# IntelLabs/bayesian-torch

Hardware: AMD Instinct MI355X
Metric: MC-samples/sec (Bayesian-ResNet18, 224^2, bs=64) (higher is better)
Workload: dtype bf16

## Files before the change

### bayesian_torch_amd/_lib.py

```python
import ctypes
import os

_HERE = os.path.dirname(os.path.abspath(__file__))
_LIB = None

KIND_REPARAM, KIND_FLIPOUT = 0, 1
ACT_F32, ACT_BF16 = 0, 1
PREC_F32, PREC_BF16, PREC_BF16X3 = 0, 1, 2
PREC_CODE = {"f32": 0, "bf16": 1, "bf16x3": 2}
FLAG_TRANSPOSED, FLAG_KL_ACCUM, FLAG_ROWFUSE, FLAG_OUT_F32, FLAG_OUT_BF16, FLAG_GATHER, FLAG_SWAP_SIGNS, FLAG_CONCURRENT = 1, 2, 4, 8, 16, 32, 64, 128
FLAG_REVERSE = 256
E_UNSUPPORTED = -3
STREAM_EPS_W, STREAM_EPS_B, STREAM_SIGN_IN, STREAM_SIGN_OUT = 0, 1, 2, 3
ABI_VERSION = 9
FLAG_LANES_SHIFT = 16
FLAG_LANES_MASK = 0xff << FLAG_LANES_SHIFT
SAMPLE_SKIP_MU = 1


class BtxError(RuntimeError):
    pass


class Geom(ctypes.Structure):
    _fields_ = [(n, ctypes.c_int32) for n in (
        "NB", "D", "H", "W", "C", "N", "KD", "KH", "KW", "sd", "sh", "sw", "pd", "ph", "pw",
        "dd", "dh", "dw", "od", "oh", "ow", "groups")]


class Rng(ctypes.Structure):
    _fields_ = [("seed", ctypes.c_uint64), ("sample_idx", ctypes.c_uint32), ("layer_id", ctypes.c_uint32),
                ("sample_idx_dev", ctypes.c_void_p)]


class BnFuse(ctypes.Structure):
    _fields_ = [("residual", ctypes.c_void_p), ("relu", ctypes.c_int32), ("mask", ctypes.c_void_p), ("dres", ctypes.c_void_p)]


class Epilogue(ctypes.Structure):
    _fields_ = [("scale", ctypes.c_void_p), ("shift", ctypes.c_void_p), ("residual", ctypes.c_void_p),
                ("relu", ctypes.c_int32), ("pool", ctypes.c_int32)]


class Lanes(ctypes.Structure):
    _fields_ = [("n", ctypes.c_int32), ("x_stride", ctypes.c_int64), ("out_stride", ctypes.c_int64),
                ("res_stride", ctypes.c_int64)]


class PlanInfo(ctypes.Structure):
    _fields_ = [(n, ctypes.c_int32) for n in ("family", "ksplits", "kper", "kgroups", "wide", "tall", "par_major", "pool_band",
                                              "nwg", "lanes")] + [("ws_bytes", ctypes.c_uint64)]


FAMILIES = ("gather", "regstage", "dma", "gemm8", "patch", "taps", "taps2", "stem", "stem_pool")


class Noise(ctypes.Structure):
    _fields_ = [("eps_w", ctypes.c_void_p), ("eps_b", ctypes.c_void_p),
                ("sign_in", ctypes.c_void_p), ("sign_out", ctypes.c_void_p), ("sampled_w", ctypes.c_void_p)]


class SampleItem(ctypes.Structure):
    _fields_ = [("geom", ctypes.POINTER(Geom)), ("mu_w", ctypes.c_void_p), ("rho_w", ctypes.c_void_p),
                ("out", ctypes.c_void_p), ("kind", ctypes.c_int32), ("layer_id", ctypes.c_uint32),
                ("src_KW", ctypes.c_int32), ("src_C", ctypes.c_int32)]


class LstmLayer(ctypes.Structure):
    _fields_ = [("mu_w", ctypes.c_void_p), ("rho_w", ctypes.c_void_p), ("mu_b", ctypes.c_void_p), ("rho_b", ctypes.c_void_p),
                ("layer_id", ctypes.c_uint32), ("sample_idx", ctypes.c_uint32), ("sample_idx_dev", ctypes.c_void_p)]


class LstmGrads(ctypes.Structure):
    _fields_ = [("dmu_w", ctypes.c_void_p), ("drho_w", ctypes.c_void_p), ("dmu_b", ctypes.c_void_p), ("drho_b", ctypes.c_void_p)]


class KlItem(ctypes.Structure):
    _fields_ = [("mu", ctypes.c_void_p), ("rho", ctypes.c_void_p), ("prior_mu_t", ctypes.c_void_p),
                ("prior_sigma_t", ctypes.c_void_p), ("dmu", ctypes.c_void_p), ("drho", ctypes.c_void_p),
                ("prior_mu", ctypes.c_float), ("prior_sigma", ctypes.c_float), ("n", ctypes.c_size_t)]


class Q8Chain(ctypes.Structure):
    _fields_ = [(n, ctypes.c_float) for n in ("s_sigma", "s_mu", "s_eps", "inv_s_eps", "s_d", "inv_s_d", "inv_s_w")] + \
               [("bias_div", ctypes.c_double)]


class Q8Add(ctypes.Structure):
    _fields_ = [(n, ctypes.c_float) for n in ("s_a", "pre_a", "s_b", "pre_b", "inv_s")] + \
               [("zero_point", ctypes.c_int32), ("relu", ctypes.c_int32)]


class Q8Delta(ctypes.Structure):
    _fields_ = [("inv_s_eps", ctypes.c_float), ("mult", ctypes.c_float), ("mean_bias", ctypes.c_int32), ("pert_bias", ctypes.c_int32),
                ("div_mean", ctypes.c_double), ("div_pert", ctypes.c_double)]


class Q8Flipout(ctypes.Structure):
    _fields_ = [(n, ctypes.c_int32) for n in ("z_x", "z_xp", "z_mean", "z_pert", "z_p2", "sin_pos", "sin_neg", "sout_pos", "sout_neg")] + \
               [(n, ctypes.c_float) for n in ("mult_xp", "mult_mean", "mult_pert", "mult_p2", "out_scale")]


class OptimItem(ctypes.Structure):
    _fields_ = [("p", ctypes.c_void_p), ("g", ctypes.c_void_p), ("state0", ctypes.c_void_p), ("state1", ctypes.c_void_p),
                ("n", ctypes.c_int64)]


class OptimHyper(ctypes.Structure):
    _fields_ = [(n, ctypes.c_float) for n in ("neg_lr", "wd", "decay_mul", "one_m_b1", "b2", "one_m_b2", "eps", "neg_step_size",
                                              "bc2s", "momentum", "one_m_damp")] + \
               [("flags", ctypes.c_uint32), ("reserved", ctypes.c_uint32 * 4)]


OPT_MAXIMIZE, OPT_NESTEROV, OPT_DECOUPLED, OPT_FIRST_STEP, OPT_COUPLED_WD = 1, 2, 4, 8, 16
OPTIM_CHUNK, OPTIM_MAX_ITEMS = 4096, 65536
Q8_BIAS_NONE, Q8_BIAS_MU, Q8_BIAS_SIGMA_EPS = 0, 1, 2

EXPORTS = ("btx_abi_version", "btx_strerror", "btx_kl_workspace_bytes", "btx_kl_gauss", "btx_kl_model_workspace_bytes",
           "btx_kl_gauss_model", "btx_kl_gauss_model_bwd", "btx_contract_wgrad",
           "btx_contract_workspace_bytes", "btx_contract_fwd", "btx_contract_fwd_ex", "btx_contract_fwd_lanes", "btx_contract_pool_shape", "btx_contract_plan_info", "btx_out_shape", "btx_fill_eps", "btx_fill_sign", "btx_rho_grad",
           "btx_mc_packed_floats", "btx_mc_accumulate", "btx_mc_accumulate_lanes", "btx_sampled_w_bytes", "btx_sample_weights", "btx_sampled_w_bytes_lanes", "btx_sample_weights_lanes", "btx_rowfuse_pack", "btx_maxpool2d_cl", "btx_avgpool_global_cl",
           "btx_bn_workspace_bytes", "btx_bn_train_fwd", "btx_bn_train_bwd", "btx_dgrad_weights",
           "btx_wgrad_workspace_bytes", "btx_contract_wgrad_ws", "btx_maxpool2d_cl_train", "btx_maxpool2d_cl_bwd",
           "btx_lstm_workspace_bytes", "btx_lstm_fwd", "btx_lstm_train_saved_bytes", "btx_lstm_train_workspace_bytes",
           "btx_lstm_fwd_train", "btx_lstm_bwd",
           "btx_calib_workspace_bytes", "btx_avu_fwd", "btx_avu_bwd", "btx_eau_fwd", "btx_eau_bwd",
           "btx_q8_weight_row_bytes", "btx_q8_quantize_act", "btx_q8_sample_weights", "btx_q8_contract",
           "btx_q8_add", "btx_q8_contract_res", "btx_q8_maxpool2d_cl", "btx_q8_avgpool2d_cl",
           "btx_q8_sample_delta", "btx_q8_contract_flipout",
           "btx_optim_sgd", "btx_optim_adam", "btx_optim_grad_norm_workspace_bytes", "btx_optim_grad_norm",
           "btx_mcloss_workspace_bytes", "btx_mc_ce_fwd", "btx_mc_ce_bwd", "btx_avu_mc_fwd", "btx_avu_mc_bwd",
           "btx_bias_grad_workspace_bytes", "btx_bias_grad")


# ... 172 lines not shown
```

### bayesian_torch_amd/csrc/btx_api.hip

```cpp
#include <hip/hip_runtime.h>
#include <math.h>
#include <string.h>
#include "../../include/btx.h"
#include <stdlib.h>
#include "btx_contract.h"
#include "btx_rng.h"
#include "btx_presample.h"

using namespace btx;

static int contract_fwd_impl(int kind, const BtxGeom* g, const void* x, const float* mu_w, const float* rho_w,
                             const float* mu_b, const float* rho_b, void* out, const BtxRng* rng, const BtxNoise* noise,
                             int act_dtype, int prec, uint32_t flags, void* ws, size_t ws_bytes, void* stream,
                             const BtxEpilogue* ep, const BtxLanes* ln) {
  if (!g || !x || !mu_w || !rho_w || !out || !rng) return BTX_E_NULL;
  const int lanes = ln ? ln->n : 1;
  if ((mu_b == nullptr) != (rho_b == nullptr)) return BTX_E_NULL;
  const uintptr_t al = (uintptr_t)x | (uintptr_t)mu_w | (uintptr_t)rho_w | (uintptr_t)out |
                       (uintptr_t)(noise && noise->eps_w ? noise->eps_w : nullptr) |
                       (uintptr_t)(ep && ep->residual ? ep->residual : nullptr);
  FwdSel sel;
  int rc = select_fwd(kind, g, act_dtype, prec, flags, (al & 15) != 0, noise, ep, &sel);
  if (rc) return rc;
  const Plan& pl = sel.pl;
  const void* sampled_w = (noise && noise->sampled_w) ? noise->sampled_w : nullptr;
  if (sel.need && (!ws || ws_bytes < sel.need)) return BTX_E_WORKSPACE;
  if (sel.need && (((uintptr_t)ws) & 15)) return BTX_E_ALIGN;

  ContractParams p;
  memset(&p, 0, sizeof(p));
  p.x = x; p.mu = mu_w; p.rho = rho_w; p.mu_b = mu_b; p.rho_b = rho_b; p.out = out;
  p.partial = pl.ksplits > 1 ? (float*)ws : nullptr;
  p.lanes = lanes; p.lane_nwg = pl.nwg; p.fd_lane_nwg = make_fastdiv((uint32_t)(pl.nwg > 0 ? pl.nwg : 1));
  if (lanes > 1) {
    p.lane_x = ln->x_stride; p.lane_out = ln->out_stride; p.lane_res = ln->res_stride;
    p.lane_partial = (long long)(plan_ws(pl, g, 1));
  }
  if (noise) {
    p.eps_w = noise->eps_w; p.eps_b = noise->eps_b;
    p.sign_in = noise->sign_in; p.sign_out = noise->sign_out;
  }
  p.NB = g->NB; p.D = g->D; p.H = g->H; p.W = g->W; p.C = g->C; p.Cg = pl.Cg;
  p.Do = pl.Do; p.Ho = pl.Ho; p.Wo = pl.Wo; p.N = g->N; p.Ng = pl.Ng;
  p.KD = g->KD; p.KH = g->KH; p.KW = g->KW;
  p.sd = g->sd; p.sh = g->sh; p.sw = g->sw; p.pd = g->pd; p.ph = g->ph; p.pw = g->pw;
  p.dd = g->dd; p.dh = g->dh; p.dw = g->dw;
  p.M = pl.M; p.K = pl.K;
  p.mtiles = pl.mtiles; p.ntiles = pl.ntiles; p.groups = g->groups; p.ksplits = pl.ksplits; p.kper = pl.kper;
  p.transposed = (flags & BTX_FLAG_TRANSPOSED) ? 1 : 0;
  p.pointwise = (!p.transposed && g->KD == 1 && g->KH == 1 && g->KW == 1 && g->sd == 1 && g->sh == 1 && g->sw == 1 &&
                 g->pd == 0 && g->ph == 0 && g->pw == 0) ? 1 : 0;
  p.out_bf16 = sel.out_bf16;
  if (ep) { p.ep_scale = ep->scale; p.ep_shift = ep->shift; p.ep_res = ep->residual; p.ep_relu = ep->relu; }
  if (flags & BTX_FLAG_ROWFUSE) {
    p.Cg = g->KW * g->C;
    p.KW = 1;
    p.sign_unaligned = 1;
  }
  p.fd_Cg = make_fastdiv((uint32_t)p.Cg); p.fd_KW = make_fastdiv((uint32_t)p.KW); p.fd_KH = make_fastdiv((uint32_t)p.KH);
  p.seed_lo = (uint32_t)rng->seed; p.seed_hi = (uint32_t)(rng->seed >> 32);
  p.sample = rng->sample_idx; p.layer = rng->layer_id;
  p.sample_ptr = rng->sample_idx_dev;
  p.fd_sd = make_fastdiv((uint32_t)g->sd); p.fd_sh = make_fastdiv((uint32_t)g->sh); p.fd_sw = make_fastdiv((uint32_t)g->sw);
  if (sel.par_major) {
    p.par_major = 1; p.par_Hh = pl.Ho / 2; p.par_Wh = pl.Wo / 2; p.par_Mq = g->NB * p.par_Hh * p.par_Wh; p.par_Mqp = sel.par_mqp;
    p.fd_par_Mqp = make_fastdiv((uint32_t)p.par_Mqp); p.fd_par_Hh = make_fastdiv((uint32_t)p.par_Hh);
    p.fd_par_Wh = make_fastdiv((uint32_t)p.par_Wh);
  }
  p.swap_signs = (flags & BTX_FLAG_SWAP_SIGNS) ? 1 : 0;
  p.reverse = (flags & BTX_FLAG_REVERSE) ? 1 : 0;
  sign_keys(rng, p.swap_signs ? BTX_STREAM_SIGN_OUT : BTX_STREAM_SIGN_IN, &p.kin_a, &p.kin_b);
  sign_keys(rng, p.swap_signs ? BTX_STREAM_SIGN_IN : BTX_STREAM_SIGN_OUT, &p.kout_a, &p.kout_b);
  {
    const long long in_elems = (long long)g->NB * g->D * g->H * g->W * g->C;
    const long long xb = in_elems * (act_dtype == BTX_ACT_BF16 ? 2 : 4), wb = (long long)g->N * pl.K * 4;
    p.x_bytes = xb < 0xffffffffLL ? (uint32_t)xb : 0xffffffffu;
    p.w_bytes = wb < 0xffffffffLL ? (uint32_t)wb : 0xffffffffu;
  }

  p.fd_inner = make_fastdiv((uint32_t)(pl.ntiles * g->groups * pl.ksplits)); p.fd_ksplits = make_fastdiv((uint32_t)pl.ksplits);
  p.fd_ntiles = make_fastdiv((uint32_t)pl.ntiles); p.fd_rtiles = make_fastdiv(1u);
  p.fd_mtiles = make_fastdiv((uint32_t)(pl.mtiles > 0 ? pl.mtiles : 1));
  {
    const double w_b = (prec == BTX_PREC_BF16 ? 2.0 : 4.0) * (double)g->N * pl.K * (kind == BTX_KIND_FLIPOUT ? 2 : 1);
    p.wg_order = (uses_tiles(sel.family) && pl.mtiles > 1 && w_b >= WG_MAJOR_MIB * 1048576.0) ? 1 : 0;
  }
  p.fd_Wo = make_fastdiv((uint32_t)pl.Wo); p.fd_Ho = make_fastdiv((uint32_t)pl.Ho); p.fd_Do = make_fastdiv((uint32_t)pl.Do);
  if (uses_tiles(sel.family)) {
    p.wt = sampled_w ? (void*)sampled_w : (void*)((unsigned char*)ws + sel.wt_off);
    p.wt_ready = sampled_w ? 1 : 0;
    p.wt_bytes = (uint32_t)sel.wt_all;
    p.wt_delta_off = (uint32_t)sel.wt_one;
    p.lane_wt = (long long)sel.wt_one;
    p.lane_wt_delta = (kind == BTX_KIND_FLIPOUT) ? 1 : 0;
  }
  hipStream_t st = (hipStream_t)stream;
  typedef int (*LaunchFn)(int, const ContractParams&, int, hipStream_t);
  auto launch = [&](LaunchFn f32, LaunchFn bf16, LaunchFn x3) {
    return (prec == BTX_PREC_BF16 ? bf16 : prec == BTX_PREC_BF16X3 ? x3 : f32)(kind, p, pl.nwg * lanes, st);
  };
  switch (sel.family) {
    case BTX_FAMILY_STEM_POOL: {
      const StemPoolPlan& spp = sel.spp;
      p.pt_R = spp.PB; p.pt_rtiles = spp.bands; p.pt_Rp = spp.Rp; p.pt_astage = spp.astage; p.st_sbytes = spp.sbytes;
      p.pt_lds = spp.lds; p.pt_PP = spp.patch_bytes; p.sp_Hq = spp.Hq; p.sp_Wq = spp.Wq;
      p.fd_rtiles = make_fastdiv((uint32_t)spp.bands);
      rc = launch_stem_pool_bf16(kind, p, pl.nwg * lanes, st);
      break;
    }
    case BTX_FAMILY_STEM: {
      const StemPlan& stp = sel.stp;
      p.pt_R = stp.R; p.pt_Rp = stp.Rp; p.pt_rtiles = stp.rtiles; p.pt_nw = stp.nw; p.pt_astage = stp.astage;
      p.st_sbytes = stp.sbytes; p.pt_lds = stp.lds; p.pt_PP = stp.patch_bytes;
      p.fd_rtiles = make_fastdiv((uint32_t)stp.rtiles);
      rc = launch(launch_contract_stem_f32, launch_contract_stem_bf16, launch_contract_stem_x3);
      break;
    }
    case BTX_FAMILY_PATCH:
    case BTX_FAMILY_TAPS:
    case BTX_FAMILY_TAPS2: {
      const PatchPlan& pt = sel.pt;
      p.pt_G = pt.G; p.pt_R = pt.R; p.pt_Rp = pt.Rp; p.pt_Wp = pt.Wp; p.pt_PP = pt.PP; p.pt_NI = pt.NI;
      p.fd_ptWp = make_fastdiv((uint32_t)pt.Wp); p.fd_ptRp = make_fastdiv((uint32_t)pt.Rp); p.fd_ptR = make_fastdiv((uint32_t)pt.R);
      p.fd_rtiles = make_fastdiv((uint32_t)pt.rtiles);
      p.pt_rtiles = pt.rtiles; p.pt_nw = pt.nw; p.pt_astage = pt.astage; p.pt_lds = pt.lds;
      p.pt_taps = pt.taps; p.pt_kg = pt.kg; p.pt_lds_g = pt.lds_g;
      p.pt_wide = (pt.taps == 33 || pt.taps == 332) ? pt.wide : 0;
      if (p.pt_wide) {
        p.fd_ntiles = make_fastdiv((uint32_t)(pl.ntiles / 2));
        p.fd_inner = make_fastdiv((uint32_t)((pl.ntiles / 2) * g->groups * pl.ksplits));
      }
      p.pt_tall = pt.tall; p.pt_P = pt.P; p.pt_Wt = pt.Wt; p.pt_ncs = pt.ncs;
      p.fd_P = make_fastdiv((uint32_t)pt.P); p.fd_Wt = make_fastdiv((uint32_t)pt.Wt); p.fd_ncs = make_fastdiv((uint32_t)pt.ncs);
      rc = launch(launch_contract_patch_f32, launch_contract_patch_bf16, launch_contract_patch_x3);
      break;
    }
    case BTX_FAMILY_GEMM8:
      p.pt_rtiles = sel.g8_pairs;
      p.fd_rtiles = make_fastdiv((uint32_t)sel.g8_pairs); p.fd_inner = make_fastdiv((uint32_t)(sel.g8_pairs * g->groups));
      rc = launch(launch_contract_gemm8_f32, launch_contract_gemm8_bf16, launch_contract_gemm8_x3);
      break;
    case BTX_FAMILY_DMA:
      rc = launch(launch_contract_dma_f32, launch_contract_dma_bf16, launch_contract_dma_x3);
      break;
    default: {
      const bool gen2 = sel.family == BTX_FAMILY_GATHER || (noise && (noise->eps_w || noise->sign_in));
      rc = (prec == BTX_PREC_BF16) ? launch_contract_bf16(kind, act_dtype == BTX_ACT_BF16, gen2, p, pl.nwg * lanes, st)
                                   : launch_contract_f32(kind, act_dtype == BTX_ACT_BF16, gen2, p, pl.nwg * lanes, st);
    }
  }
  if (rc) return rc;
  if (pl.ksplits > 1) {
    const long long total = (long long)pl.M * g->N;
// ... 124 lines not shown
```

### bayesian_torch_amd/csrc/btx_contract.h

```cpp
#pragma once
#include <hip/hip_runtime.h>
#include <stdint.h>
#include "btx_rng.h"
#include "btx_plan.h"

typedef __attribute__((ext_vector_type(8))) __bf16 bf16x8;
typedef __attribute__((ext_vector_type(4))) __bf16 bf16x4;
typedef __attribute__((ext_vector_type(4))) float f32x4;
typedef __attribute__((ext_vector_type(8))) float f32x8;
typedef __attribute__((ext_vector_type(16))) float f32x16;
typedef __attribute__((ext_vector_type(4))) uint32_t u32x4;
typedef __attribute__((ext_vector_type(2))) uint32_t u32x2;

namespace btx {

constexpr int NTHREADS = 512;
constexpr int ACTS_OFF = 0;
constexpr int SIGN_OFF = NG * BM * 16;
constexpr int WMU_OFF = SIGN_OFF + NG * BM * 4;
constexpr int WDL_OFF = WMU_OFF + NG * BN * 16;
constexpr int STAGE_BYTES = WDL_OFF + NG * BN * 16;
constexpr int LDS_BYTES = 2 * STAGE_BYTES;

struct FastDiv {
  uint32_t m, sh;
};
static inline FastDiv make_fastdiv(uint32_t d) {
  FastDiv f;
  uint32_t l = 0;
  while ((1ull << l) < d) ++l;
  f.m = (uint32_t)((((1ull << l) - d) << 32) / d + 1);
  f.sh = (l < 1 ? l : 1) | ((l > 0 ? l - 1 : 0) << 8);
  return f;
}
__device__ __forceinline__ uint32_t fdiv(uint32_t x, const FastDiv& f) {
  const uint32_t t = __umulhi(x, f.m);
  return (t + ((x - t) >> (f.sh & 31u))) >> (f.sh >> 8);
}
static inline void sign_keys(const BtxRng* rng, uint32_t stream, uint32_t* ka, uint32_t* kb) {
  const BtxPhilox4 k = btx_philox4x32_10(0u, rng->sample_idx, rng->layer_id, stream, (uint32_t)rng->seed,
                                         (uint32_t)(rng->seed >> 32));
  *ka = k.x[0];
  *kb = k.x[1];
}
__device__ __forceinline__ void fdivmod(uint32_t x, const FastDiv& f, uint32_t d, uint32_t& q, uint32_t& r) {
  q = fdiv(x, f);
  r = x - q * d;
}

struct ContractParams {
  const void* x;
  const float* mu;
  const float* rho;
  const float* mu_b;
  const float* rho_b;
  void* out;
  float* partial;
  const float* eps_w;
  const float* eps_b;
  const int8_t* sign_in;
  const int8_t* sign_out;
  int NB, D, H, W, C, Cg;
  int Do, Ho, Wo, N, Ng;
  int KD, KH, KW;
  int sd, sh, sw, pd, ph, pw, dd, dh, dw;
  int M, K;
  int mtiles, ntiles, groups, ksplits, kper;
  int transposed;
  int pointwise;
  uint32_t seed_lo, seed_hi, sample, layer;
  const uint32_t* sample_ptr;
  uint32_t kin_a, kin_b, kout_a, kout_b;
  const float* ep_scale;
  const float* ep_shift;
  const void* ep_res;
  int ep_relu;
  int out_bf16;
  int sign_unaligned;
  uint32_t x_bytes, w_bytes;
  int pt_G, pt_R, pt_Rp, pt_Wp, pt_PP, pt_NI, pt_rtiles;
  FastDiv fd_Wo, fd_Ho, fd_Do, fd_ptWp, fd_ptRp, fd_ptR;
  FastDiv fd_inner, fd_ksplits, fd_ntiles, fd_Cg, fd_KW, fd_KH, fd_rtiles;
  FastDiv fd_mtiles;
  int swap_signs;
  int par_major, par_Mq, par_Mqp, par_Hh, par_Wh;
  FastDiv fd_par_Mqp, fd_par_Hh, fd_par_Wh;
  FastDiv fd_sd, fd_sh, fd_sw;
  int wg_order;
  int pt_nw, pt_astage, pt_lds;
  int pt_kg;
  int pt_lds_g;
  int pt_taps;
  int pt_wide;
  int sp_Hq, sp_Wq;
  int st_sbytes;
  void* wt;
  uint32_t wt_bytes, wt_delta_off;
  int wt_ready;
  int pt_tall, pt_P, pt_Wt, pt_ncs;
  FastDiv fd_P, fd_Wt, fd_ncs;
  int lanes, lane_nwg;
  FastDiv fd_lane_nwg;
  long long lane_x, lane_out, lane_res, lane_wt, lane_partial;
  int lane_wt_delta;
  int reverse;
};

__device__ __forceinline__ uint32_t sample_word_scalar(const uint32_t* ptr) {
  return *(const __attribute__((address_space(4))) uint32_t*)(uintptr_t)ptr;
}

__device__ __forceinline__ int xcd_logical() {
  const int nwg = gridDim.x, L = blockIdx.x;
  const int q = nwg >> 3, r = nwg & 7, xcd = L & 7, slot = L >> 3;
  return (xcd < r ? xcd * (q + 1) : r * (q + 1) + (xcd - r) * q) + slot;
}

__device__ __forceinline__ ContractParams lane_view(const ContractParams& q, int& logical) {
  ContractParams p = q;
  if (q.reverse) logical = (int)gridDim.x - 1 - logical;
  if (q.lanes > 1) {
    uint32_t lane, loc;
    fdivmod((uint32_t)logical, q.fd_lane_nwg, (uint32_t)q.lane_nwg, lane, loc);
    logical = (int)loc;
    const long long l = (long long)lane;
    p.x = (const unsigned char*)q.x + l * q.lane_x;
    p.out = (unsigned char*)q.out + l * q.lane_out;
    if (q.ep_res) p.ep_res = (const unsigned char*)q.ep_res + l * q.lane_res;
    if (q.wt) {
      if (q.lane_wt_delta) p.wt_delta_off = q.wt_delta_off + (uint32_t)(l * q.lane_wt);
      else p.wt = (unsigned char*)q.wt + l * q.lane_wt;
    }
    if (q.partial) p.partial = (float*)((unsigned char*)q.partial + l * q.lane_partial);
    if (q.sample_ptr) p.sample_ptr = q.sample_ptr + lane;
    p.sample = q.sample + lane;
  }
  return p;
}

#define BTX_SECTION_PARAMS(name, logical_var)                                                                         \
  const __attribute__((address_space(4))) ContractParams* name##_karg =                                               \
      (const __attribute__((address_space(4))) ContractParams*)__builtin_amdgcn_kernarg_segment_ptr();                \
  asm volatile("" : "+s"(name##_karg));                                                                               \
  int logical_var = xcd_logical();                                                                                    \
  const ContractParams name = lane_view(*(const ContractParams*)name##_karg, logical_var)

__device__ __forceinline__ ContractParams lane_view_flat(const ContractParams& q, int& logical) {
  ContractParams p = q;
  const int q_rev = q.reverse, q_lnwg = q.lane_nwg, q_lwd = q.lane_wt_delta;
  const FastDiv q_fd = {q.fd_lane_nwg.m, q.fd_lane_nwg.sh};
  const long long q_lx = q.lane_x, q_lo = q.lane_out, q_lr = q.lane_res, q_lw = q.lane_wt, q_lp = q.lane_partial;
  const unsigned char* q_x = (const unsigned char*)q.x;
  unsigned char* q_out = (unsigned char*)q.out;
  const unsigned char* q_res = (const unsigned char*)q.ep_res;
  unsigned char* q_wt = (unsigned char*)q.wt;
  unsigned char* q_part = (unsigned char*)q.partial;
  const uint32_t* q_sp = q.sample_ptr;
  const uint32_t q_smp = q.sample, q_wdo = q.wt_delta_off;
  asm volatile("" ::"s"(q_rev), "s"(q_lnwg), "s"(q_lwd), "s"(q_fd.m), "s"(q_fd.sh), "s"(q_lx), "s"(q_lo), "s"(q_lr), "s"(q_lw), "s"(q_lp), "s"(q_x),
               "s"(q_out), "s"(q_res), "s"(q_wt), "s"(q_part), "s"(q_sp), "s"(q_smp), "s"(q_wdo));
  logical = q_rev ? (int)gridDim.x - 1 - logical : logical;
  uint32_t lane, loc;
  fdivmod((uint32_t)logical, q_fd, (uint32_t)q_lnwg, lane, loc);
  logical = (int)loc;
  const long long l = (long long)lane;
  const long long wo = l * q_lw;
  p.x = q_x + l * q_lx;
  p.out = q_out + l * q_lo;
  p.ep_res = q_res ? (const void*)(q_res + l * q_lr) : nullptr;
  p.wt_delta_off = q_wdo + (q_lwd ? (uint32_t)wo : 0u);
  p.wt = q_wt ? (void*)(q_wt + (q_lwd ? 0ll : wo)) : nullptr;
  p.partial = q_part ? (float*)(q_part + l * q_lp) : nullptr;
  p.sample_ptr = q_sp ? q_sp + lane : nullptr;
  p.sample = q_smp + lane;
  return p;
}
#define BTX_SECTION_PARAMS_FLAT(name, logical_var)                                                                    \
  const __attribute__((address_space(4))) ContractParams* name##_karg =                                               \
      (const __attribute__((address_space(4))) ContractParams*)__builtin_amdgcn_kernarg_segment_ptr();                \
  asm volatile("" : "+s"(name##_karg));                                                                               \
  int logical_var = xcd_logical();                                                                                    \
  const ContractParams name = lane_view_flat(*(const ContractParams*)name##_karg, logical_var)


struct RngLive {
  uint32_t sample, kin_a, kin_b, kout_a, kout_b;
};
template <int KIND>
// ... 621 lines not shown
```

### bayesian_torch_amd/csrc/btx_contract_patch.h

```cpp
#pragma once
#include <type_traits>
#include "btx_contract.h"
#include "btx_contract_dma.h"
#include "btx_epilogue.h"
#include "btx_presample.h"
#include "btx_mma.h"
#include "btx_contract_taps.h"
#include "btx_contract_taps2.h"

namespace btx {



template <int PREC, int KIND, int NW, int MI>
__global__ __launch_bounds__(64 * NW, (MI == 4) ? 1 : 2) void contract_patch_kernel(const ContractParams) {
  BTX_SECTION_PARAMS(p, logical);
  const RngLive rl = rng_live<KIND>(p);
  constexpr int NT = 64 * NW;
  constexpr int WPX = 32 * MI;
  constexpr int MAXNI = (MI == 4) ? 16 : PT_MAXNI;
  constexpr int SJ = (MI == 4) ? 4 : 2;
  using ACT = typename std::conditional<PREC == 1, __bf16, float>::type;
  constexpr int G = (PREC == 1) ? 8 : 4;
  constexpr int BK = NG * G;
// ... 180 lines not shown
      int allowed = nissued - m1;
      if (next_cb && t == (T >= 2 ? T - 2 : 0)) allowed = min(allowed, nissued - mpiece);
      wait_vmcnt(allowed);
      asm volatile("s_waitcnt lgkmcnt(0)\n\ts_barrier" ::: "memory");
      m1 = m2;
      if (++t == T) { t = 0; ++cbi; }
    };
    int s = 0;
    for (; s + 1 < nstages; s += 2) {
      iter(s, fa, fb);
      iter(s + 1, fb, fa);
    }
    if (s < nstages) iter(s, fa, fb);
  }

  {
    BTX_SECTION_PARAMS(pe, logical2);
    const int nimg = min(pe.pt_G, pe.NB - img0), nrow = min(pe.pt_R, pe.Ho - row0);
    const int nvalid = nimg * nrow * pe.Wo;
    const uint32_t m0 = (uint32_t)(img0 * pe.Ho + row0) * (uint32_t)pe.Wo;
    if constexpr (MI == 2) {
      staged_epilogue<KIND, NW>(pe, rl, accm, accd, smem, tid, wave, lane, ntile, group, split, m0, nvalid);
    } else {
#pragma unroll
      for (int hf = 0; hf < MI / 2; ++hf) {
        __builtin_amdgcn_sched_barrier(0);
        staged_epilogue<KIND, NW>(pe, rl, reinterpret_cast<const f32x16(&)[2][2]>(accm[2 * hf]),
                                  reinterpret_cast<const f32x16(&)[2][2]>(accd[2 * hf]), smem, tid, wave, lane, ntile,
                                  group, split, m0, nvalid, wave * (MI / 2) + hf, hf == 0);
      }
    }
  }
}

template <int PREC>
static int launch_contract_patch_impl(int kind, const ContractParams& p, int nwg, hipStream_t st) {
#define BTX_LAUNCH_PT(KIND, NW, MI)                                                                                 \
  do {                                                                                                            \
    auto kfn = contract_patch_kernel<PREC, KIND, NW, MI>;                                                           \
    static bool attr_done = false;                                                                                \
    if (!attr_done) {                                                                                             \
      hipError_t e = hipFuncSetAttribute((const void*)kfn, hipFuncAttributeMaxDynamicSharedMemorySize, 163840);   \
      if (e != hipSuccess) return (int)e;                                                                         \
      attr_done = true;                                                                                           \
    }                                                                                                             \
    hipLaunchKernelGGL(kfn, dim3(nwg), dim3(64 * NW), p.pt_lds, st, p);                                           \
  } while (0)
  int rc = launch_presample_impl<PREC>(kind, p, st);
  if (rc) return rc;
  if (p.pt_taps == 332) {
#define BTX_LAUNCH_T2(KIND, ...)                                                                                  \
  do {                                                                                                            \
    auto kfn = contract_taps2_kernel<PREC, KIND, ##__VA_ARGS__>;                                                  \
    static bool attr_done = false;                                                                                \
    if (!attr_done) {                                                                                             \
      hipError_t e = hipFuncSetAttribute((const void*)kfn, hipFuncAttributeMaxDynamicSharedMemorySize, 163840);   \
      if (e != hipSuccess) return (int)e;                                                                         \
      attr_done = true;                                                                                           \
    }                                                                                                             \
    hipLaunchKernelGGL(kfn, dim3(nwg), dim3(256), p.pt_lds, st, p);                                               \
  } while (0)
    if constexpr (PREC == 1) {
      if (p.pt_wide && kind == 0) {
        BTX_LAUNCH_T2(0, true);
        return (int)hipGetLastError();
      }
    }
    if (kind == 0) BTX_LAUNCH_T2(0); else BTX_LAUNCH_T2(1);
#undef BTX_LAUNCH_T2
    return (int)hipGetLastError();
  }
  if (p.pt_taps == 33) {
#define BTX_LAUNCH_TP(KIND, KG, ...)                                                                               \
  do {                                                                                                            \
    auto kfn = contract_taps_kernel<PREC, KIND, 3, 3, KG, ##__VA_ARGS__>;                                           \
    static bool attr_done = false;                                                                                \
    if (!attr_done) {                                                                                             \
      hipError_t e = hipFuncSetAttribute((const void*)kfn, hipFuncAttributeMaxDynamicSharedMemorySize, 163840);   \
      if (e != hipSuccess) return (int)e;                                                                         \
      attr_done = true;                                                                                           \
    }                                                                                                             \
    hipLaunchKernelGGL(kfn, dim3(nwg), dim3(256 * KG), p.pt_lds, st, p);                                          \
  } while (0)
    if (p.pt_kg == 2) { if (kind == 0) BTX_LAUNCH_TP(0, 2); else BTX_LAUNCH_TP(1, 2); }
    else {
      if constexpr (PREC == 1) {
        if (p.pt_wide && kind == 0) {
          BTX_LAUNCH_TP(0, 1, true);
          return (int)hipGetLastError();
        }
      }
      if (kind == 0) BTX_LAUNCH_TP(0, 1); else BTX_LAUNCH_TP(1, 1);
    }
#undef BTX_LAUNCH_TP
    return (int)hipGetLastError();
  }
  if (p.pt_nw == 4) { if (kind == 0) BTX_LAUNCH_PT(0, 4, 2); else BTX_LAUNCH_PT(1, 4, 2); }
  else { if (kind == 0) BTX_LAUNCH_PT(0, 8, 2); else BTX_LAUNCH_PT(1, 8, 2); }
#undef BTX_LAUNCH_PT
  return (int)hipGetLastError();
}

}
```

### bayesian_torch_amd/csrc/btx_contract_taps.h

```cpp
#pragma once
#include <type_traits>
#include "btx_contract.h"
#include "btx_contract_dma.h"
#include "btx_epilogue.h"
#include "btx_mma.h"

namespace btx {

__device__ __forceinline__ void dma16s(__amdgpu_buffer_rsrc_t rsrc, uint32_t voff, uint32_t soff,
                                       unsigned char* lds_wave_base) {
  __builtin_amdgcn_raw_ptr_buffer_load_lds(rsrc, (__attribute__((address_space(3))) void*)lds_wave_base, 16, voff, soff,
                                           0, 0);
}

template <int N>
__device__ __forceinline__ void end_stage() {
  asm volatile("s_waitcnt vmcnt(%0)\n\ts_waitcnt lgkmcnt(0)\n\ts_barrier" ::"n"(N) : "memory");
}

template <int I, int N, class F>
__device__ __forceinline__ void static_for(F&& f) {
  if constexpr (I < N) {
    f(std::integral_constant<int, I>{});
    static_for<I + 1, N>(f);
  }
}

constexpr int TP_MAXNI = 6;

template <int T>
constexpr int tp_pieces(int t) {
  constexpr int PST = T - 3;
  constexpr int PPS = (TP_MAXNI + PST - 1) / PST;
  if (t < 0) t += T;
  if (t >= PST) return 0;
  int n = 0;
  for (int i = 0; i < PPS; ++i)
    if (t + PST * i < TP_MAXNI) ++n;
  return n;
}

template <int PREC, int KIND, int KH, int KW, int KG, bool WIDE = false>
__global__ __launch_bounds__(256 * KG, 2) void contract_taps_kernel(const ContractParams) {
  static_assert(!WIDE || (PREC == 1 && KG == 1 && KIND == 0), "wide tile: bf16 Reparameterization, one K-group");
  constexpr int K2 = (KIND == 1 || WIDE) ? 1 : 0;
  BTX_SECTION_PARAMS(p, logical);
  constexpr int NW = 4, NT = 256, MI = 2, T = KH * KW;
  static_assert(T >= 5 && T <= 32, "tap-unrolled kernel: 5..32 taps");
  constexpr int MAXNI = TP_MAXNI;
  constexpr int PST = T - 3;
  constexpr int WOPS = K2 ? 2 : 1;
  using ACT = typename std::conditional<PREC == 1, __bf16, float>::type;
  constexpr int G = (PREC == 1) ? 8 : 4;
  constexpr int BK = NG * G;
  constexpr int ESZ = (int)sizeof(ACT);
  extern __shared__ __attribute__((aligned(16))) unsigned char smem_all[];

  uint32_t smp = p.sample;
  if (p.sample_ptr) smp = sample_word_scalar(p.sample_ptr);

  const int tid = threadIdx.x & 255;
  const int lane = tid & 63;
  const int l31 = lane & 31;
  const int h = lane >> 5;
  const int wave_all = __builtin_amdgcn_readfirstlane((int)(threadIdx.x >> 6));
  const int wave = wave_all & 3;
  const int kg = (KG == 1) ? 0 : (wave_all >> 2);
  unsigned char* const smem = smem_all + kg * p.pt_lds_g;

  uint32_t u_mtile, u_rem, u_split, u_ntile, u_group, u_t;
  const uint32_t ntg = (uint32_t)(WIDE ? p.ntiles >> 1 : p.ntiles);
  if (p.wg_order) fdivmod((uint32_t)logical, p.fd_mtiles, (uint32_t)p.mtiles, u_rem, u_mtile);
  else fdivmod((uint32_t)logical, p.fd_inner, ntg * (uint32_t)(p.groups * p.ksplits), u_mtile, u_rem);
  fdivmod(u_rem, p.fd_ksplits, (uint32_t)p.ksplits, u_t, u_split);
  fdivmod(u_t, p.fd_ntiles, ntg, u_group, u_ntile);
  const int mtile = (int)u_mtile, split = (int)u_split, ntile = (int)u_ntile, group = (int)u_group;

  const bool tall = p.pt_tall != 0;
  uint32_t u_ig, u_rt;
  if (tall) fdivmod((uint32_t)mtile, p.fd_ncs, (uint32_t)p.pt_ncs, u_rt, u_ig);
  else fdivmod((uint32_t)mtile, p.fd_rtiles, (uint32_t)p.pt_rtiles, u_ig, u_rt);
  const int img0 = tall ? 0 : (int)u_ig * p.pt_G, row0 = (int)u_rt * p.pt_R, col0 = tall ? (int)u_ig * p.pt_Wt : 0;
  auto patch_src = [&](int q, bool& ok) __attribute__((always_inline)) -> uint32_t {
    uint32_t ut, upc, ugi, upr;
    fdivmod((uint32_t)q, p.fd_ptWp, (uint32_t)p.pt_Wp, ut, upc);
    int img, ih, iw;
    if (tall) {
      fdivmod((uint32_t)row0 + ut, p.fd_P, (uint32_t)p.pt_P, ugi, upr);
      img = (int)ugi; ih = (int)upr - p.ph; iw = col0 + (int)upc - p.pw;
      ok = (int)ut < p.pt_Rp;
    } else {
      fdivmod(ut, p.fd_ptRp, (uint32_t)p.pt_Rp, ugi, upr);
      img = img0 + (int)ugi; ih = row0 + (int)upr - p.ph; iw = (int)upc - p.pw;
      ok = true;
    }
    ok = ok && img < p.NB && (unsigned)ih < (unsigned)p.H && (unsigned)iw < (unsigned)p.W;
    return (uint32_t)((img * p.H + ih) * p.W + iw);
  };
  const int ncb_total = p.Cg / BK;
  const int cb_per = p.kper / BK;
  const int cb0 = split * cb_per + kg * (cb_per / KG);
  const int ncb = (KG == 1) ? min(ncb_total, cb0 + cb_per) - cb0 : cb_per / KG;
  const int a_stage = p.pt_astage, s_stage = p.pt_astage >> 4;
  const int PT_A_OFF = 0, PT_S_OFF = 2 * a_stage, PT_W_OFF = 2 * a_stage + 2 * s_stage;
  const int PT_X_OFF = PT_W_OFF + PT_WD * DW_STAGE;

  const __amdgpu_buffer_rsrc_t x_rsrc = __builtin_amdgcn_make_buffer_rsrc((void*)p.x, 0, p.x_bytes, 0x00020000);
  const __amdgpu_buffer_rsrc_t wt_rsrc = __builtin_amdgcn_make_buffer_rsrc((void*)p.wt, 0, p.wt_bytes, 0x00020000);

  const uint32_t w_voff = (uint32_t)lane * 16u + (uint32_t)wave * 1024u;
  const uint32_t w_sbase = (uint32_t)(group * p.ntiles + (WIDE ? 2 * ntile : ntile)) * (uint32_t)(p.K / G) * 1024u;
  const uint32_t w_second = WIDE ? (uint32_t)(p.K / G) * 1024u : p.wt_delta_off;
  const uint32_t CgG = (uint32_t)(p.Cg / G);
  const int w_lds = PT_W_OFF + wave * 1024;
  int wslot = 0;
  auto issue_w = [&](uint32_t tap, uint32_t cb, int slot) __attribute__((always_inline)) {
    const uint32_t soff = w_sbase + (tap * CgG + cb * (uint32_t)NG) * 1024u;
    unsigned char* ld = smem + w_lds + slot * DW_STAGE;
    dma16s(wt_rsrc, w_voff, soff, ld);
    if constexpr (K2) dma16s(wt_rsrc, w_voff, soff + w_second, ld + 4096);
  };
  if (ncb > 0) issue_w(0u, (uint32_t)cb0, 0);

  uint32_t sg_off[2];
  bool sg_ok[2];
  uint32_t* const pix_tab = (uint32_t*)(smem + PT_S_OFF + s_stage);
#pragma unroll
  for (int j = 0; j < 2; ++j) {
    const int q = tid + NT * j;
    sg_ok[j] = q < p.pt_PP;
    bool inside;
    const uint32_t ipix = patch_src(sg_ok[j] ? q : 0, inside);
    sg_off[j] = ipix * (uint32_t)p.C + (uint32_t)(group * p.Cg);
    if (q * 4 < s_stage) pix_tab[q] = (sg_ok[j] && inside) ? sg_off[j] : 0xffffffffu;
    if (p.sign_in)
      sg_ok[j] = sg_ok[j] && inside;
  }
  asm volatile("s_waitcnt lgkmcnt(0)\n\ts_barrier" ::: "memory");

  const int g_lane = (lane & 3) ^ ((lane >> 4) & 3);
  uint32_t pp_boff[MAXNI];
  uint32_t pmask = 0;
  uint32_t pp_e[MAXNI];
#pragma unroll
  for (int j = 0; j < MAXNI; ++j) {
    const int q = 16 * (wave + NW * j) + (lane >> 2);
    pp_e[j] = pix_tab[q < p.pt_PP ? q : 0];
  }
#pragma unroll
  for (int j = 0; j < MAXNI; ++j) {
    const int q = 16 * (wave + NW * j) + (lane >> 2);
    uint32_t bo = DMA_OOB;
    if (j < p.pt_NI && q < p.pt_PP) {
      const uint32_t e = pp_e[j];
      if (e != 0xffffffffu) bo = (e + (uint32_t)(G * g_lane)) * (uint32_t)ESZ;
    }
    pp_boff[j] = bo;
    if (j < p.pt_NI && 16 * (wave + NW * j) < p.pt_PP) {
      pmask |= 1u << j;
      if (ncb > 0)
        dma16(x_rsrc, bo == DMA_OOB ? DMA_OOB : bo + (uint32_t)(cb0 * BK * ESZ), smem + PT_A_OFF + (wave + NW * j) * 1024);
    }
  }
  pmask = __builtin_amdgcn_readfirstlane(pmask);
  if (ncb > 0) {
    issue_w(1u, (uint32_t)cb0, 1);
    issue_w(2u, (uint32_t)cb0, 2);
  }

  RngLive rl = {smp, p.kin_a, p.kin_b, p.kout_a, p.kout_b};
  if (p.sample_ptr || p.lanes > 1) {
    rl.sample = __builtin_amdgcn_readfirstlane(smp);
    if constexpr (KIND == 1) {
      const uint32_t si = p.swap_signs ? 3u : 2u, so = p.swap_signs ? 2u : 3u;
      const BtxPhilox4 ki = btx_philox4x32_10(0u, rl.sample, p.layer, si, p.seed_lo, p.seed_hi);
      const BtxPhilox4 ko = btx_philox4x32_10(0u, rl.sample, p.layer, so, p.seed_lo, p.seed_hi);
      rl.kin_a = __builtin_amdgcn_readfirstlane(ki.x[0]); rl.kin_b = __builtin_amdgcn_readfirstlane(ki.x[1]);
      rl.kout_a = __builtin_amdgcn_readfirstlane(ko.x[0]); rl.kout_b = __builtin_amdgcn_readfirstlane(ko.x[1]);
    }
  }

  auto write_signs = [&](int slot, int cb) __attribute__((always_inline)) {
    if constexpr (KIND == 1) {
      unsigned char* ss = smem + PT_S_OFF + slot * s_stage;
#pragma unroll
      for (int j = 0; j < 2; ++j) {
        if (sg_ok[j]) {
          const uint32_t off = sg_off[j] + (uint32_t)(cb * BK);
          uint32_t w;
          if (p.sign_in) w = sign_word_explicit(p.sign_in, off, p.x_bytes / (uint32_t)ESZ);
          else w = btx_sign_word(off >> 5, rl.kin_a, rl.kin_b);
          if constexpr (G == 4) w <<= 8 * ((off >> 4) & 1);
          *(uint32_t*)(ss + (tid + NT * j) * 4) = w;
        }
      }
    }
  };

  int q0[MI];
#pragma unroll
  for (int mi = 0; mi < MI; ++mi) {
    const int pl = wave * 64 + mi * 32 + l31;
    uint32_t ut, uc, ugi, ur;
    if (tall) {
      fdivmod((uint32_t)pl, p.fd_Wt, (uint32_t)p.pt_Wt, ur, uc);
      q0[mi] = ((int)ur < p.pt_R) ? (int)ur * p.pt_Wp + (int)uc : 0;
    } else {
      fdivmod((uint32_t)pl, p.fd_Wo, (uint32_t)p.Wo, ut, uc);
      fdivmod(ut, p.fd_ptR, (uint32_t)p.pt_R, ugi, ur);
      const int c = (int)uc, r = (int)ur, gi = (int)ugi;
      const bool ok = (gi < p.pt_G) && (img0 + gi < p.NB) && (row0 + r < p.Ho);
      q0[mi] = ok ? (gi * p.pt_Rp + r) * p.pt_Wp + c : 0;
    }
  }
  const int row_step = p.dh * p.pt_Wp;

  constexpr bool ZI = (PREC == 1 && KG == 1);
  f32x16 accm[MI][2], accd[MI][2];
  auto clear_acc = [&](int a0) __attribute__((always_inline)) {
#pragma unroll
    for (int a = 0; a < MI; ++a)
#pragma unroll
      for (int b = 0; b < 2; ++b)
#pragma unroll
        for (int r = 0; r < 16; ++r)
          if (a >= a0) { accm[a][b][r] = 0.f; accd[a][b][r] = 0.f; }
  };
  if (!ZI || ncb <= 0) clear_acc(0);

  using Frag = StageFragT<MI>;
  auto load_frag = [&](Frag& f, int aslot, int toffv, int wsl, auto mia_tag) __attribute__((always_inline)) {
    constexpr int MIA = decltype(mia_tag)::value;
    const unsigned char* as = smem + PT_A_OFF + aslot * a_stage;
    const unsigned char* ss = smem + PT_S_OFF + aslot * s_stage;
    const unsigned char* ws = smem + PT_W_OFF + wsl * DW_STAGE;
    int q[MI];
#pragma unroll
    for (int mi = 0; mi < MI; ++mi) q[mi] = q0[mi] + toffv;
#pragma unroll
    for (int kk = 0; kk < NG / 2; ++kk) {
      const int row = 2 * kk + h;
#pragma unroll
      for (int mi = 0; mi < MIA; ++mi) f.a[kk][mi] = *(const u32x4*)(as + q[mi] * 64 + ((row ^ ((q[mi] >> 2) & 3)) * 16));
#pragma unroll
      for (int ni = 0; ni < 2; ++ni) f.wm[kk][ni] = *(const u32x4*)(ws + (row * BN + ni * 32 + l31) * 16);
    }
    if constexpr (KIND == 1) {
#pragma unroll
      for (int mi = 0; mi < MIA; ++mi) f.sw[mi] = *(const uint32_t*)(ss + q[mi] * 4);
    }
  };

  if (ncb > 0) {
    write_signs(0, cb0);
    asm volatile("s_waitcnt vmcnt(%0)\n\ts_waitcnt lgkmcnt(0)\n\ts_barrier" ::"n"(KG == 1 ? WOPS : 2 * WOPS) : "memory");
    Frag fa, fb;
    const int nvalid_px = tall ? p.pt_R * p.pt_Wt : min(p.pt_G, p.NB - img0) * min(p.pt_R, p.Ho - row0) * p.Wo;
    const bool mi1_dead = wave * 64 + 32 >= nvalid_px;
    auto kloop = [&](auto mia_tag) __attribute__((always_inline)) {
    constexpr int MIA = decltype(mia_tag)::value;
    if constexpr (KG == 1) load_frag(fa, 0, 0, 0, mia_tag);
    auto block = [&](auto par_tag, auto first_tag, int cbi, bool last) __attribute__((always_inline)) {
      constexpr int PAR = decltype(par_tag)::value;
      constexpr bool FIRST = decltype(first_tag)::value;
      static_for<0, T>([&](auto t_tag) __attribute__((always_inline)) {
        constexpr int t = decltype(t_tag)::value;
        constexpr int sp = (PAR * T + t) & 1;
        Frag& cur = (KG == 1 && sp) ? fb : fa;
        Frag& nxt = (KG == 1 && sp) ? fa : fb;
        asm volatile("" : "+v"(q0[0]), "+v"(q0[1]));
        constexpr int t3 = (t + 3) % T, c3 = (t + 3) / T;
        if constexpr (c3 == 0) {
          issue_w((uint32_t)t3, (uint32_t)(cb0 + cbi), (wslot + 3) & 3);
        } else {
          if (!last) issue_w((uint32_t)t3, (uint32_t)(cb0 + cbi + 1), (wslot + 3) & 3);
        }
        constexpr int KP = tp_pieces<T>(t);
        if constexpr (t < PST) {
          if (!last) {
            const uint32_t cboff = (uint32_t)((cb0 + cbi + 1) * BK * ESZ);
#pragma unroll
            for (int i = 0; i < KP; ++i) {
              const int j = t + PST * i;
              const uint32_t bo = pp_boff[j];
              unsigned char* dst = ((pmask >> j) & 1u) ? smem + PT_A_OFF + (PAR ^ 1) * a_stage + (wave + NW * j) * 1024
                                                        : smem + PT_X_OFF;
              dma16(x_rsrc, bo == DMA_OOB ? DMA_OOB : bo + cboff, dst);
            }
            if constexpr (t == 0) write_signs(PAR ^ 1, cb0 + cbi + 1);
          }
        }
        DeltaFrag df;
        if constexpr (KG == 1) {
          load_delta<K2>(df, smem + PT_W_OFF + wslot * DW_STAGE, l31, h);
          constexpr int t1 = (t + 1) % T, c1 = (t + 1) / T;
          load_frag(nxt, PAR ^ c1, (t1 / KW) * row_step + (t1 % KW) * p.dw, (wslot + 1) & 3, mia_tag);
          if constexpr (FIRST && t == 0) stage_mma<PREC, K2, MI, MIA, true, KIND == 1>(cur, df, accm, accd, l31, h);
          else stage_mma<PREC, K2, MI, MIA, false, KIND == 1>(cur, df, accm, accd, l31, h);
          if (!last) end_stage<WOPS + KP>();
          else end_stage<(c3 == 0) ? WOPS : 0>();
        } else {
          load_delta<KIND>(df, smem + PT_W_OFF + wslot * DW_STAGE, l31, h);
          load_frag(cur, PAR, (t / KW) * row_step + (t % KW) * p.dw, wslot, mia_tag);
          __builtin_amdgcn_sched_barrier(0);
          asm volatile("s_barrier" ::: "memory");
          __builtin_amdgcn_sched_barrier(0);
          stage_mma<PREC, KIND, MI, MIA>(cur, df, accm, accd, l31, h);
          __builtin_amdgcn_sched_barrier(0);
          if (!last) {
            end_stage<2 * WOPS + KP + tp_pieces<T>(t - 1) + tp_pieces<T>(t - 2)>();
          } else {
            constexpr int a_ = (t + 3 < T) ? 1 : 0, b_ = (t == 0) ? 1 : ((t + 2 < T) ? 1 : 0);
            end_stage<WOPS * (a_ + b_)>();
          }
        }
        wslot = (wslot + 1) & 3;
      });
    };
    if (KG == 2 && kg == 1) asm volatile("s_barrier" ::: "memory");
    using P0 = std::integral_constant<int, 0>;
    using P1 = std::integral_constant<int, 1>;
    if constexpr (ZI) {
      if constexpr (MIA < MI) clear_acc(MIA);
      block(P0{}, std::true_type{}, 0, ncb == 1);
      int cbi = 1;
      for (; cbi + 2 <= ncb; cbi += 2) {
        block(P1{}, std::false_type{}, cbi, false);
        block(P0{}, std::false_type{}, cbi + 1, cbi + 2 == ncb);
      }
      if (cbi < ncb) block(P1{}, std::false_type{}, cbi, true);
    } else {
      int cbi = 0;
      for (; cbi + 2 <= ncb; cbi += 2) {
        block(P0{}, std::false_type{}, cbi, false);
        block(P1{}, std::false_type{}, cbi + 1, cbi + 2 == ncb);
      }
      if (cbi < ncb) block(P0{}, std::false_type{}, cbi, true);
    }
    if (KG == 2 && kg == 0) asm volatile("s_barrier" ::: "memory");
    };
    if (mi1_dead) kloop(std::integral_constant<int, 1>{});
    else kloop(std::integral_constant<int, 2>{});
  }

  {
    BTX_SECTION_PARAMS(pe, logical2);
    const int nimg = min(pe.pt_G, pe.NB - img0), nrow = min(pe.pt_R, pe.Ho - row0);
    const int nvalid = nimg * nrow * pe.Wo;
    const uint32_t m0 = (uint32_t)(img0 * pe.Ho + row0) * (uint32_t)pe.Wo;
    const PixTall pmt = {pe, row0, col0};
    if constexpr (KG == 1) {
      if constexpr (WIDE) {
        float* const ba0 = (float*)(smem + NW * PT_EP_WAVE);
        float* const ba1 = ba0 + 4 * BN;
        {
          const bool has_bias = (split == 0) && (pe.mu_b != nullptr);
          const bool has_aff = (pe.ksplits == 1) && ((pe.ep_scale != nullptr) || (pe.ep_shift != nullptr));
          if (has_bias || has_aff) {
            if (tid < 64) ep_fill_constants<0>(pe, rl, ba0, tid, 2 * ntile, group, has_bias, has_aff);
            else if (tid < 128) ep_fill_constants<0>(pe, rl, ba1, tid - 64, 2 * ntile + 1, group, has_bias, has_aff);
          }
          __syncthreads();
        }
        if (tall) {
          staged_epilogue_pm<0, NW, PixTall>(pe, rl, accm, accm, smem, tid, wave, lane, 2 * ntile, group, split, pmt, -1, true, ba0);
          staged_epilogue_pm<0, NW, PixTall>(pe, rl, accd, accd, smem, tid, wave, lane, 2 * ntile + 1, group, split, pmt, -1, true, ba1);
        } else {
          staged_epilogue<0, NW>(pe, rl, accm, accm, smem, tid, wave, lane, 2 * ntile, group, split, m0, nvalid, -1, true, ba0);
          staged_epilogue<0, NW>(pe, rl, accd, accd, smem, tid, wave, lane, 2 * ntile + 1, group, split, m0, nvalid, -1, true, ba1);
        }
      } else
      if (tall) staged_epilogue_pm<KIND, NW, PixTall>(pe, rl, accm, accd, smem, tid, wave, lane, ntile, group, split, pmt);
      else staged_epilogue<KIND, NW>(pe, rl, accm, accd, smem, tid, wave, lane, ntile, group, split, m0, nvalid);
    } else {
      float* ba_lds = (float*)(smem_all + 131072);
      const bool to_partial = pe.ksplits > 1;
      const bool has_bias = (split == 0) && (pe.mu_b != nullptr);
      const bool has_aff = !to_partial && ((pe.ep_scale != nullptr) || (pe.ep_shift != nullptr));
      if (kg == 1) {
#pragma unroll
        for (int mi = 0; mi < MI; ++mi)
#pragma unroll
          for (int ni = 0; ni < 2; ++ni)
#pragma unroll
            for (int c = 0; c < 4; ++c) {
              const int i = (mi * 2 + ni) * 4 + c;
              *(f32x4*)(smem_all + (i * 256 + tid) * 16) =
                  (f32x4){accm[mi][ni][4 * c], accm[mi][ni][4 * c + 1], accm[mi][ni][4 * c + 2], accm[mi][ni][4 * c + 3]};
              if constexpr (KIND == 1)
                *(f32x4*)(smem_all + ((16 + i) * 256 + tid) * 16) =
                    (f32x4){accd[mi][ni][4 * c], accd[mi][ni][4 * c + 1], accd[mi][ni][4 * c + 2], accd[mi][ni][4 * c + 3]};
            }
      } else if (has_bias || has_aff) {
        ep_fill_constants<KIND>(pe, rl, ba_lds, tid, ntile, group, has_bias, has_aff);
      }
      __syncthreads();
      if (kg == 0) {
#pragma unroll
        for (int mi = 0; mi < MI; ++mi)
#pragma unroll
          for (int ni = 0; ni < 2; ++ni)
#pragma unroll
            for (int c = 0; c < 4; ++c) {
              const int i = (mi * 2 + ni) * 4 + c;
              const f32x4 v = *(const f32x4*)(smem_all + (i * 256 + tid) * 16);
#pragma unroll
              for (int r = 0; r < 4; ++r) accm[mi][ni][4 * c + r] += v[r];
              if constexpr (KIND == 1) {
                const f32x4 w = *(const f32x4*)(smem_all + ((16 + i) * 256 + tid) * 16);
#pragma unroll
                for (int r = 0; r < 4; ++r) accd[mi][ni][4 * c + r] += w[r];
              }
            }
      }
      __syncthreads();
      if (kg == 0) {
        if (tall) staged_epilogue_pm<KIND, NW, PixTall>(pe, rl, accm, accd, smem_all, tid, wave, lane, ntile, group, split, pmt, -1,
                                                        true, ba_lds);
        else staged_epilogue<KIND, NW>(pe, rl, accm, accd, smem_all, tid, wave, lane, ntile, group, split, m0, nvalid, -1, true,
                                       ba_lds);
      }
    }
  }
}

}
```

### bayesian_torch_amd/csrc/btx_contract_taps2.h

```cpp
#pragma once
#include <type_traits>
#include "btx_contract.h"
#include "btx_contract_dma.h"
#include "btx_contract_taps.h"
#include "btx_epilogue.h"
#include "btx_mma.h"

namespace btx {

constexpr int T2_MAXNI = 5;
constexpr int T2_WD = 3;
constexpr int T2_T = 9;

constexpr int t2_seq(int s) { return s < 4 ? 0 : (s == 4 ? 1 : (s < 7 ? 2 : 3)); }
constexpr int t2_tap(int s) {
  return s == 0 ? 0 : s == 1 ? 2 : s == 2 ? 6 : s == 3 ? 8 : s == 4 ? 4 : s == 5 ? 1 : s == 6 ? 7 : s == 7 ? 3 : 5;
}
constexpr int t2_a(int k) { return (k == 0 || k == 2) ? 1 : 0; }
constexpr int t2_b(int k) { return (k == 0 || k == 3) ? 1 : 0; }
constexpr int t2_np(int s) { return (s == 0 || s == 5 || s == 7) ? 3 : ((s == 1 || s == 6 || s == 8) ? 2 : (s == 4 ? 5 : 0)); }
constexpr int t2_p0(int s) { return (s == 1 || s == 6 || s == 8) ? 3 : 0; }
constexpr int t2_fseq(int s) { return s < 2 ? 2 : (s == 4 ? 3 : (s < 7 ? 4 : 5)); }

template <int PREC, int KIND, bool WIDE = false>
// ... 174 lines not shown
    for (int kk = 0; kk < NG / 2; ++kk) {
      const int row = 2 * kk + h;
#pragma unroll
      for (int mi = 0; mi < MIA; ++mi) f.a[kk][mi] = *(const u32x4*)(as + q[mi] * 64 + ((row ^ ((q[mi] >> 2) & 3)) * 16));
#pragma unroll
      for (int ni = 0; ni < 2; ++ni) f.wm[kk][ni] = *(const u32x4*)(ws + (row * BN + ni * 32 + l31) * 16);
    }
    if constexpr (KIND == 1) {
#pragma unroll
      for (int mi = 0; mi < MIA; ++mi) f.sw[mi] = *(const uint32_t*)(ss + q[mi] * 4);
    }
  };

  if (ncb > 0) {
    int sl0 = 0, sl1 = 1, sl2 = 2;
    issue_plane(0, MAXNI, 1, 1, cb0, sl0 * a_stage);
    issue_w((uint32_t)t2_tap(1), (uint32_t)cb0, 1);
    issue_plane(0, MAXNI, 0, 0, cb0, sl1 * a_stage);
    write_signs(1, 1, cb0, sl0 * s_stage);
    write_signs(0, 0, cb0, sl1 * s_stage);
    asm volatile("s_waitcnt vmcnt(%0)\n\ts_waitcnt lgkmcnt(0)\n\ts_barrier" ::"n"(MAXNI + WOPS) : "memory");
    Frag fa;
    const int nvalid_px = min(p.pt_G, p.NB - img0) * min(p.pt_R, p.Ho - row0) * p.Wo;
    const bool mi1_dead = wave * 64 + 32 >= nvalid_px;
    auto kloop = [&](auto mia_tag) __attribute__((always_inline)) {
      constexpr int MIA = decltype(mia_tag)::value;
      auto block = [&](int cbi, bool last) __attribute__((always_inline)) {
        static_for<0, T>([&](auto t_tag) __attribute__((always_inline)) {
          constexpr int s = decltype(t_tag)::value;
          asm volatile("" : "+v"(q0[0]), "+v"(q0[1]), "+v"(pvalid), "+v"(sg_v), "+v"(sg_base[0]), "+v"(sg_base[1]));
          asm volatile("" : "+v"(pp_base[0]), "+v"(pp_base[1]), "+v"(pp_base[2]), "+v"(pp_base[3]), "+v"(pp_base[4]));
          auto slot_of = [&](int k) __attribute__((always_inline)) { return (k % 3) == 0 ? sl0 : ((k % 3) == 1 ? sl1 : sl2); };
          constexpr int s2 = (s + 2) % T, c2 = (s + 2) / T;
          if constexpr (c2 == 0) issue_w((uint32_t)t2_tap(s2), (uint32_t)(cb0 + cbi), (wslot + 2) % WD);
          else { if (!last) issue_w((uint32_t)t2_tap(s2), (uint32_t)(cb0 + cbi + 1), (wslot + 2) % WD); }
          constexpr int NP = t2_np(s);
          if constexpr (NP > 0) {
            constexpr int FS = t2_fseq(s), FK = FS % 4, FC = FS / 4;
            if (FC == 0 || !last) {
              const int so = slot_of(FS);
              issue_plane(t2_p0(s), NP, t2_a(FK), t2_b(FK), cb0 + cbi + FC, so * a_stage);
              if constexpr (t2_p0(s) == 0) write_signs(t2_a(FK), t2_b(FK), cb0 + cbi + FC, so * s_stage);
            }
          }
          DeltaFrag df;
          load_delta<K2>(df, smem + PT_W_OFF + wslot * DW_STAGE, l31, h);
          {
            constexpr int TP = t2_tap(s);
            const int so = slot_of(t2_seq(s));
            load_frag(fa, so * a_stage, so * s_stage, ((TP / 3) == 2 ? Wp : 0) + ((TP % 3) == 2 ? 1 : 0), wslot, mia_tag);
          }
          stage_mma<PREC, K2, MI, MIA, false, KIND == 1>(fa, df, accm, accd, l31, h);
          if (!last) end_stage<WOPS + NP>();
          else end_stage<((s + 2 < T) ? WOPS : 0) + ((t2_fseq(s) < 4) ? NP : 0)>();
          wslot = (wslot + 1) % WD;
        });
        const int t0 = sl0; sl0 = sl1; sl1 = sl2; sl2 = t0;
      };
      for (int cbi = 0; cbi + 1 < ncb; ++cbi) block(cbi, false);
      block(ncb - 1, true);
    };
    if (mi1_dead) kloop(std::integral_constant<int, 1>{});
    else kloop(std::integral_constant<int, 2>{});
  }

  {
    BTX_SECTION_PARAMS(pe, logical2);
    const int nimg = min(pe.pt_G, pe.NB - img0), nrow = min(pe.pt_R, pe.Ho - row0);
    const int nvalid = nimg * nrow * pe.Wo;
    const uint32_t m0 = (uint32_t)(img0 * pe.Ho + row0) * (uint32_t)pe.Wo;
    if constexpr (WIDE) {
      float* const ba0 = (float*)(smem + NW * PT_EP_WAVE);
      float* const ba1 = ba0 + 4 * BN;
      const bool has_bias = (split == 0) && (pe.mu_b != nullptr);
      const bool has_aff = (pe.ksplits == 1) && ((pe.ep_scale != nullptr) || (pe.ep_shift != nullptr));
      if (has_bias || has_aff) {
        if (tid < 64) ep_fill_constants<0>(pe, rl, ba0, tid, 2 * ntile, group, has_bias, has_aff);
        else if (tid < 128) ep_fill_constants<0>(pe, rl, ba1, tid - 64, 2 * ntile + 1, group, has_bias, has_aff);
      }
      __syncthreads();
      staged_epilogue<0, NW>(pe, rl, accm, accm, smem, tid, wave, lane, 2 * ntile, group, split, m0, nvalid, -1, true, ba0);
      staged_epilogue<0, NW>(pe, rl, accd, accd, smem, tid, wave, lane, 2 * ntile + 1, group, split, m0, nvalid, -1, true, ba1);
    } else
    staged_epilogue<KIND, NW>(pe, rl, accm, accd, smem, tid, wave, lane, ntile, group, split, m0, nvalid);
  }
}

}
```

### bayesian_torch_amd/csrc/btx_epilogue.h

```cpp
#pragma once
#include <type_traits>
#include "btx_contract.h"

namespace btx {

template <int I, int N, class F>
__device__ __forceinline__ void static_for_ep(F&& f) {
  if constexpr (I < N) {
    f(std::integral_constant<int, I>{});
    static_for_ep<I + 1, N>(f);
  }
}

struct EpRaw {
  float mu, rho, eps, sc, sh;
};
__device__ __forceinline__ EpRaw ep_load_constants(const ContractParams& p, int t, int ntile, int group, bool has_bias,
                                                   bool has_aff) {
  EpRaw r = {0.f, 0.f, 0.f, 1.f, 0.f};
  if (t < BN) {
    const int col = ntile * BN + t;
    const int gcol = group * p.Ng + (col < p.Ng ? col : 0);
    if (has_bias && col < p.Ng) {
      r.mu = p.mu_b[gcol];
// ... 25 lines not shown
  }
}
template <int KIND>
__device__ __forceinline__ void ep_fill_constants(const ContractParams& p, const RngLive& rl, float* ba_lds, int t,
                                                  int ntile, int group, bool has_bias, bool has_aff) {
  const EpRaw r = ep_load_constants(p, t, ntile, group, has_bias, has_aff);
  ep_store_constants<KIND>(p, rl, r, ba_lds, t, ntile, group, has_bias);
}

struct PixContig {
  uint32_t m0;
  int nvalid;
  __device__ __forceinline__ uint32_t operator()(int pl, bool& ok) const { ok = pl < nvalid; return m0 + (uint32_t)pl; }
  __device__ __forceinline__ uint32_t first() const { return m0; }
  struct Walk {
    uint32_t g; int pl, nvalid;
    __device__ __forceinline__ uint32_t get(bool& ok) const { ok = pl < nvalid; return g; }
    __device__ __forceinline__ void step8() { g += 8u; pl += 8; }
  };
  __device__ __forceinline__ Walk walk(int pl) const { return Walk{m0 + (uint32_t)pl, pl, nvalid}; }
};
__device__ __forceinline__ uint32_t par_major_pixel(const ContractParams& p, uint32_t L) {
  uint32_t cls, q, t, b, nb, a;
  fdivmod(L, p.fd_par_Mqp, (uint32_t)p.par_Mqp, cls, q);
  fdivmod(q, p.fd_par_Wh, (uint32_t)p.par_Wh, t, b);
  fdivmod(t, p.fd_par_Hh, (uint32_t)p.par_Hh, nb, a);
  return (nb * (uint32_t)p.Ho + 2u * a + (cls >> 1)) * (uint32_t)p.Wo + 2u * b + (cls & 1u);
}
struct PixParity {
  const ContractParams& p;
  uint32_t m0;
  int nvalid;
  __device__ __forceinline__ uint32_t operator()(int pl, bool& ok) const {
    ok = pl < nvalid;
    return ok ? par_major_pixel(p, m0 + (uint32_t)pl) : 0u;
  }
  __device__ __forceinline__ uint32_t first() const { return 0u; }
  struct Walk {
    const ContractParams& p;
    uint32_t L; int pl, nvalid;
    __device__ __forceinline__ uint32_t get(bool& ok) const { ok = pl < nvalid; return ok ? par_major_pixel(p, L) : 0u; }
    __device__ __forceinline__ void step8() { L += 8u; pl += 8; }
  };
  __device__ __forceinline__ Walk walk(int pl) const { return Walk{p, m0 + (uint32_t)pl, pl, nvalid}; }
};
struct PixTall {
  const ContractParams& p;
  int row0, col0;
  __device__ __forceinline__ uint32_t operator()(int pl, bool& ok) const {
    uint32_t r, c, img, oh;
    fdivmod((uint32_t)pl, p.fd_Wt, (uint32_t)p.pt_Wt, r, c);
    fdivmod((uint32_t)row0 + r, p.fd_P, (uint32_t)p.pt_P, img, oh);
    const int ow = col0 + (int)c;
    ok = (int)r < p.pt_R && (int)oh < p.Ho && (int)img < p.NB && ow < p.Wo;
    return ok ? ((img * (uint32_t)p.Ho + oh) * (uint32_t)p.Wo + (uint32_t)ow) : 0u;
  }
  __device__ __forceinline__ uint32_t first() const { return 0u; }
  struct Walk {
    const ContractParams& p;
    int r, c, oh, img, col0;
    __device__ __forceinline__ uint32_t get(bool& ok) const {
      const int ow = col0 + c;
      ok = r < p.pt_R && oh < p.Ho && img < p.NB && ow < p.Wo;
      return ok ? (uint32_t)((img * p.Ho + oh) * p.Wo + ow) : 0u;
    }
    __device__ __forceinline__ void step8() {
      c += 8;
#pragma unroll
      for (int i = 0; i < 2; ++i)
        if (c >= p.pt_Wt) { c -= p.pt_Wt; ++r; if (++oh >= p.pt_P) { oh -= p.pt_P; ++img; } }
    }
  };
  __device__ __forceinline__ Walk walk(int pl) const {
    uint32_t r, c, img, oh;
    fdivmod((uint32_t)pl, p.fd_Wt, (uint32_t)p.pt_Wt, r, c);
    fdivmod((uint32_t)row0 + r, p.fd_P, (uint32_t)p.pt_P, img, oh);
    return Walk{p, (int)r, (int)c, (int)oh, (int)img, col0};
  }
};

struct EpNoHook {
  __device__ __forceinline__ void operator()() const {}
};
template <int KIND, int NW, class PM = PixContig, bool RES_PRE = false, class HOOK = EpNoHook>
__device__ __forceinline__ void staged_epilogue_pm(const ContractParams& p, const RngLive& rl, const f32x16 (&accm)[2][2],
                                                   const f32x16 (&accd)[2][2], unsigned char* smem, int tid, int wave,
                                                   int lane, int ntile, int group, int split, const PM& pm,
                                                   int pwave = -1, bool first = true,
                                                   float* ba_ext = nullptr, const HOOK& hook = HOOK{},
                                                   const uint32_t* wsh_ext = nullptr) {
  if (pwave < 0) pwave = wave;
  constexpr int EP_ROW = PT_EP_ROW;
  constexpr int EP_WAVE = PT_EP_WAVE;
  const int l31 = lane & 31, h = lane >> 5;
  const bool to_partial = p.ksplits > 1;
  const bool has_bias = (split == 0) && (p.mu_b != nullptr);
  const bool has_aff = !to_partial && ((p.ep_scale != nullptr) || (p.ep_shift != nullptr));
  const bool has_ba = has_bias || has_aff;
  float* ba_lds = ba_ext ? ba_ext : (float*)(smem + NW * EP_WAVE);
  if (has_ba && first && !ba_ext) {
    ep_fill_constants<KIND>(p, rl, ba_lds, tid, ntile, group, has_bias, has_aff);
    __syncthreads();
  }
  unsigned char* ep = smem + wave * EP_WAVE;

  constexpr bool BUFIO = RES_PRE && std::is_same<PM, PixContig>::value;
  u32x4 rpre[8];
  auto io_off = [&](int lane_) __attribute__((always_inline)) -> uint32_t {
    return ((pm.first() + (uint32_t)(pwave * 64 + (lane_ >> 3))) * (uint32_t)p.N + (uint32_t)(group * p.Ng + ntile * BN + (lane_ & 7) * 8)) * 2u;
  };
  const uint32_t io_step = 8u * (uint32_t)p.N * 2u, io_bytes = (uint32_t)p.M * (uint32_t)p.N * 2u;
  if constexpr (RES_PRE) {
    const bool all_vec = ((p.N & 7) == 0) && (((group * p.Ng) & 7) == 0) && (ntile * BN + BN <= p.Ng);
    if (all_vec && !to_partial && p.ep_res != nullptr && p.out_bf16 && p.ep_relu != 2) {
      if constexpr (BUFIO) {
        const __amdgpu_buffer_rsrc_t res_rsrc = __builtin_amdgcn_make_buffer_rsrc((void*)p.ep_res, 0, io_bytes, 0x00020000);
        const uint32_t io_voff = io_off(lane);
#pragma unroll
        for (int i = 0; i < 8; ++i) rpre[i] = __builtin_amdgcn_raw_buffer_load_b128(res_rsrc, io_voff, io_step * (uint32_t)i, 0);
      } else {
        const uint32_t cbase = (uint32_t)(group * p.Ng + ntile * BN + (lane & 7) * 8);
        auto wk = pm.walk(pwave * 64 + (lane >> 3));
#pragma unroll
        for (int i = 0; i < 8; ++i) {
          bool ok;
          const uint32_t gp = wk.get(ok);
          wk.step8();
          rpre[i] = *(const u32x4*)((const __bf16*)p.ep_res + (ok ? gp * (uint32_t)p.N + cbase : cbase + pm.first() * (uint32_t)p.N));
        }
      }
    }
  }

  hook();

  const bool fast = (ntile * BN + BN <= p.Ng) &&
                    (KIND == 0 || (!p.sign_out && (p.N & 31) == 0 && ((group * p.Ng) & 31) == 0));
  if (fast) {
    uint32_t wsh[2][2];
    uint32_t SB = 0x80000000u;
    asm volatile("" : "+s"(SB));
    if constexpr (KIND == 1) {
      if (wsh_ext) {
#pragma unroll
        for (int i = 0; i < 4; ++i) wsh[i >> 1][i & 1] = wsh_ext[i];
      } else {
#pragma unroll
        for (int mi = 0; mi < 2; ++mi) {
          bool pok;
          const uint32_t orow = pm(pwave * 64 + mi * 32 + l31, pok) * (uint32_t)p.N + (uint32_t)(group * p.Ng + ntile * BN);
#pragma unroll
          for (int ni = 0; ni < 2; ++ni)
            wsh[mi][ni] = btx_sign_word((orow + 32u * ni) >> 5, rl.kout_a, rl.kout_b) << (2 * h);
        }
      }
    }
    auto body = [&](auto bias_tag, auto aff_tag) __attribute__((always_inline)) {
      constexpr bool BIAS = decltype(bias_tag)::value, BA = decltype(aff_tag)::value;
      struct Cst { f32x4 bm, bd, sc, sh; };
      auto ldc = [&](int g, Cst& c) __attribute__((always_inline)) {
        const int cl = (g >> 2) * 32 + 8 * (g & 3) + 4 * h;
        if constexpr (BIAS) {
          c.bm = *(const f32x4*)(ba_lds + cl);
          c.bd = *(const f32x4*)(ba_lds + BN + cl);
        }
        if constexpr (BA) {
          c.sc = *(const f32x4*)(ba_lds + 2 * BN + cl);
          c.sh = *(const f32x4*)(ba_lds + 3 * BN + cl);
        }
      };
      Cst c0, c1;
      ldc(0, c0);
      static_for_ep<0, 8>([&](auto g_tag) __attribute__((always_inline)) {
        constexpr int g = decltype(g_tag)::value, ni = g >> 2, q = g & 3;
        Cst& cur = (g & 1) ? c1 : c0;
        Cst& nxt = (g & 1) ? c0 : c1;
        if constexpr (g < 7) ldc(g + 1, nxt);
        const int cl = ni * 32 + 8 * q + 4 * h;
#pragma unroll
        for (int mi = 0; mi < 2; ++mi) {
          f32x4 v;
#pragma unroll
          for (int rr = 0; rr < 4; ++rr) {
            float val = accm[mi][ni][4 * q + rr];
            if constexpr (BIAS) val += cur.bm[rr];
            if constexpr (KIND == 1) {
              float dl = accd[mi][ni][4 * q + rr];
              if constexpr (BIAS) dl += cur.bd[rr];
              const int sft = 31 - (((rr & 1) ? 31 : 15) - 4 * q - (rr >> 1));
              val += u2f(__builtin_amdgcn_bitop3_b32(f2u(dl), wsh[mi][ni] << sft, SB, 0x78));
            }
            if constexpr (BA) val = __builtin_fmaf(val, cur.sc[rr], cur.sh[rr]);
            v[rr] = val;
          }
          *(f32x4*)(ep + (mi * 32 + l31) * EP_ROW + cl * 4) = v;
        }
      });
    };
    if (has_bias) body(std::true_type{}, std::true_type{});
    else if (has_ba) body(std::false_type{}, std::true_type{});
    else body(std::false_type{}, std::false_type{});
  } else {
#pragma unroll 1
    for (int mi = 0; mi < 2; ++mi) {
      bool pix_ok;
      const uint32_t gp_ = pm(pwave * 64 + mi * 32 + l31, pix_ok);
      const uint32_t orow = (pix_ok ? gp_ : pm.first()) * (uint32_t)p.N + (uint32_t)(group * p.Ng);
#pragma unroll
      for (int ni = 0; ni < 2; ++ni) {
#pragma unroll
        for (int q = 0; q < 4; ++q) {
          const int cl = ni * 32 + 8 * q + 4 * h;
          const int c0 = ntile * BN + cl;
          float v[4];
#pragma unroll
          for (int rr = 0; rr < 4; ++rr) {
            const int col = c0 + rr;
            float val = (mi == 0 ? accm[0][ni][4 * q + rr] : accm[1][ni][4 * q + rr]);
            if (has_ba) val += ba_lds[cl + rr];
            if constexpr (KIND == 1) {
              float dl = (mi == 0 ? accd[0][ni][4 * q + rr] : accd[1][ni][4 * q + rr]);
              if (has_ba) dl += ba_lds[BN + cl + rr];
              uint32_t flip = 0;
              if (col < p.Ng && pix_ok) {
                if (p.sign_out) {
                  flip = (p.sign_out[orow + col] < 0) ? 0x80000000u : 0u;
                } else {
                  const uint32_t io = orow + col;
                  const uint32_t w1 = btx_sign_word(io >> 5, rl.kout_a, rl.kout_b);
                  flip = (w1 << (31 - btx_sign_bitpos(io & 31u))) & 0x80000000u;
                }
              }
              val += u2f(f2u(dl) ^ flip);
            }
            if (has_ba) val = __builtin_fmaf(val, ba_lds[2 * BN + cl + rr], ba_lds[3 * BN + cl + rr]);
            v[rr] = val;
          }
          *(f32x4*)(ep + (mi * 32 + l31) * EP_ROW + cl * 4) = (f32x4){v[0], v[1], v[2], v[3]};
        }
      }
    }
  }
  asm volatile("s_waitcnt lgkmcnt(0)" ::: "memory");
  __builtin_amdgcn_sched_barrier(0);

  {
    const int cg = lane & 7;
    const int col0 = ntile * BN + cg * 8;
    const int nv = min(8, p.Ng - col0);
    const uint32_t cbase = (uint32_t)(group * p.Ng + col0);
    const bool all_vec = ((p.N & 7) == 0) && (((group * p.Ng) & 7) == 0) && (ntile * BN + BN <= p.Ng) && p.ep_relu != 2;
    const bool res = !to_partial && p.ep_res != nullptr, relu = !to_partial && p.ep_relu;
    const bool relu6 = relu && p.ep_relu == 2;
    auto fast = [&](auto outk_tag, auto res_tag, auto relu_tag) __attribute__((always_inline)) {
      constexpr int OUTK = decltype(outk_tag)::value;
      constexpr bool RES = decltype(res_tag)::value, RELU = decltype(relu_tag)::value;
      auto wk = pm.walk(pwave * 64 + (lane >> 3));
      int lane_s2 = lane;
      asm volatile("" : "+v"(lane_s2));
      const uint32_t io_voff = BUFIO ? io_off(lane_s2) : 0u;
      constexpr int NP = RES_PRE ? 8 : 4;
#pragma unroll
      for (int hf = 0; hf < 8 / NP; ++hf) {
        uint32_t idx[NP];
        bool pk[NP];
        u32x4 r0[NP], r1[NP];
#pragma unroll
        for (int i = 0; i < NP; ++i) {
          if constexpr (BUFIO && OUTK == 1) {
            pk[i] = true; idx[i] = 0;
            if constexpr (RES) r0[i] = rpre[hf * NP + i];
            continue;
          }
          const uint32_t gp = wk.get(pk[i]);
          wk.step8();
          idx[i] = gp * (uint32_t)p.N + cbase;
          if constexpr (RES) {
            const uint32_t li = pk[i] ? idx[i] : cbase + pm.first() * (uint32_t)p.N;
            if constexpr (OUTK == 1 && RES_PRE) r0[i] = rpre[hf * NP + i];
            else if constexpr (OUTK == 1) r0[i] = *(const u32x4*)((const __bf16*)p.ep_res + li);
            else { r0[i] = *(const u32x4*)((const float*)p.ep_res + li); r1[i] = *(const u32x4*)((const float*)p.ep_res + li + 4); }
          }
        }
        f32x4 lo[NP], hi[NP];
#pragma unroll
        for (int i = 0; i < NP; ++i) {
          const int pix = (hf * NP + i) * 8 + (lane >> 3);
          lo[i] = *(const f32x4*)(ep + pix * EP_ROW + cg * 32);
          hi[i] = *(const f32x4*)(ep + pix * EP_ROW + cg * 32 + 16);
        }
#pragma unroll
        for (int i = 0; i < NP; ++i) {
          float v[8] = {lo[i][0], lo[i][1], lo[i][2], lo[i][3], hi[i][0], hi[i][1], hi[i][2], hi[i][3]};
          if constexpr (RES) {
            if constexpr (OUTK == 1) {
#pragma unroll
              for (int j = 0; j < 4; ++j) { v[2 * j] += u2f(r0[i][j] << 16); v[2 * j + 1] += u2f(r0[i][j] & 0xffff0000u); }
            } else {
#pragma unroll
              for (int j = 0; j < 4; ++j) { v[j] += u2f(r0[i][j]); v[4 + j] += u2f(r1[i][j]); }
            }
          }
          if constexpr (RELU) {
#pragma unroll
            for (int j = 0; j < 8; ++j) v[j] = fmaxf(v[j], 0.f);
          }
          if constexpr (OUTK == 1 && !BUFIO) {
            const f32x4 x0 = {v[0], v[1], v[2], v[3]}, x1 = {v[4], v[5], v[6], v[7]};
            const u32x2 p0 = __builtin_bit_cast(u32x2, __builtin_convertvector(x0, bf16x4));
            const u32x2 p1 = __builtin_bit_cast(u32x2, __builtin_convertvector(x1, bf16x4));
            const __amdgpu_buffer_rsrc_t out_rsrc = __builtin_amdgcn_make_buffer_rsrc((void*)p.out, 0, io_bytes, 0x00020000);
            __builtin_amdgcn_raw_buffer_store_b128((u32x4){p0[0], p0[1], p1[0], p1[1]}, out_rsrc, pk[i] ? idx[i] * 2u : 0xfffffff0u, 0, 0);
          } else
          if (pk[i]) {
            if constexpr (OUTK == 0) {
              float* dst = p.partial + (size_t)split * p.M * p.N + idx[i];
              *(f32x4*)dst = (f32x4){v[0], v[1], v[2], v[3]};
              *(f32x4*)(dst + 4) = (f32x4){v[4], v[5], v[6], v[7]};
            } else if constexpr (OUTK == 1) {
              const f32x4 x0 = {v[0], v[1], v[2], v[3]}, x1 = {v[4], v[5], v[6], v[7]};
              const u32x2 p0 = __builtin_bit_cast(u32x2, __builtin_convertvector(x0, bf16x4));
              const u32x2 p1 = __builtin_bit_cast(u32x2, __builtin_convertvector(x1, bf16x4));
              if constexpr (BUFIO) {
                const __amdgpu_buffer_rsrc_t out_rsrc = __builtin_amdgcn_make_buffer_rsrc((void*)p.out, 0, io_bytes, 0x00020000);
                __builtin_amdgcn_raw_buffer_store_b128((u32x4){p0[0], p0[1], p1[0], p1[1]}, out_rsrc, io_voff,
                                                       io_step * (uint32_t)(hf * NP + i), 0);
              } else {
                *(u32x4*)((__bf16*)p.out + idx[i]) = (u32x4){p0[0], p0[1], p1[0], p1[1]};
              }
            } else {
              float* dst = (float*)p.out + idx[i];
              *(f32x4*)dst = (f32x4){v[0], v[1], v[2], v[3]};
              *(f32x4*)(dst + 4) = (f32x4){v[4], v[5], v[6], v[7]};
            }
          }
        }
      }
    };
    using T = std::true_type;
    using F = std::false_type;
    if (all_vec) {
      if (to_partial) fast(std::integral_constant<int, 0>{}, F{}, F{});
      else if (p.out_bf16) {
        if (res) { if (relu) fast(std::integral_constant<int, 1>{}, T{}, T{}); else fast(std::integral_constant<int, 1>{}, T{}, F{}); }
        else { if (relu) fast(std::integral_constant<int, 1>{}, F{}, T{}); else fast(std::integral_constant<int, 1>{}, F{}, F{}); }
      } else {
        if (res) { if (relu) fast(std::integral_constant<int, 2>{}, T{}, T{}); else fast(std::integral_constant<int, 2>{}, T{}, F{}); }
        else { if (relu) fast(std::integral_constant<int, 2>{}, F{}, T{}); else fast(std::integral_constant<int, 2>{}, F{}, F{}); }
      }
    } else {
      auto wk = pm.walk(pwave * 64 + (lane >> 3));
#pragma unroll 1
      for (int r8 = 0; r8 < 8; ++r8) {
        const int pix = r8 * 8 + (lane >> 3);
        bool pok;
        const uint32_t gp = wk.get(pok);
        wk.step8();
        if (pok && nv > 0) {
          const uint32_t idx = gp * (uint32_t)p.N + cbase;
          const float* row = (const float*)(ep + pix * EP_ROW + cg * 32);
#pragma unroll 1
          for (int j = 0; j < nv; ++j) {
            float y = row[j];
            if (to_partial) { p.partial[(size_t)split * p.M * p.N + idx + j] = y; continue; }
            if (res) y += p.out_bf16 ? (float)((const __bf16*)p.ep_res)[idx + j] : ((const float*)p.ep_res)[idx + j];
            if (relu) y = fmaxf(y, 0.f);
            if (relu6) y = fminf(y, 6.f);
            if (p.out_bf16) ((__bf16*)p.out)[idx + j] = (__bf16)y;
            else ((float*)p.out)[idx + j] = y;
          }
        }
      }
    }
  }
}

template <int KIND, int NW, bool RES_PRE = false>
__device__ __forceinline__ void staged_epilogue(const ContractParams& p, const RngLive& rl, const f32x16 (&accm)[2][2],
                                                const f32x16 (&accd)[2][2], unsigned char* smem, int tid, int wave,
                                                int lane, int ntile, int group, int split, uint32_t m0, int nvalid,
                                                int pwave = -1, bool first = true, float* ba_ext = nullptr) {
  const PixContig pm = {m0, nvalid};
  staged_epilogue_pm<KIND, NW, PixContig, RES_PRE>(p, rl, accm, accd, smem, tid, wave, lane, ntile, group, split, pm, pwave, first,
                                                   ba_ext);
}

}
```

### bayesian_torch_amd/csrc/btx_mma.h

```cpp
#pragma once
#include "btx_contract.h"

namespace btx {

typedef __attribute__((ext_vector_type(2))) float f32x2;
typedef __attribute__((ext_vector_type(2))) __bf16 bf16x2;

__device__ __forceinline__ void split_bf16_pair(uint32_t x0, uint32_t x1, uint32_t& hi, uint32_t& lo) {
#pragma clang fp contract(off)
  const f32x2 v = {u2f(x0), u2f(x1)};
  hi = __builtin_bit_cast(uint32_t, __builtin_convertvector(v, bf16x2));
  const f32x2 r = {v[0] - u2f(hi << 16), v[1] - u2f(hi & 0xffff0000u)};
  lo = __builtin_bit_cast(uint32_t, __builtin_convertvector(r, bf16x2));
}
__device__ __forceinline__ void split_bf16_granules(const u32x4& g0, const u32x4& g1, u32x4& hi, u32x4& lo) {
  uint32_t h_, l_;
  split_bf16_pair(g0[0], g0[1], h_, l_); hi[0] = h_; lo[0] = l_;
  split_bf16_pair(g0[2], g0[3], h_, l_); hi[1] = h_; lo[1] = l_;
  split_bf16_pair(g1[0], g1[1], h_, l_); hi[2] = h_; lo[2] = l_;
  split_bf16_pair(g1[2], g1[3], h_, l_); hi[3] = h_; lo[3] = l_;
}
__device__ __forceinline__ f32x16 mfma3(const u32x4& wh, const u32x4& wl, const u32x4& ah, const u32x4& al, f32x16 c) {
  c = __builtin_amdgcn_mfma_f32_32x32x16_bf16(__builtin_bit_cast(bf16x8, wl), __builtin_bit_cast(bf16x8, ah), c, 0, 0, 0);
  c = __builtin_amdgcn_mfma_f32_32x32x16_bf16(__builtin_bit_cast(bf16x8, wh), __builtin_bit_cast(bf16x8, al), c, 0, 0, 0);
  return __builtin_amdgcn_mfma_f32_32x32x16_bf16(__builtin_bit_cast(bf16x8, wh), __builtin_bit_cast(bf16x8, ah), c, 0, 0, 0);
}

template <int MI>
struct StageFragT {
  u32x4 a[NG / 2][MI], wm[NG / 2][2];
  uint32_t sw[MI];
};
using StageFrag = StageFragT<2>;

struct DeltaFrag {
  u32x4 w[NG / 2][2];
};
template <int KIND>
__device__ __forceinline__ void load_delta(DeltaFrag& d, const unsigned char* ws, int l31, int h) {
  if constexpr (KIND == 1) {
#pragma unroll
    for (int kk = 0; kk < NG / 2; ++kk)
#pragma unroll
      for (int ni = 0; ni < 2; ++ni)
        d.w[kk][ni] = *(const u32x4*)(ws + NG * BN * 16 + ((2 * kk + h) * BN + ni * 32 + l31) * 16);
  }
}

template <int PREC, int KIND, int MI = 2, int MIA = MI, bool ZERO = false, bool MASK = true>
__device__ __forceinline__ void stage_mma(StageFragT<MI>& f, const DeltaFrag& dfrag, f32x16 (&accm)[MI][2],
                                          f32x16 (&accd)[MI][2], int l31, int h) {
    const u32x4 (&wd)[NG / 2][2] = dfrag.w;
    if constexpr (PREC == 2) {
      static_assert(NG == 4, "split-bf16: one 32x32x16 K-step per 16-k stage");
      u32x4 ah[MI], al[MI];
#pragma unroll
      for (int mi = 0; mi < MIA; ++mi) split_bf16_granules(f.a[0][mi], f.a[1][mi], ah[mi], al[mi]);
#pragma unroll
      for (int ni = 0; ni < 2; ++ni) {
        const u32x4 wh = {f.wm[0][ni][0], f.wm[0][ni][1], f.wm[1][ni][0], f.wm[1][ni][1]};
        const u32x4 wl = {f.wm[0][ni][2], f.wm[0][ni][3], f.wm[1][ni][2], f.wm[1][ni][3]};
#pragma unroll
        for (int mi = 0; mi < MIA; ++mi) accm[mi][ni] = mfma3(wh, wl, ah[mi], al[mi], accm[mi][ni]);
      }
      if constexpr (KIND == 1) {
#pragma unroll
        for (int mi = 0; mi < MIA; ++mi) {
#pragma unroll
          for (int r = 0; r < 4; ++r) {
            const uint32_t m = (f.sw[mi] << (2 * ((r >> 1) * 2 + h) + (r & 1))) & 0x80008000u;
            ah[mi][r] ^= m;
            al[mi][r] ^= m;
          }
        }
#pragma unroll
        for (int ni = 0; ni < 2; ++ni) {
          const u32x4 dh = {wd[0][ni][0], wd[0][ni][1], wd[1][ni][0], wd[1][ni][1]};
          const u32x4 dl = {wd[0][ni][2], wd[0][ni][3], wd[1][ni][2], wd[1][ni][3]};
#pragma unroll
          for (int mi = 0; mi < MIA; ++mi) accd[mi][ni] = mfma3(dh, dl, ah[mi], al[mi], accd[mi][ni]);
        }
      }
      return;
    }
#pragma unroll
    for (int kk = 0; kk < NG / 2; ++kk) {
      if constexpr (PREC == 1) {
#pragma unroll
        for (int mi = 0; mi < MIA; ++mi)
#pragma unroll
          for (int ni = 0; ni < 2; ++ni) {
            if constexpr (ZERO) {
              const f32x16 zc = {0.f, 0.f, 0.f, 0.f, 0.f, 0.f, 0.f, 0.f, 0.f, 0.f, 0.f, 0.f, 0.f, 0.f, 0.f, 0.f};
              accm[mi][ni] = __builtin_amdgcn_mfma_f32_32x32x16_bf16(
                  __builtin_bit_cast(bf16x8, f.wm[kk][ni]), __builtin_bit_cast(bf16x8, f.a[kk][mi]), kk == 0 ? zc : accm[mi][ni], 0, 0, 0);
            } else accm[mi][ni] = __builtin_amdgcn_mfma_f32_32x32x16_bf16(
                __builtin_bit_cast(bf16x8, f.wm[kk][ni]), __builtin_bit_cast(bf16x8, f.a[kk][mi]), accm[mi][ni], 0, 0, 0);
          }
      } else {
#pragma unroll
        for (int e = 0; e < 4; ++e)
#pragma unroll
          for (int mi = 0; mi < MIA; ++mi)
#pragma unroll
            for (int ni = 0; ni < 2; ++ni)
              accm[mi][ni] = __builtin_amdgcn_mfma_f32_32x32x2f32(u2f(f.wm[kk][ni][e]), u2f(f.a[kk][mi][e]), accm[mi][ni], 0, 0, 0);
      }
    }
    if constexpr (KIND == 1) {
#pragma unroll
      for (int kk = 0; kk < NG / 2; ++kk) {
        const int row = 2 * kk + h;
        if constexpr (PREC == 1) {
          if constexpr (MASK) {
#pragma unroll
            for (int mi = 0; mi < MIA; ++mi) {
              const uint32_t swr = f.sw[mi] << (4 * row);
#pragma unroll
              for (int d = 0; d < 4; ++d) f.a[kk][mi][d] ^= ((swr << d) & 0x80008000u);
            }
          }
#pragma unroll
          for (int mi = 0; mi < MIA; ++mi)
#pragma unroll
            for (int ni = 0; ni < 2; ++ni) {
              if constexpr (ZERO) {
                const f32x16 zc = {0.f, 0.f, 0.f, 0.f, 0.f, 0.f, 0.f, 0.f, 0.f, 0.f, 0.f, 0.f, 0.f, 0.f, 0.f, 0.f};
                accd[mi][ni] = __builtin_amdgcn_mfma_f32_32x32x16_bf16(
                    __builtin_bit_cast(bf16x8, wd[kk][ni]), __builtin_bit_cast(bf16x8, f.a[kk][mi]), kk == 0 ? zc : accd[mi][ni], 0, 0, 0);
              } else accd[mi][ni] = __builtin_amdgcn_mfma_f32_32x32x16_bf16(
                  __builtin_bit_cast(bf16x8, wd[kk][ni]), __builtin_bit_cast(bf16x8, f.a[kk][mi]), accd[mi][ni], 0, 0, 0);
            }
        } else {
#pragma unroll
          for (int mi = 0; mi < MIA; ++mi) {
            const uint32_t swr = f.sw[mi] << (2 * row);
#pragma unroll
            for (int e = 0; e < 4; ++e) f.a[kk][mi][e] ^= ((swr << ((e >> 1) + ((e & 1) ? 0 : 16))) & 0x80000000u);
          }
#pragma unroll
          for (int e = 0; e < 4; ++e)
#pragma unroll
            for (int mi = 0; mi < MIA; ++mi)
#pragma unroll
              for (int ni = 0; ni < 2; ++ni)
                accd[mi][ni] = __builtin_amdgcn_mfma_f32_32x32x2f32(u2f(wd[kk][ni][e]), u2f(f.a[kk][mi][e]), accd[mi][ni], 0, 0, 0);
        }
      }
    }
}

}
```

### bayesian_torch_amd/csrc/btx_plan.cpp

```cpp
#include <string.h>
#include "btx_plan.h"

namespace btx {

static inline long long plan_lanes(uint32_t flags) {
  const long long n = (flags >> BTX_FLAG_LANES_SHIFT) & 0xffu;
  return n > 1 ? n : 1;
}

static inline bool throughput_plan(uint32_t flags) { return (flags & BTX_FLAG_CONCURRENT) || plan_lanes(flags) > 1; }

static int split_k(long long base1, int units, int unit_cost, int max_split, bool full_splits, bool throughput, bool short_exit) {
  int ks = 1;
  long long best = -1;
  for (int c = 1; c <= max_split; ++c) {
    if (full_splits && units % c) continue;
    const int per = (units + c - 1) / c;
    const long long rounds = (base1 * c + SLOTS - 1) / SLOTS;
    const long long cost = rounds * (per * unit_cost + 4) + (c > 1 ? 1 : 0);
    if (best < 0 || cost < best) { best = cost; ks = c; }
    if (throughput && (base1 * c >= 64 || (short_exit && base1 * c >= 16 && per <= 16))) { ks = c; break; }
  }
  return ks;
}
// ... 312 lines not shown
      pl.mtiles = (int)(4 * tiles_per_class);
      pl.ksplits = 1; pl.kper = pl.K;
      pl.nwg = pl.mtiles * pl.ntiles * g->groups;
    }
  }
  StemPlan stp = {};
  bool stem = false;
  if (dma && rowfuse) {
    Plan sp;
    if (!make_plan(g, prec, flags, DBM, &sp) && make_stem_plan(g, act_dtype, prec, sp, &stp)) {
      sp.ksplits = 1; sp.kper = sp.K; sp.nwg = stp.nwg;
      pl = sp;
      stem = true;
    }
  }
  StemPoolPlan spp = {};
  const bool want_pool = ep && ep->pool;
  if (want_pool) {
    Plan sp;
    if (ep->pool != 1 || !stem || ep->residual || ep->relu == 2 || (noise && (noise->sign_in || noise->sign_out)) ||
        (flags & (BTX_FLAG_OUT_F32 | BTX_FLAG_SWAP_SIGNS)) || make_plan(g, prec, flags, DBM, &sp) ||
        !make_stem_pool_plan(g, act_dtype, prec, sp, &spp, lanes))
      return BTX_E_UNSUPPORTED;
    pl.nwg = spp.nwg;
  }
  PatchPlan pt = {};
  bool patch = false;
  if (dma && !rowfuse) {
    Plan pp;
    if (make_patch_plan(g, act_dtype, prec, flags, &pp, &pt, kind)) { pl = pp; patch = true; }
    else if (make_patch2_plan(g, act_dtype, prec, flags, &pp, &pt, kind)) { pl = pp; patch = true; }
  }
  int out_bf16 = (act_dtype == BTX_ACT_BF16) ? 1 : 0;
  if (flags & (BTX_FLAG_OUT_F32 | BTX_FLAG_OUT_BF16)) {
    if (!dma) return BTX_E_UNSUPPORTED;
    out_bf16 = (flags & BTX_FLAG_OUT_BF16) ? 1 : 0;
  }
  bool gemm8 = false;
  int g8_pairs = 1;
  {
    const int bk8 = NG * (prec == BTX_PREC_BF16 ? 8 : 4);
    if (dma && !rowfuse && !patch && kind == BTX_KIND_FLIPOUT &&
        !(flags & BTX_FLAG_TRANSPOSED) && g->KD == 1 && g->KH == 1 && g->KW == 1 &&
        g->pd == 0 && g->ph == 0 && g->pw == 0 && (pl.K % bk8) == 0 && pl.K >= 4 * bk8 && pl.K >= GEMM8_MIN_K && (pl.Ng % 128) == 0) {
      const long long mt = (pl.M + 255) / 256;
      g8_pairs = pl.Ng / 128;
      const long long nwg = mt * g->groups * g8_pairs;
      if (nwg * lanes <= 0x7fffffffLL) {
        gemm8 = true;
        pl.mtiles = (int)mt; pl.ksplits = 1; pl.kper = pl.K; pl.nwg = (int)nwg;
      }
    }
  }
  size_t need = plan_ws(pl, g, lanes);
  size_t wt_off = 0, wt_one = 0, wt_all = 0;
  const void* sampled_w = (noise && noise->sampled_w) ? noise->sampled_w : nullptr;
  if (sampled_w && (((uintptr_t)sampled_w) & 15)) return BTX_E_ALIGN;
  if (dma) {
    wt_off = pad256(need);
    wt_all = patch_wt_bytes(pl, g, kind, prec, &wt_one, lanes);
    if (sampled_w && wt_all < 0xfff00000ULL) wt_off = need;
    if (wt_off + wt_all >= 0xfff00000ULL) {
      if (rowfuse || (flags & (BTX_FLAG_OUT_F32 | BTX_FLAG_OUT_BF16)) || lanes > 1) return BTX_E_UNSUPPORTED;
      dma = false;
      rc = make_plan(g, prec, flags, BM, &pl);
      if (rc) return rc;
      need = plan_ws(pl, g, lanes);
    } else if (!sampled_w) {
      need = wt_off + wt_all;
    }
  }
  if ((long long)pl.nwg * lanes > 0x7fffffffLL) return BTX_E_UNSUPPORTED;
  if (!dma) s->family = gen ? BTX_FAMILY_GATHER : BTX_FAMILY_REGSTAGE;
  else if (want_pool) s->family = BTX_FAMILY_STEM_POOL;
  else if (stem) s->family = BTX_FAMILY_STEM;
  else if (patch) s->family = pt.taps == 33 ? BTX_FAMILY_TAPS : pt.taps == 332 ? BTX_FAMILY_TAPS2 : BTX_FAMILY_PATCH;
  else s->family = gemm8 ? BTX_FAMILY_GEMM8 : BTX_FAMILY_DMA;
  s->par_major = (par_major && s->family == BTX_FAMILY_DMA) ? 1 : 0;
  s->par_mqp = par_mqp; s->g8_pairs = g8_pairs; s->out_bf16 = out_bf16;
  s->stp = stp; s->spp = spp;
  if (dma && patch) s->pt = pt;
  else s->pt.kg = 1;
  s->need = need; s->wt_off = wt_off; s->wt_one = wt_one; s->wt_all = wt_all;
  return 0;
}

}

using namespace btx;

extern "C" {

int btx_out_shape(const BtxGeom* g, uint32_t flags, int32_t* Do, int32_t* Ho, int32_t* Wo) {
  if (!g || !Do || !Ho || !Wo) return BTX_E_NULL;
  if (g->NB <= 0 || g->D <= 0 || g->H <= 0 || g->W <= 0 || g->C <= 0 || g->N <= 0 || g->KD <= 0 || g->KH <= 0 ||
      g->KW <= 0 || g->sd <= 0 || g->sh <= 0 || g->sw <= 0 || g->dd <= 0 || g->dh <= 0 || g->dw <= 0 ||
      g->pd < 0 || g->ph < 0 || g->pw < 0 || g->groups <= 0)
    return BTX_E_SHAPE;
  if (g->C % g->groups || g->N % g->groups) return BTX_E_SHAPE;
  if (flags & BTX_FLAG_TRANSPOSED) {
    *Do = (g->D - 1) * g->sd - 2 * g->pd + g->dd * (g->KD - 1) + g->od + 1;
    *Ho = (g->H - 1) * g->sh - 2 * g->ph + g->dh * (g->KH - 1) + g->oh + 1;
    *Wo = (g->W - 1) * g->sw - 2 * g->pw + g->dw * (g->KW - 1) + g->ow + 1;
  } else {
    *Do = (g->D + 2 * g->pd - g->dd * (g->KD - 1) - 1) / g->sd + 1;
    *Ho = (g->H + 2 * g->ph - g->dh * (g->KH - 1) - 1) / g->sh + 1;
    *Wo = (g->W + 2 * g->pw - g->dw * (g->KW - 1) - 1) / g->sw + 1;
  }
  if (*Do <= 0 || *Ho <= 0 || *Wo <= 0) return BTX_E_SHAPE;
  return 0;
}

int btx_contract_pool_shape(const BtxGeom* g, int act_dtype, int prec, uint32_t flags, int32_t* Hq, int32_t* Wq) {
  if (!g || !(flags & BTX_FLAG_ROWFUSE) || (flags & (BTX_FLAG_TRANSPOSED | BTX_FLAG_OUT_F32 | BTX_FLAG_SWAP_SIGNS | BTX_FLAG_GATHER)))
    return 0;
  Plan sp;
  StemPlan stp;
  StemPoolPlan spp;
  if (make_plan(g, prec, flags, DBM, &sp) || !make_stem_plan(g, act_dtype, prec, sp, &stp) ||
      !make_stem_pool_plan(g, act_dtype, prec, sp, &spp))
    return 0;
  if (Hq) *Hq = spp.Hq;
  if (Wq) *Wq = spp.Wq;
  return 1;
}

size_t btx_contract_workspace_bytes(const BtxGeom* g, int kind, int act_dtype, int prec, uint32_t flags) {
  Plan a, b;
  if (!g || make_plan(g, prec, flags, BM, &a) || make_plan(g, prec, flags, DBM, &b)) return 0;
  (void)kind;
  const int lanes = (int)plan_lanes(flags);
  auto with_tiles = [&](const Plan& pl) {
    return pad256(plan_ws(pl, g, lanes)) + patch_wt_bytes(pl, g, BTX_KIND_FLIPOUT, prec, nullptr, lanes);
  };
  auto raise = [](size_t& w, size_t v) { if (v > w) w = v; };
  size_t wa = plan_ws(a, g, lanes);
  raise(wa, with_tiles(b));
  Plan b4;
  if (!make_plan(g, prec, flags, 256, &b4)) raise(wa, with_tiles(b4));
  Plan c;
  PatchPlan pt;
  if (make_patch_plan(g, act_dtype, prec, flags, &c, &pt) || make_patch2_plan(g, act_dtype, prec, flags, &c, &pt)) {
    raise(wa, with_tiles(c));
    if ((make_patch_plan(g, act_dtype, prec, flags, &c, &pt, BTX_KIND_REPARAM) ||
         make_patch2_plan(g, act_dtype, prec, flags, &c, &pt, BTX_KIND_REPARAM)) && pt.wide)
      raise(wa, with_tiles(c));
  }
  return wa;
}

int btx_contract_plan_info(int kind, const BtxGeom* g, int act_dtype, int prec, uint32_t flags, const BtxEpilogue* ep,
                           BtxPlanInfo* out) {
  if (!g || !out) return BTX_E_NULL;
  memset(out, 0, sizeof(*out));
  FwdSel s;
  const int rc = select_fwd(kind, g, act_dtype, prec, flags, false, nullptr, ep, &s);
  if (rc) return rc;
  out->family = s.family;
  out->ksplits = s.pl.ksplits;
  out->kper = s.pl.kper;
  out->kgroups = s.pt.kg;
  out->wide = s.pt.wide;
  out->tall = s.pt.tall;
  out->par_major = s.par_major;
  out->pool_band = s.spp.PB;
  out->nwg = s.pl.nwg;
  out->lanes = (int32_t)plan_lanes(flags);
  out->ws_bytes = (uint64_t)s.need;
  return 0;
}

size_t btx_sampled_w_bytes(const BtxGeom* g, int kind, int prec) { return btx_sampled_w_bytes_lanes(g, kind, prec, 1); }

size_t btx_sampled_w_bytes_lanes(const BtxGeom* g, int kind, int prec, int lanes) {
  Plan pl;
  if (!g || lanes < 1 || lanes > 255 || make_plan(g, prec, 0, DBM, &pl)) return 0;
  size_t one = 0;
  const size_t tiles = patch_wt_bytes(pl, g, kind, prec, &one, lanes);
  return tiles + (kind == BTX_KIND_FLIPOUT ? one * (prec == BTX_PREC_BF16 ? 2 : 1) : 0);
}

}
```

### bayesian_torch_amd/csrc/btx_plan.h

```cpp
#pragma once
#include <stddef.h>
#include <stdint.h>
#include "../../include/btx.h"

namespace btx {

constexpr int BM = 256;
constexpr int BN = 64;
constexpr int NG = 4;
constexpr int DBM = 512;

constexpr int PT_WD = 4;
constexpr int PT_EP_ROW = 272;
constexpr int PT_EP_WAVE = 64 * PT_EP_ROW;
constexpr int PT_MAXNI = 8;

constexpr long long SLOTS = 256;
constexpr double TALL_MIN_GAIN = 1.15;
constexpr int GEMM8_MIN_K = 128;
constexpr double WG_MAJOR_MIB = 3.0;

struct Plan {
  int Do, Ho, Wo, Cg, Ng, M, K, mtiles, ntiles, ksplits, kper, nwg;
};

struct PatchPlan {
  int G, R, Rp, Wp, PP, NI, rtiles, nw, astage, lds;
  int taps, kg, lds_g;
  int wide;
  int tall, P, Wt, ncs;
};

struct StemPlan {
  int R, Rp, rtiles, nw, astage, sbytes, lds, patch_bytes, nwg;
};

struct StemPoolPlan {
  int PB, bands, Rp, astage, sbytes, lds, patch_bytes, nwg, Hq, Wq;
};

struct FwdSel {
  int family;
  Plan pl;
  int par_major;
  int par_mqp, g8_pairs, out_bf16;
  StemPlan stp;
  StemPoolPlan spp;
  PatchPlan pt;
  size_t need, wt_off, wt_one, wt_all;
};
static inline bool uses_tiles(int family) { return family >= BTX_FAMILY_DMA; }

int select_fwd(int kind, const BtxGeom* g, int act_dtype, int prec, uint32_t flags, bool unaligned, const BtxNoise* noise,
               const BtxEpilogue* ep, FwdSel* s);

int make_plan(const BtxGeom* g, int prec, uint32_t flags, int bm, Plan* pl);
size_t plan_ws(const Plan& pl, const BtxGeom* g, int lanes = 1);
size_t patch_wt_bytes(const Plan& pl, const BtxGeom* g, int kind, int prec, size_t* one, int lanes = 1);

}
```

### bayesian_torch_amd/functional.py

```python
import ctypes
import os

import torch
import torch.nn.functional as F

from . import _lib
from . import rng as _rng

_PRECISION = os.environ.get("BTX_PRECISION", "f32")
PRECISIONS = ("f32", "bf16", "bf16x3")


def set_precision(prec):
    global _PRECISION
    if prec not in PRECISIONS:
        raise ValueError("precision must be one of %s" % (PRECISIONS,))
    _PRECISION = prec


def get_precision():
    return _PRECISION


_ALT_ORDER = True
# ... 157 lines not shown
def _alloc_out(op, nb, out_sp, dtype, device):
    if op.nd == 0:
        return torch.empty((nb, op.out_channels), dtype=dtype, device=device)
    if op.nd == 3:
        return torch.empty((nb, op.out_channels) + tuple(out_sp), dtype=dtype, device=device,
                           memory_format=torch.channels_last_3d)
    return torch.empty((nb, op.out_channels, out_sp[1], out_sp[2]), dtype=dtype, device=device,
                       memory_format=torch.channels_last)


def _sign_to_int8_cl(s, op):
    phys, _, _, _ = _to_channels_last(s.to(torch.int8), op)
    return phys


def _weight_geom(op):
    g = _lib.Geom()
    g.NB, g.D, g.H, g.W = 1, max(op.kernel[0], 1), max(op.kernel[1], 1), max(op.kernel[2], 1)
    g.C, g.N = op.in_channels, op.out_channels
    g.KD, g.KH, g.KW = op.kernel
    g.sd = g.sh = g.sw = 1
    g.dd = g.dh = g.dw = 1
    g.groups = op.groups
    return g


def sample_weights(items, seed, sample_idx, prec, device, sample_dev=None, lanes=1, bufs=None, skip_mu=False):
    L = _lib.lib()
    if not items:
        return []
    prec_c = _lib.PREC_CODE[prec]
    arr = (_lib.SampleItem * len(items))()
    geoms, outs = [], []
    for i, (kind, op, mu_p, rho_p, layer_id, *src) in enumerate(items):
        g = _weight_geom(op)
        geoms.append(g)
        nbytes = L.btx_sampled_w_bytes_lanes(ctypes.byref(g), kind, prec_c, int(lanes))
        if nbytes == 0:
            raise _lib.BtxError("btx_sampled_w_bytes: unsupported geometry")
        buf = bufs[i] if bufs is not None else torch.empty(nbytes, dtype=torch.uint8, device=device)
        if buf.numel() != nbytes:
            raise _lib.BtxError("sample_weights: buffer %d does not match the item (bytes %d != %d)" % (i, buf.numel(), nbytes))
        outs.append(buf)
        arr[i].geom = ctypes.pointer(g)
        arr[i].mu_w, arr[i].rho_w, arr[i].out = mu_p.data_ptr(), rho_p.data_ptr(), buf.data_ptr()
        arr[i].kind, arr[i].layer_id = kind, int(layer_id) & 0xFFFFFFFF
        if src:
            arr[i].src_KW, arr[i].src_C = int(src[0]), int(src[1])
    stream = torch.cuda.current_stream(device).cuda_stream
    r = _lib.Rng(int(seed), int(sample_idx) & 0xFFFFFFFF, 0, sample_dev.data_ptr() if sample_dev is not None else None)
    _lib.check(L.btx_sample_weights_lanes(arr, len(items), ctypes.byref(r), prec_c, stream, int(lanes),
                                          _lib.SAMPLE_SKIP_MU if skip_mu else 0))
    return outs


_REFUSED_CACHE = {}


def _lanes_refused(kind, op, nb, spatial, dtype, out_dtype, prec_c, extra_flags, lanes):
    flags = (_lib.FLAG_TRANSPOSED if op.transposed else 0) | extra_flags | (lanes << _lib.FLAG_LANES_SHIFT)
    if out_dtype is not None and out_dtype != dtype:
        flags |= _lib.FLAG_OUT_BF16 if out_dtype == torch.bfloat16 else _lib.FLAG_OUT_F32
    act = _lib.ACT_BF16 if dtype == torch.bfloat16 else _lib.ACT_F32
    key = (id(op), nb, spatial, kind, act, prec_c, flags)
    hit = _REFUSED_CACHE.get(key)
    if hit is None or hit[1] is not op:
        L = _lib.lib()
        g = _lib.Geom()
        g.NB, (g.D, g.H, g.W), g.C, g.N = nb, spatial, op.in_channels, op.out_channels
        g.KD, g.KH, g.KW = op.kernel
        g.sd, g.sh, g.sw = op.stride
        g.pd, g.ph, g.pw = op.padding
        g.dd, g.dh, g.dw = op.dilation
        g.od, g.oh, g.ow = op.output_padding
        g.groups = op.groups
        info = _lib.PlanInfo()
        rc = L.btx_contract_plan_info(kind, ctypes.byref(g), act, prec_c, flags, None, ctypes.byref(info))
        if len(_REFUSED_CACHE) > 4096:
            _REFUSED_CACHE.clear()
        hit = _REFUSED_CACHE[key] = (rc == _lib.E_UNSUPPORTED and
                                     L.btx_contract_plan_info(kind, ctypes.byref(g), act, prec_c, flags & ~_lib.FLAG_LANES_MASK,
                                                              None, ctypes.byref(info)) == 0, op)
    return hit[0]


def act_code(act):
    if isinstance(act, str):
        codes = {"none": 0, "relu": 1, "relu6": 2}
        if act not in codes:
            raise ValueError("epilogue activation must be one of %s, got %r" % (sorted(codes), act))
        return codes[act]
    if act is None or isinstance(act, bool):
        return int(bool(act))
    if act in (0, 1, 2):
        return int(act)
    raise ValueError("epilogue activation code must be 0, 1 or 2, got %r" % (act,))


def apply_act_aten(out, act):
    code = act_code(act)
    if code == 1:
        return torch.relu(out)
    if code == 2:
        return torch.clamp(out, 0.0, 6.0)
    return out


def contract_hip(kind, x, mu_p, rho_p, mu_b, rho_b, op, seed, sample_idx, layer_id, prec=None, noise=None,
                 extra_flags=0, out_dtype=None, epilogue=None, sampled_w=None, sample_dev=None, lanes=1, lane_batch=None,
                 self_sampling_weights=None):
    L = _lib.lib()
    if not x.is_cuda:
        raise _lib.BtxError("contract_hip needs a CUDA (ROCm) tensor")
    if x.dtype == torch.float32:
        act = _lib.ACT_F32
    elif x.dtype == torch.bfloat16:
        act = _lib.ACT_BF16
    else:
        raise _lib.BtxError("activations must be float32 or bfloat16, got %s" % x.dtype)
    prec = prec or _PRECISION
    prec_c = _lib.PREC_CODE[prec]
    xp, nb, spatial, restore = _to_channels_last(x, op)
    out_sp = op.out_spatial(spatial)
    if min(out_sp) <= 0:
        raise ValueError("output size is too small")
    lanes = int(lanes)
    nb_out, x_shared = nb, False
    if lanes > 1:
        if noise:
            raise _lib.BtxError("explicit noise tensors are single-sample (lanes == 1)")
        if lane_batch is None:
            raise _lib.BtxError("lanes > 1 needs lane_batch")
        rows = int(lane_batch) * (nb // x.shape[0] if (op.nd == 0 and x.dim() > 1 and x.shape[0] > 0) else 1)
        if nb == rows:
            x_shared, nb_out = True, rows * lanes
        elif nb != rows * lanes:
            raise _lib.BtxError("lanes=%d x lane_batch=%d does not match the input batch %d" % (lanes, lane_batch, x.shape[0]))
        nb = rows
        esz_o = (out_dtype or x.dtype).itemsize
        out_lane = nb * out_sp[0] * out_sp[1] * out_sp[2] * op.out_channels * esz_o
        x_lane = 0 if x_shared else (xp.numel() // lanes) * xp.element_size()
        pooled = epilogue is not None and epilogue.get("pool")
        if not pooled and (((x_lane | out_lane) & 15) or _lanes_refused(kind, op, nb, spatial, x.dtype, out_dtype, prec_c,
                                                                         extra_flags, lanes)):
            outs = []
            if sampled_w is not None and self_sampling_weights is not None:
                mu_p, rho_p = self_sampling_weights()
            elif sampled_w is not None and (extra_flags & _lib.FLAG_ROWFUSE):
                raise _lib.BtxError("row-fused launch with pre-sampled tiles and unaligned lane strides: the per-lane fallback "
                                    "needs the padded parameters (self_sampling_weights)")
            xl = x.reshape((lanes, -1) + tuple(x.shape[1:])) if not x_shared else None
            res = epilogue.get("residual") if epilogue is not None else None
            for l in range(lanes):
                ep_l = epilogue
                if res is not None:
                    ep_l = dict(epilogue, residual=res.reshape((lanes, -1) + tuple(res.shape[1:]))[l])
                with concurrent_plan():
                    outs.append(contract_hip(kind, x if x_shared else xl[l], mu_p, rho_p, mu_b, rho_b, op, seed,
                                             int(sample_idx) + l, layer_id, prec=prec, extra_flags=extra_flags,
                                             out_dtype=out_dtype, epilogue=ep_l,
                                             sample_dev=sample_dev[l:l + 1] if sample_dev is not None else None))
            return torch.cat(outs, 0)
    flags = (_lib.FLAG_TRANSPOSED if op.transposed else 0) | extra_flags | (_lib.FLAG_CONCURRENT if _CONCURRENT else 0)
    if lanes > 1:
        flags |= lanes << _lib.FLAG_LANES_SHIFT
    rev = 0
    if _ALT_ORDER:
        _ORDER_TOGGLE[0] ^= 1
        rev = _lib.FLAG_REVERSE if _ORDER_TOGGLE[0] else 0
    if out_dtype is not None and out_dtype != x.dtype:
        flags |= _lib.FLAG_OUT_BF16 if out_dtype == torch.bfloat16 else _lib.FLAG_OUT_F32
    gkey = (id(op), nb, spatial, kind, act, prec_c, flags)
    cached = _GEOM_CACHE.get(gkey)
    if cached is None or cached[2] is not op:
        g = _lib.Geom()
        g.NB, (g.D, g.H, g.W), g.C, g.N = nb, spatial, op.in_channels, op.out_channels
        g.KD, g.KH, g.KW = op.kernel
        g.sd, g.sh, g.sw = op.stride
        g.pd, g.ph, g.pw = op.padding
        g.dd, g.dh, g.dw = op.dilation
        g.od, g.oh, g.ow = op.output_padding
        g.groups = op.groups
        if len(_GEOM_CACHE) > 4096:
            _GEOM_CACHE.clear()
        cached = _GEOM_CACHE[gkey] = (g, L.btx_contract_workspace_bytes(ctypes.byref(g), kind, act, prec_c, flags), op)
    g, need = cached[0], cached[1]
    if epilogue is not None and epilogue.get("pool"):
        hq, wq = ctypes.c_int32(0), ctypes.c_int32(0)
        if not L.btx_contract_pool_shape(ctypes.byref(g), act, prec_c, flags, ctypes.byref(hq), ctypes.byref(wq)):
            raise _lib.BtxError("the fused stem max-pool is not available for this geometry (contract_pool_ok)")
        out_sp = (1, hq.value, wq.value)
    out = _alloc_out(op, nb_out, out_sp, out_dtype or x.dtype, x.device)
    stream = torch.cuda.current_stream(x.device).cuda_stream
    ws = _workspace(x.device, need, stream) if need else None
    r = _lib.Rng(int(seed), int(sample_idx) & 0xFFFFFFFF, int(layer_id) & 0xFFFFFFFF,
                 sample_dev.data_ptr() if sample_dev is not None else None)
    keep = []
    nz = None
    if sampled_w is not None:
        nz = _lib.Noise()
        nz.sampled_w = sampled_w.data_ptr()
        keep.append(sampled_w)
    if noise:
        nz = nz or _lib.Noise()
        if noise.get("eps_w_packed") is not None:
            t = noise["eps_w_packed"]
            keep.append(t); nz.eps_w = t.data_ptr()
        elif noise.get("eps_w") is not None:
            t = pack_gemm_major(noise["eps_w"].to(device=x.device, dtype=torch.float32), op)
            keep.append(t); nz.eps_w = t.data_ptr()
        if noise.get("eps_b") is not None:
            t = noise["eps_b"].to(device=x.device, dtype=torch.float32).contiguous()
            keep.append(t); nz.eps_b = t.data_ptr()
        if noise.get("sign_in") is not None:
            t = _sign_to_int8_cl(noise["sign_in"].to(x.device), op)
            keep.append(t); nz.sign_in = t.data_ptr()
        if noise.get("sign_out") is not None:
            so = noise["sign_out"].to(x.device)
            if op.nd == 0:
                so = so.reshape(-1, op.out_channels)
            t = _sign_to_int8_cl(so, op)
            keep.append(t); nz.sign_out = t.data_ptr()
    ev0 = None
    if _LAUNCH_LOG is not None:
        ev0 = torch.cuda.Event(enable_timing=True)
        ev0.record(torch.cuda.current_stream(x.device))
    ep = None
    if epilogue is not None:
        ep = _lib.Epilogue()
        for name in ("scale", "shift"):
            t = epilogue.get(name)
            if t is not None:
                if t.dtype != torch.float32 or t.numel() != op.out_channels or not t.is_contiguous():
                    raise ValueError("epilogue %s must be a contiguous float32 [out_channels] tensor" % name)
                keep.append(t)
                setattr(ep, name, t.data_ptr())
        res = epilogue.get("residual")
        if res is not None:
            if op.nd == 0:
                res = res.reshape(-1, op.out_channels)
            rp, _, _, _ = _to_channels_last(res, OpDesc(op.nd, op.out_channels, op.out_channels))
            rp = on_grid(rp)
            if rp.dtype != out.dtype or rp.numel() != out.numel():
                raise ValueError("epilogue residual must match the output shape and dtype")
            keep.append(rp)
            ep.residual = rp.data_ptr()
        ep.relu = act_code(epilogue.get("relu"))
        ep.pool = 1 if epilogue.get("pool") else 0
    args = (kind, ctypes.byref(g), xp.data_ptr(), mu_p.data_ptr(), rho_p.data_ptr(),
            mu_b.data_ptr() if mu_b is not None else None, rho_b.data_ptr() if rho_b is not None else None,
            out.data_ptr(), ctypes.byref(r), ctypes.byref(nz) if nz is not None else None,
            act, prec_c, flags | rev, ws.data_ptr() if ws is not None else None,
            ws.numel() if ws is not None else 0, stream, ctypes.byref(ep) if ep is not None else None)
    if lanes > 1:
        ln = _lib.Lanes()
        ln.n = lanes
        ln.x_stride = 0 if x_shared else (xp.numel() // lanes) * xp.element_size()
        ln.out_stride = (out.numel() // lanes) * out.element_size()
        ln.res_stride = ln.out_stride
        rc = L.btx_contract_fwd_lanes(*args, ctypes.byref(ln))
    else:
        rc = L.btx_contract_fwd_ex(*args)
    if rc == _lib.E_UNSUPPORTED and ep is not None and ep.relu == 2:
        ep.relu = 1
        rc = L.btx_contract_fwd_lanes(*args, ctypes.byref(ln)) if lanes > 1 else L.btx_contract_fwd_ex(*args)
        _lib.check(rc)
        out.clamp_(max=6.0)
    _lib.check(rc)
    if ev0 is not None:
        ev1 = torch.cuda.Event(enable_timing=True)
        ev1.record(torch.cuda.current_stream(x.device))
        m_rows = nb_out * out_sp[0] * out_sp[1] * out_sp[2]
        k_red = op.kernel[0] * op.kernel[1] * op.kernel[2] * (op.in_channels // op.groups)
        flops = 2.0 * m_rows * op.out_channels * k_red * (2 if kind == _lib.KIND_FLIPOUT else 1)
        tag = "%s/%s/%s k%dx%dx%d cin%d cout%d M%d" % ("flipout" if kind else "reparam", prec,
                                                     "bf16" if act == _lib.ACT_BF16 else "f32", op.kernel[0],
                                                     op.kernel[1], op.kernel[2], op.in_channels, op.out_channels, m_rows)
        _LAUNCH_LOG.append((tag, flops, ev0, ev1))
    if op.nd == 0 and x_shared:
        res = out.reshape((lanes * x.shape[0],) + tuple(x.shape[1:-1]) + (op.out_channels,))
    else:
        res = restore(out, out_sp)
    return res.contiguous() if (_OUT_LAYOUT == "contiguous" and op.nd > 0) else res


WGRAD_ATOMICS = False
BIAS_ATOMICS = False


def wgrad_hip(kind, x, dy, op, seed, sample_idx, layer_id, w_shape, signs=None, swap=False, bias=False, rowfuse=None,
              _flags=0, raw=False, sample_dev=None, rho_flat=None):
    L = _lib.lib()
    if op.transposed:
        raise _lib.BtxError("wgrad_hip wants the plain-convolution geometry (exchange x and dy for transposed layers)")
    if rowfuse is not None:
        plan, fop = rowfuse, rowfuse["op"]
        xin = rowfuse_input(x, plan, dy.dtype)
        fo = fop.out_spatial((1, plan["Hp"], plan["Wp"]))
        if (fo[1], fo[2]) != tuple(dy.shape[2:]):
            dy = F.pad(dy, (0, fo[2] - dy.shape[3], 0, fo[1] - dy.shape[2]))
        kh, kwp, cp, kw, cin = fop.kernel[1], plan["kwp"], plan["cp"], plan["kw"], plan["cin"]
        dwm, dwd, dbm, dbd = wgrad_hip(kind, xin, dy, fop, seed, sample_idx, layer_id, (fop.out_channels, cp, kh, kwp),
                                       bias=bias, _flags=_lib.FLAG_ROWFUSE, sample_dev=sample_dev)
        un = lambda t: t[:, :cin, :, :kw].contiguous() if t is not None else None
        return un(dwm), un(dwd), dbm, dbd
    xp, nb, spatial, _ = _to_channels_last(x, op)
    yop = OpDesc(op.nd, op.out_channels, op.out_channels)
    dy2 = dy.reshape(-1, op.out_channels) if op.nd == 0 else dy
    dyp, _, _, _ = _to_channels_last(dy2, yop)
    if xp.dtype != dyp.dtype:
        dyp = dyp.to(xp.dtype)
    act = _lib.ACT_BF16 if xp.dtype == torch.bfloat16 else _lib.ACT_F32
    if xp.dtype not in (torch.float32, torch.bfloat16):
        raise _lib.BtxError("activations must be float32 or bfloat16, got %s" % xp.dtype)
    g = _lib.Geom()
    g.NB, (g.D, g.H, g.W), g.C, g.N = nb, spatial, op.in_channels, op.out_channels
    g.KD, g.KH, g.KW = op.kernel
    g.sd, g.sh, g.sw = op.stride
    g.pd, g.ph, g.pw = op.padding
    g.dd, g.dh, g.dw = op.dilation
    g.groups = op.groups
    n, kred = op.out_channels, op.kernel[0] * op.kernel[1] * op.kernel[2] * (op.in_channels // op.groups)
    dev = x.device
    dwm = torch.empty(n * kred, dtype=torch.float32, device=dev)
    flip = kind == _lib.KIND_FLIPOUT
    dwd = torch.empty(n * kred, dtype=torch.float32, device=dev) if flip else None
    dbm = torch.empty(n, dtype=torch.float32, device=dev) if bias else None
    dbd = torch.empty(n, dtype=torch.float32, device=dev) if (bias and flip) else None
    nz, keep = None, []
    if signs is not None and flip:
        nz = _lib.Noise()
# ... 458 lines not shown
```

### bayesian_torch_amd/layers/base_variational_layer.py

```python
import collections
import warnings
from itertools import repeat

import torch
import torch.nn as nn
from torch.nn import Parameter

from .. import _lib
from .. import functional as BF
from .. import rng as _rng

_BACKEND = "auto"


def set_backend(name):
    global _BACKEND
    if name not in ("auto", "hip", "torch"):
        raise ValueError("backend must be auto|hip|torch")
    _BACKEND = name


def get_kernel_size(x, n):
    if isinstance(x, collections.abc.Iterable):
        return tuple(x)
# ... 214 lines not shown
            if return_kl:
                kl = kl + self.kl_div(self.mu_bias, sigma_b, self.prior_bias_mu, self.prior_bias_sigma)
        x_tmp = x * sign_in
        pert_tmp = BF.contract_aten(x_tmp, delta, b, op)
        pert = pert_tmp * sign_out
        out = outputs + pert
        for stub, t in zip(self.quint_quant, (x, outputs, sign_in, sign_out, x_tmp, pert_tmp, pert, out)):
            stub(t)
        for stub, t in zip(self.qint_quant, (sigma_w, mu, eps_w, delta)):
            stub(t)
        if return_kl:
            return out, kl
        return out

    def forward(self, input, return_kl=True):
        if self.dnn_to_bnn_flag:
            return_kl = False
        if self.quant_prepare:
            return self._forward_calibrate(input, return_kl)
        if self._use_hip(input):
            if self._needs_grad(input):
                if self.__dict__.get("_btx_lanes", 1) > 1:
                    raise _lib.BtxError("MC sample lanes are an inference feature: clear them before a training step")
                from .. import autograd as _ag
                s_idx = self._btx_sample
                self.__dict__["_btx_sample"] = s_idx + 1
                mu, rho = self._w()
                out = _ag.ContractFn.apply(self, s_idx, input, mu, rho, self.mu_bias, self.rho_bias)
            else:
                out = self._forward_hip(input)
            if return_kl:
                return out, self.kl_loss()
            return out
        return self._forward_aten(input, return_kl)

    def presample_item(self, sample_idx, prec):
        shape = getattr(self, "_btx_last_xshape", None)
        if shape is None or self.__dict__.get("_btx_fused_seq"):
            return None
        mu, rho = self._w()
        op0 = self._op
        mu_p, rho_p = BF.gemm_major_view(mu, op0), BF.gemm_major_view(rho, op0)
        plan = None
        if op0.nd == 2 and op0.in_channels <= 4:
            plan = self.__dict__.get("_btx_plans", {}).get(tuple(shape)) or BF.rowfuse_plan(op0, tuple(shape))
        if plan is not None:
            tag, op, src = ("rowfuse", plan["cp"], plan["kwp"]), plan["op"], (plan["kw"], plan["cin"])
        elif self._btx_cpad is not None:
            kw_last = op0.kernel[2] if op0.nd else 1
            tag, op, src = ("cpad", self._btx_cpad), self._op_pad, (kw_last, op0.in_channels)
        else:
            tag, op, src = ("plain",), op0, ()
        if src and op0.transposed:
            return None
        if op0.nd == 0 and (self.precision or prec) != "bf16x3" and self._lanes()[0] == 1 and not BF._CONCURRENT:
            rows = 1
            for v in shape[:-1]:
                rows *= int(v)
            if rows <= 256:
                return None
        bk = 32 if (self.precision or prec) == "bf16" else 16
        cg = op.in_channels // op.groups
        if plan is None and cg % bk != 0:
            return None
        kind = _lib.KIND_FLIPOUT if self._family == "flipout" else _lib.KIND_REPARAM
        key = (_rng.seed(), self._sample_key(sample_idx), self._btx_layer_id, self.precision or prec, tag)
        return key, (kind, op, mu_p, rho_p, self._btx_layer_id) + tuple(src)

    def _lanes(self):
        return self.__dict__.get("_btx_lanes", 1), self.__dict__.get("_btx_lane_batch")

    def _sample_key(self, sample_idx):
        sdev = getattr(self, "_btx_sample_dev", None)
        n = self.__dict__.get("_btx_lanes", 1)
        return ("dev", sdev.data_ptr(), n) if sdev is not None else (int(sample_idx), n)

    def _take_presampled(self, sample_idx, prec, tag):
        pre = self.__dict__.get("_btx_pre")
        self.__dict__["_btx_pre"] = None
        if pre is not None and pre[0] == (_rng.seed(), self._sample_key(sample_idx), self._btx_layer_id, prec, tag):
            return pre[1]
        return None

    def _forward_hip(self, x, noise=None, sample_idx=None, epilogue=None, gather=False):
        if self._op.nd > 0 and x.dim() == self._op.nd + 1:
            if epilogue is not None and epilogue.get("residual") is not None:
                epilogue = dict(epilogue, residual=epilogue["residual"].unsqueeze(0))
            return self._forward_hip(x.unsqueeze(0), noise, sample_idx, epilogue, gather).squeeze(0)
        mu, rho = self._w()
        mu_p, rho_p = BF.gemm_major_view(mu, self._op), BF.gemm_major_view(rho, self._op)
        lanes, lane_batch = self._lanes()
        if lanes > 1 and noise is not None:
            raise _lib.BtxError("explicit noise is single-sample: clear the sample lanes first (rng.set_sample_lanes)")
        if sample_idx is None:
            sample_idx = self._btx_sample
            self.__dict__["_btx_sample"] = sample_idx + lanes
        kind = _lib.KIND_FLIPOUT if self._family == "flipout" else _lib.KIND_REPARAM
        mb = self.mu_bias.detach() if self.mu_bias is not None else None
        rb = self.rho_bias.detach() if self.rho_bias is not None else None
        op = self._op
        self.__dict__["_btx_last_xshape"] = tuple(x.shape)
        plan = self._rowfuse_plan(x) if noise is None else None
        if plan is not None:
            prec = self.precision or BF.get_precision()
            pre = self._take_presampled(sample_idx, prec, ("rowfuse", plan["cp"], plan["kwp"]))
            mu_f, rho_f = BF.rowfuse_weights(mu_p, rho_p, plan) if pre is None else (mu_p, rho_p)
            xin = self._rowfuse_packed(x, plan, torch.bfloat16 if prec == "bf16" else torch.float32)
            fo = plan["op"].out_spatial((1, plan["Hp"], plan["Wp"]))
            if epilogue is not None and epilogue.get("residual") is not None and fo[2] != plan["Wo"]:
                raise _lib.BtxError("residual epilogue is not available for this row-fused stem geometry")
            out = BF.contract_hip(kind, xin, mu_f, rho_f, mb, rb, plan["op"], _rng.seed(), sample_idx,
                                  self._btx_layer_id, prec=prec, extra_flags=_lib.FLAG_ROWFUSE, out_dtype=x.dtype,
                                  epilogue=epilogue, sampled_w=pre, sample_dev=getattr(self, "_btx_sample_dev", None),
                                  lanes=lanes, lane_batch=lane_batch,
                                  self_sampling_weights=(lambda: BF.rowfuse_weights(mu_p, rho_p, plan)) if pre is not None else None)
            if epilogue is not None and epilogue.get("pool"):
                return out
            return out[:, :, :plan["Ho"], :plan["Wo"]]
        if epilogue is not None and epilogue.get("pool"):
            raise _lib.BtxError("the fused max-pool needs the row-fused stem path (pool_fusable)")
        if self._btx_cpad is not None and noise is None:
            extra = self._btx_cpad - op.in_channels
            x = BF.pad_channels(x, op, extra)
            mu_p = torch.nn.functional.pad(mu_p, (0, extra))
            rho_p = torch.nn.functional.pad(rho_p, (0, extra))
            op = self._op_pad
        pre = None
        if noise is None:
            tag = ("cpad", self._btx_cpad) if self._btx_cpad is not None else ("plain",)
            pre = self._take_presampled(sample_idx, self.precision or BF.get_precision(), tag)
        return BF.contract_hip(kind, x, mu_p, rho_p, mb, rb, op, _rng.seed(), sample_idx,
                               self._btx_layer_id, prec=self.precision, noise=noise, epilogue=epilogue, sampled_w=pre,
                               sample_dev=getattr(self, "_btx_sample_dev", None),
                               extra_flags=_lib.FLAG_GATHER if gather else 0, lanes=lanes, lane_batch=lane_batch)

    def _rowfuse_packed(self, x, plan, dtype):
        store = self.__dict__.get("_btx_static_x")
        if store is None or store is False:
            return BF.rowfuse_input(x, plan, dtype)
        key = (x.data_ptr(), tuple(x.shape), x.dtype, dtype)
        st = store.get(id(self))
        if st is None or st[0] != key:
            if torch.cuda.is_current_stream_capturing():
                raise _lib.BtxError("static_input: the stem input must be packed before the capture starts")
            st = (key, BF.rowfuse_input(x, plan, dtype))
            store[id(self)] = st
        return st[1]

    def _static_repack(self, x, store):
        st = store.get(id(self))
        if st is None or st[0][0] != x.data_ptr():
            return
        plan = self._rowfuse_plan(x)
        st[1].copy_(BF.rowfuse_input(x, plan, st[1].dtype))

    def pool_fusable(self, x):
        if not self._use_hip(x) or x.dtype != torch.bfloat16 or (self.precision or BF.get_precision()) != "bf16":
            return False
        plan = self._rowfuse_plan(x)
        if plan is None:
            return False
        fo = plan["op"].out_spatial((1, plan["Hp"], plan["Wp"]))
        if (fo[1], fo[2]) != (plan["Ho"], plan["Wo"]):
            return False
        return BF.contract_pool_ok(plan["op"], x.shape[0], (1, plan["Hp"], plan["Wp"]), torch.bfloat16, "bf16",
                                   _lib.FLAG_ROWFUSE)

    def forward_fused(self, x, scale=None, shift=None, residual=None, relu=False, pool=False, act=None):
        relu = BF.act_code(act if act is not None else relu)
        if self._use_hip(x) and not self._needs_grad(x):
            return self._forward_hip(x, epilogue=dict(scale=scale, shift=shift, residual=residual, relu=relu, pool=pool))
        if pool:
            raise _lib.BtxError("forward_fused(pool=True) is an inference-only GPU path (pool_fusable)")
        out = self.forward(x, return_kl=False) if self._use_hip(x) else self._forward_aten(x, False)
        shape = (1, -1) + (1,) * self._op.nd if self._op.nd else (1, -1)
        if scale is not None:
            out = out * scale.view(shape).to(out.dtype)
        if shift is not None:
            out = out + shift.view(shape).to(out.dtype)
        if residual is not None:
            out = out + residual
        return BF.apply_act_aten(out, relu)

    def _rowfuse_plan(self, x):
        if self._op.nd != 2 or self._op.in_channels > 4 or not x.is_cuda:
            return None
        cache = self.__dict__.setdefault("_btx_plans", {})
        key = tuple(x.shape)
        if key not in cache:
            if len(cache) > 64:
                cache.clear()
            cache[key] = BF.rowfuse_plan(self._op, key)
        return cache[key]

    def materialize_noise(self, sample_idx, x_shape=None, out_shape=None, x_dtype=None, signs=True, sample_dev=None):
        mu, _ = self._w()
        op, seed, lid = self._op, _rng.seed(), self._btx_layer_id
        cin, cpad = op.in_channels, self._btx_cpad
        if sample_dev is not None and signs and self._family == "flipout" and x_shape is not None:
            raise _lib.BtxError("sign tensors of padded layouts need a host-side sample index: this layer cannot run in a captured step")
        _fill_eps = BF.fill_eps_hip
        if sample_dev is not None:
            _fill_eps = lambda n, dev, sd, si, li, st: BF.fill_eps_hip(n, dev, sd, si, li, st, sample_dev=sample_dev)
        plan = None
        if x_shape is not None and op.nd == 2 and cin <= 4:
            plan = BF.rowfuse_plan(op, tuple(x_shape))
        if plan is not None:
            kh, kw, kwp, cp = op.kernel[1], plan["kw"], plan["kwp"], plan["cp"]
            flat = _fill_eps(mu.shape[0] * kh * kwp * cp, mu.device, seed, sample_idx, lid, _lib.STREAM_EPS_W)
            e = flat.reshape(mu.shape[0], kh, kwp, cp)[:, :, :kw, :cin].permute(0, 3, 1, 2).contiguous()
            d = {"eps_w": e}
            getattr(self, "eps_" + self._wn).copy_(e)
            if self.mu_bias is not None:
                d["eps_b"] = _fill_eps(self.mu_bias.numel(), mu.device, seed, sample_idx, lid, _lib.STREAM_EPS_B)
                self.eps_bias.copy_(d["eps_b"])
            if self._family == "flipout" and signs:
                n, _, h, w = x_shape
                sp = BF.fill_sign_hip(n * plan["Hp"] * plan["Wp"] * cp, mu.device, seed, sample_idx, lid,
                                      _lib.STREAM_SIGN_IN).reshape(n, plan["Hp"], plan["Wp"], cp)
                d["sign_in"] = sp[:, plan["ph"]:plan["ph"] + h, plan["pw"]:plan["pw"] + w, :cin].permute(0, 3, 1, 2)
                fo = plan["op"].out_spatial((1, plan["Hp"], plan["Wp"]))
                so = BF.fill_sign_hip(n * fo[1] * fo[2] * op.out_channels, mu.device, seed, sample_idx, lid,
                                      _lib.STREAM_SIGN_OUT).reshape(n, fo[1], fo[2], op.out_channels)
                d["sign_out"] = so[:, :plan["Ho"], :plan["Wo"], :].permute(0, 3, 1, 2)
            return d
        if cpad is None:
            flat = _fill_eps(mu.numel(), mu.device, seed, sample_idx, lid, _lib.STREAM_EPS_W)
        else:
            flat = _fill_eps(mu.numel() // cin * cpad, mu.device, seed, sample_idx, lid, _lib.STREAM_EPS_W)
            flat = flat.reshape(-1, cpad)[:, :cin].reshape(-1)
        d = {"eps_w": BF.unpack_gemm_major(flat, tuple(mu.shape), op)}
        getattr(self, "eps_" + self._wn).copy_(d["eps_w"])
        if self.mu_bias is not None:
            d["eps_b"] = _fill_eps(self.mu_bias.numel(), mu.device, seed, sample_idx, lid, _lib.STREAM_EPS_B)
            self.eps_bias.copy_(d["eps_b"])
        if self._family == "flipout" and x_shape is not None and signs:
            def cl_to_logical(flat8, shape):
                if op.nd == 0:
                    return flat8.reshape(shape)
                n, c, sp = shape[0], shape[1], tuple(shape[2:])
                t = flat8.reshape((n,) + sp + (c,))
                return t.permute((0, op.nd + 1) + tuple(range(1, op.nd + 1)))
            nin = 1
            for v in x_shape:
                nin *= v
            nout = 1
            for v in out_shape:
                nout *= v
            if cpad is None:
                d["sign_in"] = cl_to_logical(BF.fill_sign_hip(nin, mu.device, seed, sample_idx, lid,
                                                              _lib.STREAM_SIGN_IN), tuple(x_shape))
            else:
                sp = BF.fill_sign_hip(nin // cin * cpad, mu.device, seed, sample_idx, lid, _lib.STREAM_SIGN_IN)
                d["sign_in"] = cl_to_logical(sp.reshape(-1, cpad)[:, :cin].reshape(-1), tuple(x_shape))
# ... 245 lines not shown
```

### bayesian_torch_amd/models/fuse.py

```python
import types

import torch
import torch.nn as nn


STEM_POOL_FUSION = True


def fold_bn(bn):
    with torch.no_grad():
        w = bn.weight.float() if bn.weight is not None else torch.ones_like(bn.running_var, dtype=torch.float32)
        b = bn.bias.float() if bn.bias is not None else torch.zeros_like(bn.running_var, dtype=torch.float32)
        scale = w / torch.sqrt(bn.running_var.float() + bn.eps)
        shift = b - bn.running_mean.float() * scale
    return scale.contiguous(), shift.contiguous()


def _is_var(m):
    return hasattr(m, "forward_fused")


def _is_q8(m):
    return getattr(m, "_btx_q8", False)


def _is_lstm(m):
    return hasattr(m, "fused_sequence") and hasattr(m, "ih") and hasattr(m, "hh")


def _out(o):
    return o[0] if isinstance(o, tuple) else o


def _textbook_block(m, x):
    y = torch.relu(m.bn1(_out(m.conv1(x))))
    y = m.bn2(_out(m.conv2(y)))
    if hasattr(m, "conv3") and hasattr(m, "bn3"):
        y = m.bn3(_out(m.conv3(torch.relu(y))))
    idt = x if m.downsample is None else m.downsample(x)
    return torch.relu(y + _out(idt))


def _textbook_resnet(m, x):
    x = m.maxpool(torch.relu(m.bn1(_out(m.conv1(x)))))
    x = m.layer4(m.layer3(m.layer2(m.layer1(x))))
    return _out(m.fc(m.avgpool(x).flatten(1)))


def _behaves_like(m, ref_fn, shapes):
    import copy
    import warnings
    with warnings.catch_warnings():
        warnings.simplefilter("ignore")
        try:
            probe = copy.deepcopy(m).to("cpu").float().eval()
            with torch.no_grad():
                for name, prm in probe.named_parameters():
                    if name.rsplit(".", 1)[-1].startswith("rho_"):
                        prm.fill_(-40.0)
        except Exception:
            return False
        for shp in shapes:
            try:
                with torch.no_grad(), torch.random.fork_rng(devices=[]):
                    x = torch.randn(*shp, generator=torch.Generator().manual_seed(7))
                    torch.manual_seed(1234)
                    a = _out(type(probe).forward(probe, x))
                    torch.manual_seed(1234)
                    b = ref_fn(probe, x)
                return bool(a.shape == b.shape and torch.allclose(a, b, rtol=1e-5, atol=1e-6))
            except Exception:
                continue
    return False


def _cin(conv):
    for k in ("in_channels", "in_features"):
        if hasattr(conv, k):
            return int(getattr(conv, k))
    return None


def block_is_textbook(m):
    if "_btx_textbook" in m.__dict__:
        return m.__dict__["_btx_textbook"]
    ok = all(hasattr(m, k) for k in ("conv1", "bn1", "conv2", "bn2", "downsample")) and _cin(m.conv1) is not None
    if ok:
        ok = _behaves_like(m, _textbook_block, [(2, _cin(m.conv1), 8, 8)])
        if not ok:
            import warnings
            warnings.warn("bayesian_torch_amd.models.fuse: %s has conv1/bn1/conv2/bn2/downsample but not the ResNet block dataflow "
                          "(relu(bn(conv)) ... + identity, relu): left unfused" % type(m).__name__)
    object.__setattr__(m, "_btx_textbook", bool(ok))
    return bool(ok)


def resnet_is_textbook(model):
    if "_btx_textbook" in model.__dict__:
        return model.__dict__["_btx_textbook"]
    ok = all(hasattr(model, k) for k in ("conv1", "bn1", "maxpool", "layer1", "layer2", "layer3", "layer4", "avgpool", "fc"))
    ok = ok and _cin(model.conv1) is not None
    if ok:
        c = _cin(model.conv1)
        ok = _behaves_like(model, _textbook_resnet, [(1, c, 64, 64), (1, c, 224, 224)])
        if not ok:
            import warnings
            warnings.warn("bayesian_torch_amd.models.fuse: %s has a ResNet's attributes but not its forward: stem / head left unfused"
                          % type(model).__name__)
    object.__setattr__(model, "_btx_textbook", bool(ok))
    return bool(ok)


class _Folded:

    def __init__(self, conv, bn):
        self.conv, self.bn = conv, bn
        self._key, self._ss = None, None

    def _scale_shift(self):
        bn = self.bn
        ts = [t for t in (bn.weight, bn.bias, bn.running_mean, bn.running_var) if t is not None]
        key = tuple((t.data_ptr(), t._version) for t in ts)
        if key != self._key:
            self._ss, self._key = fold_bn(bn), key
        return self._ss

    def __call__(self, x, residual=None, relu=False, pool=False):
        scale, shift = self._scale_shift()
        return self.conv.forward_fused(x, scale, shift, residual, relu, pool=pool)


def _downsample(self, x):
    f = self.__dict__.get("_fds")
    if f is not None:
        return f(x)
    return x if self.downsample is None else self.downsample(x)


def _basic_forward(self, x):
    idt = _downsample(self, x)
    y = self._f1(x, None, True)
    return self._f2(y, idt, True)


def _bottleneck_forward(self, x):
    idt = _downsample(self, x)
    y = self._f1(x, None, True)
    y = self._f2(y, None, True)
    return self._f3(y, idt, True)


def fuse_resnet(model):
    n = 0
    for m in model.modules():
        names = [k for k in ("conv1", "bn1", "conv2", "bn2") if hasattr(m, k)]
        if (len(names) == 4 and hasattr(m, "downsample") and _is_var(m.conv1) and _is_var(m.conv2)
                and ("_f1" in m.__dict__ or block_is_textbook(m))):
            object.__setattr__(m, "_f1", _Folded(m.conv1, m.bn1))
            object.__setattr__(m, "_f2", _Folded(m.conv2, m.bn2))
            if hasattr(m, "conv3") and _is_var(m.conv3):
                object.__setattr__(m, "_f3", _Folded(m.conv3, m.bn3))
                m.forward = types.MethodType(_bottleneck_forward, m)
            else:
                m.forward = types.MethodType(_basic_forward, m)
            ds = m.downsample
            if isinstance(ds, nn.Sequential) and len(ds) == 2 and _is_var(ds[0]) and isinstance(ds[1], nn.BatchNorm2d):
                object.__setattr__(m, "_fds", _Folded(ds[0], ds[1]))
            n += 1
    if (hasattr(model, "conv1") and hasattr(model, "bn1") and hasattr(model, "maxpool") and _is_var(model.conv1)
            and ("_stem" in model.__dict__ or resnet_is_textbook(model))):
        object.__setattr__(model, "_stem", _Folded(model.conv1, model.bn1))

        def pool(mp, y):
            ints = all(isinstance(v, int) for v in (mp.kernel_size, mp.stride, mp.padding, mp.dilation))
            if (y.is_cuda and isinstance(mp, nn.MaxPool2d) and ints and mp.dilation == 1 and not mp.ceil_mode
                    and not mp.return_indices and y.shape[1] % 8 == 0 and 2 * mp.padding <= mp.kernel_size
                    and y.dtype in (torch.float32, torch.bfloat16) and not torch.is_grad_enabled()):
                from .. import functional as BF
                return BF.maxpool2d_hip(y, mp.kernel_size, mp.stride, mp.padding)
            return mp(y)

        def stem_pool_fusable(self, x):
            mp = self.maxpool
            if not STEM_POOL_FUSION:
                return False
            if not (isinstance(mp, nn.MaxPool2d) and mp.kernel_size in (3, (3, 3)) and mp.stride in (2, (2, 2))
                    and mp.padding in (1, (1, 1)) and mp.dilation in (1, (1, 1)) and not mp.ceil_mode
                    and not mp.return_indices and not torch.is_grad_enabled()):
                return False
            from .. import functional as BF
            cache = self.__dict__.setdefault("_stem_pool_ok", {})
            key = (tuple(x.shape), x.dtype, x.device, self.conv1.precision or BF.get_precision())
            if key not in cache:
                cache[key] = bool(self.conv1.pool_fusable(x))
            return cache[key]

        def fwd(self, x):
            if stem_pool_fusable(self, x):
                x = self._stem(x, None, True, pool=True)
            else:
                x = pool(self.maxpool, self._stem(x, None, True))
            x = self.layer4(self.layer3(self.layer2(self.layer1(x))))
            ap = self.avgpool
            is_global = (isinstance(ap, nn.AdaptiveAvgPool2d) and ap.output_size in (1, (1, 1))) or (
                isinstance(ap, nn.AvgPool2d) and ap.padding in (0, (0, 0)) and not ap.ceil_mode
                and ap.divisor_override is None
                and (ap.kernel_size if isinstance(ap.kernel_size, tuple) else (ap.kernel_size,) * 2) == tuple(x.shape[2:]))
            if (x.is_cuda and is_global and x.shape[1] % 8 == 0
                    and x.dtype in (torch.float32, torch.bfloat16) and not torch.is_grad_enabled()):
                from .. import functional as BF
                return self.fc(BF.avgpool_global_hip(x))
            return self.fc(ap(x).flatten(1))
        model.forward = types.MethodType(fwd, model)
        n += 1
    return n


def _basic_forward_train(self, x):
    if not (self.training and x.is_cuda):
        return self._btx_fwd_eval(x)
    from .. import autograd as _ag
    idt = x if self.downsample is None else self.downsample(x)
    y = _ag.bn_act(self.bn1, self.conv1(x))
# ... 421 lines not shown
```

### include/btx.h

```cpp
#ifndef BTX_H_
#define BTX_H_

#include <stddef.h>
#include <stdint.h>

#ifdef __cplusplus
extern "C" {
#endif

#define BTX_ABI_VERSION 9

#define BTX_E_NULL        (-1)
#define BTX_E_SHAPE       (-2)
#define BTX_E_UNSUPPORTED (-3)
#define BTX_E_WORKSPACE   (-4)
#define BTX_E_DTYPE       (-5)
#define BTX_E_ALIGN       (-6)

#define BTX_KIND_REPARAM 0
#define BTX_KIND_FLIPOUT 1
#define BTX_ACT_F32  0
#define BTX_ACT_BF16 1
#define BTX_PREC_F32  0
#define BTX_PREC_BF16 1
#define BTX_PREC_BF16X3 2
#define BTX_FLAG_TRANSPOSED   1u
#define BTX_FLAG_KL_ACCUM     2u
#define BTX_FLAG_ROWFUSE      4u
#define BTX_FLAG_OUT_F32      8u
#define BTX_FLAG_OUT_BF16    16u
#define BTX_FLAG_SWAP_SIGNS  64u
#define BTX_FLAG_CONCURRENT 128u
#define BTX_FLAG_REVERSE    256u
#define BTX_FLAG_GATHER      32u

#define BTX_FLAG_LANES_SHIFT 16
#define BTX_FLAG_LANES_MASK  (0xffu << BTX_FLAG_LANES_SHIFT)
#define BTX_FLAG_LANES(n)    (((uint32_t)(n) & 0xffu) << BTX_FLAG_LANES_SHIFT)

#define BTX_STREAM_EPS_W    0u
#define BTX_STREAM_EPS_B    1u
#define BTX_STREAM_SIGN_IN  2u
#define BTX_STREAM_SIGN_OUT 3u

typedef struct BtxGeom {
  int32_t NB, D, H, W, C;
  int32_t N;
  int32_t KD, KH, KW;
  int32_t sd, sh, sw;
  int32_t pd, ph, pw;
  int32_t dd, dh, dw;
  int32_t od, oh, ow;
  int32_t groups;
} BtxGeom;

typedef struct BtxRng {
  uint64_t seed;
  uint32_t sample_idx;
  uint32_t layer_id;
  const uint32_t* sample_idx_dev;
} BtxRng;

typedef struct BtxNoise {
  const float*  eps_w;
  const float*  eps_b;
  const int8_t* sign_in;
  const int8_t* sign_out;
  const void*   sampled_w;
} BtxNoise;

int         btx_abi_version(void);
const char* btx_strerror(int code);

size_t btx_kl_workspace_bytes(size_t n);
int btx_kl_gauss(const float* mu, const float* rho, size_t n,
                 const float* prior_mu_t, const float* prior_sigma_t,
                 float prior_mu, float prior_sigma,
                 float* kl_out, uint32_t flags, void* ws, size_t ws_bytes, void* stream);

typedef struct BtxKlItem {
  const float* mu;
  const float* rho;
  const float* prior_mu_t;
  const float* prior_sigma_t;
  float*       dmu;
  float*       drho;
  float        prior_mu, prior_sigma;
  size_t       n;
} BtxKlItem;
size_t btx_kl_model_workspace_bytes(int n_items);
int btx_kl_gauss_model(const BtxKlItem* items_host, int n_items, float* kl_out, void* ws, size_t ws_bytes, void* stream);
int btx_kl_gauss_model_bwd(const BtxKlItem* items_host, int n_items, const float* grad_out, void* stream);

size_t btx_contract_workspace_bytes(const BtxGeom* g, int kind, int act_dtype, int prec, uint32_t flags);
int btx_contract_fwd(int kind, const BtxGeom* g,
                     const void* x, const float* mu_w, const float* rho_w,
                     const float* mu_b, const float* rho_b,
                     void* out,
                     const BtxRng* rng, const BtxNoise* noise ,
                     int act_dtype, int prec, uint32_t flags,
                     void* ws, size_t ws_bytes, void* stream);

typedef struct BtxEpilogue {
  const float* scale;
  const float* shift;
  const void*  residual;
  int32_t      relu;
  int32_t      pool;
} BtxEpilogue;
int btx_contract_pool_shape(const BtxGeom* g, int act_dtype, int prec, uint32_t flags, int32_t* Hq, int32_t* Wq);
int btx_contract_fwd_ex(int kind, const BtxGeom* g,
                        const void* x, const float* mu_w, const float* rho_w,
                        const float* mu_b, const float* rho_b,
                        void* out,
                        const BtxRng* rng, const BtxNoise* noise ,
                        int act_dtype, int prec, uint32_t flags,
                        void* ws, size_t ws_bytes, void* stream,
                        const BtxEpilogue* epilogue );

typedef struct BtxLanes {
  int32_t n;
  int64_t x_stride, out_stride, res_stride;
} BtxLanes;
int btx_contract_fwd_lanes(int kind, const BtxGeom* g,
                           const void* x, const float* mu_w, const float* rho_w,
                           const float* mu_b, const float* rho_b,
                           void* out,
                           const BtxRng* rng, const BtxNoise* noise ,
                           int act_dtype, int prec, uint32_t flags,
                           void* ws, size_t ws_bytes, void* stream,
                           const BtxEpilogue* epilogue , const BtxLanes* lanes);

#define BTX_FAMILY_GATHER    0
#define BTX_FAMILY_REGSTAGE  1
#define BTX_FAMILY_DMA       2
#define BTX_FAMILY_GEMM8     3
#define BTX_FAMILY_PATCH     4
#define BTX_FAMILY_TAPS      5
#define BTX_FAMILY_TAPS2     6
#define BTX_FAMILY_STEM      7
#define BTX_FAMILY_STEM_POOL 8
typedef struct BtxPlanInfo {
  int32_t  family;
  int32_t  ksplits;
  int32_t  kper;
  int32_t  kgroups;
  int32_t  wide;
  int32_t  tall;
  int32_t  par_major;
  int32_t  pool_band;
  int32_t  nwg;
  int32_t  lanes;
  uint64_t ws_bytes;
} BtxPlanInfo;
int btx_contract_plan_info(int kind, const BtxGeom* g, int act_dtype, int prec, uint32_t flags,
                           const BtxEpilogue* ep , BtxPlanInfo* out);

int btx_contract_wgrad(int kind, const BtxGeom* g, const void* x, const void* dy, float* dw_mu, float* dw_delta,
                       float* db_mu, float* db_delta, const BtxRng* rng, const BtxNoise* noise ,
                       int act_dtype, uint32_t flags, void* stream);
size_t btx_wgrad_workspace_bytes(int kind, const BtxGeom* g, int act_dtype, uint32_t flags);
int btx_contract_wgrad_ws(int kind, const BtxGeom* g, const void* x, const void* dy, float* dw_mu, float* dw_delta,
                          float* db_mu, float* db_delta, const BtxRng* rng, const BtxNoise* noise ,
                          int act_dtype, uint32_t flags, void* ws, size_t ws_bytes, const float* rho_w ,
                          float* drho , void* stream);

typedef struct BtxSampleItem {
  const BtxGeom* geom;
  const float*   mu_w;
  const float*   rho_w;
  void*          out;
  int32_t        kind;
  uint32_t       layer_id;
  int32_t        src_KW, src_C;
} BtxSampleItem;
size_t btx_sampled_w_bytes(const BtxGeom* g, int kind, int prec);
int btx_sample_weights(const BtxSampleItem* items_host, int n_items, const BtxRng* rng ,
                       int prec, void* stream);
#define BTX_SAMPLE_SKIP_MU 1u
size_t btx_sampled_w_bytes_lanes(const BtxGeom* g, int kind, int prec, int lanes);
int btx_sample_weights_lanes(const BtxSampleItem* items_host, int n_items, const BtxRng* rng ,
                             int prec, void* stream, int lanes, uint32_t sflags);

int btx_dgrad_weights(const float* mu_w, const float* rho_w, float* out_mu, float* out_rho, float* out_eps, int N, int T, int C,
                      int flip, const BtxRng* rng, void* stream);

int btx_rho_grad(const float* dw, const float* rho, float* drho, size_t n, const BtxRng* rng, uint32_t rng_stream,
                 void* stream);

int btx_rowfuse_pack(const void* x, int in_dtype, const int64_t* strides_ncHW_host, int NB, int C, int H, int W,
                     void* out, int out_dtype, int Hp, int Wp, int cp, int ph, int pw, void* stream);

int btx_maxpool2d_cl(const void* x, void* out, int dtype, int NB, int H, int W, int C, int k, int stride, int pad,
                     void* stream);
int btx_maxpool2d_cl_train(const void* x, void* out, uint8_t* idx, int dtype, int NB, int H, int W, int C, int k, int stride,
                           int pad, void* stream);
int btx_maxpool2d_cl_bwd(const void* dy, const uint8_t* idx, void* dx, int dtype, int NB, int H, int W, int C, int k, int stride,
                         int pad, void* stream);

size_t btx_bn_workspace_bytes(long long M, int C);
typedef struct BtxBnFuse {
  const void* residual;
  int32_t     relu;
  void*       mask;
  void*       dres;
} BtxBnFuse;
int btx_bn_train_fwd(const void* x, void* y, int act_dtype, long long M, int C, const void* gamma, const void* beta,
                     void* running_mean, void* running_var, int param_dtype, float momentum, float eps, float* save_mean,
                     float* save_invstd, long long* num_batches_tracked ,
                     const BtxBnFuse* fuse , void* ws, size_t ws_bytes, void* stream);
int btx_bn_train_bwd(const void* x, const void* dy, void* dx, int act_dtype, long long M, int C, const void* gamma,
                     int param_dtype, const float* save_mean, const float* save_invstd, void* dgamma, void* dbeta,
                     const BtxBnFuse* fuse , void* ws, size_t ws_bytes, void* stream);

int btx_avgpool_global_cl(const void* x, void* out, int dtype, int NB, int HW, int C, void* stream);

int btx_out_shape(const BtxGeom* g, uint32_t flags, int32_t* Do, int32_t* Ho, int32_t* Wo);

int btx_fill_eps(float* out, size_t n, const BtxRng* rng, uint32_t rng_stream, void* stream);
int btx_fill_sign(int8_t* out, size_t n, const BtxRng* rng, uint32_t rng_stream, void* stream);

size_t btx_mc_packed_floats(int bs, int C);
int btx_mc_accumulate(const void* logits, int bs, int C, int act_dtype, float kl,
                      float* packed, void* stream);
int btx_mc_accumulate_lanes(const void* logits, int lanes, int bs, int C, int act_dtype, float kl,
                            float* packed, void* stream);

typedef struct BtxLstmLayer {
  const float* mu_w;
  const float* rho_w;
  const float* mu_b;
  const float* rho_b;
  uint32_t layer_id;
  uint32_t sample_idx;
  const void* sample_idx_dev;
} BtxLstmLayer;
// ... 128 lines not shown
```

Measured before the change: 1958.

## Hand off Flipout input signs from conv1 epilogue to conv2 via bf16 sign bits

In ResNet basic blocks using bf16 Flipout, conv1's epilogue now applies ReLU, packs outputs to bf16, and XORs the next layer's input-sign bits into each value's sign bit, which is zero after ReLU. A swizzled LDS layout feeds 128-bit buffer stores. conv2 then runs a CARRY variant of the taps kernel that skips generating and applying the Philox input signs, since they already sit in the activations. This targets the per-tile sign generation and sign multiply in conv2, at the cost of a more complex epilogue, eligibility checks in Python, and a dependence on both layers agreeing on the sample and sign keys.

```diff
diff --git a/bayesian_torch_amd/_lib.py b/bayesian_torch_amd/_lib.py
--- a/bayesian_torch_amd/_lib.py
+++ b/bayesian_torch_amd/_lib.py
@@ -10,6 +10,7 @@
 PREC_CODE = {"f32": 0, "bf16": 1, "bf16x3": 2}
 FLAG_TRANSPOSED, FLAG_KL_ACCUM, FLAG_ROWFUSE, FLAG_OUT_F32, FLAG_OUT_BF16, FLAG_GATHER, FLAG_SWAP_SIGNS, FLAG_CONCURRENT = 1, 2, 4, 8, 16, 32, 64, 128
 FLAG_REVERSE = 256
+FLAG_CARRY_OUT, FLAG_CARRIED_IN = 512, 1024
 E_UNSUPPORTED = -3
 STREAM_EPS_W, STREAM_EPS_B, STREAM_SIGN_IN, STREAM_SIGN_OUT = 0, 1, 2, 3
 ABI_VERSION = 9
@@ -39,7 +40,7 @@
 
 class Epilogue(ctypes.Structure):
     _fields_ = [("scale", ctypes.c_void_p), ("shift", ctypes.c_void_p), ("residual", ctypes.c_void_p),
-                ("relu", ctypes.c_int32), ("pool", ctypes.c_int32)]
+                ("relu", ctypes.c_int32), ("pool", ctypes.c_int32), ("carry_layer", ctypes.c_uint32)]
 
 
 class Lanes(ctypes.Structure):
@@ -49,7 +50,8 @@
 
 class PlanInfo(ctypes.Structure):
     _fields_ = [(n, ctypes.c_int32) for n in ("family", "ksplits", "kper", "kgroups", "wide", "tall", "par_major", "pool_band",
-                                              "nwg", "lanes")] + [("ws_bytes", ctypes.c_uint64)]
+                                              "nwg", "lanes")] + [("ws_bytes", ctypes.c_uint64), ("carry_out", ctypes.c_int32),
+                                                                  ("carry_in", ctypes.c_int32)]
 
 
 FAMILIES = ("gather", "regstage", "dma", "gemm8", "patch", "taps", "taps2", "stem", "stem_pool")
diff --git a/bayesian_torch_amd/csrc/btx_api.hip b/bayesian_torch_amd/csrc/btx_api.hip
--- a/bayesian_torch_amd/csrc/btx_api.hip
+++ b/bayesian_torch_amd/csrc/btx_api.hip
@@ -69,6 +69,9 @@
   }
   p.swap_signs = (flags & BTX_FLAG_SWAP_SIGNS) ? 1 : 0;
   p.reverse = (flags & BTX_FLAG_REVERSE) ? 1 : 0;
+  p.carry_out = (flags & BTX_FLAG_CARRY_OUT) ? 1 : 0;
+  p.carried_in = (flags & BTX_FLAG_CARRIED_IN) ? 1 : 0;
+  p.carry_layer = (p.carry_out && ep) ? ep->carry_layer : 0u;
   sign_keys(rng, p.swap_signs ? BTX_STREAM_SIGN_OUT : BTX_STREAM_SIGN_IN, &p.kin_a, &p.kin_b);
   sign_keys(rng, p.swap_signs ? BTX_STREAM_SIGN_IN : BTX_STREAM_SIGN_OUT, &p.kout_a, &p.kout_b);
   {
diff --git a/bayesian_torch_amd/csrc/btx_contract.h b/bayesian_torch_amd/csrc/btx_contract.h
--- a/bayesian_torch_amd/csrc/btx_contract.h
+++ b/bayesian_torch_amd/csrc/btx_contract.h
@@ -104,6 +104,8 @@
   long long lane_x, lane_out, lane_res, lane_wt, lane_partial;
   int lane_wt_delta;
   int reverse;
+  int carry_out, carried_in;
+  uint32_t carry_layer;
 };
 
 __device__ __forceinline__ uint32_t sample_word_scalar(const uint32_t* ptr) {
diff --git a/bayesian_torch_amd/csrc/btx_contract_patch.h b/bayesian_torch_amd/csrc/btx_contract_patch.h
--- a/bayesian_torch_amd/csrc/btx_contract_patch.h
+++ b/bayesian_torch_amd/csrc/btx_contract_patch.h
@@ -286,6 +286,12 @@
     }                                                                                                             \
     hipLaunchKernelGGL(kfn, dim3(nwg), dim3(256 * KG), p.pt_lds, st, p);                                          \
   } while (0)
+    if constexpr (PREC == 1) {
+      if (p.carried_in) {
+        if (p.pt_kg == 2) BTX_LAUNCH_TP(1, 2, false, true); else BTX_LAUNCH_TP(1, 1, false, true);
+        return (int)hipGetLastError();
+      }
+    }
     if (p.pt_kg == 2) { if (kind == 0) BTX_LAUNCH_TP(0, 2); else BTX_LAUNCH_TP(1, 2); }
     else {
       if constexpr (PREC == 1) {
diff --git a/bayesian_torch_amd/csrc/btx_contract_taps.h b/bayesian_torch_amd/csrc/btx_contract_taps.h
--- a/bayesian_torch_amd/csrc/btx_contract_taps.h
+++ b/bayesian_torch_amd/csrc/btx_contract_taps.h
@@ -40,9 +40,12 @@
   return n;
 }
 
-template <int PREC, int KIND, int KH, int KW, int KG, bool WIDE = false>
+template <int PREC, int KIND, int KH, int KW, int KG, bool WIDE = false, bool CARRY = false>
 __global__ __launch_bounds__(256 * KG, 2) void contract_taps_kernel(const ContractParams) {
   static_assert(!WIDE || (PREC == 1 && KG == 1 && KIND == 0), "wide tile: bf16 Reparameterization, one K-group");
+  static_assert(!CARRY || (PREC == 1 && KIND == 1 && !WIDE), "carried signs: bf16 Flipout, narrow tile");
+  constexpr bool SGN = (KIND == 1) && !CARRY;
+  constexpr bool ST16 = (PREC == 1 && KIND == 1);
   constexpr int K2 = (KIND == 1 || WIDE) ? 1 : 0;
   BTX_SECTION_PARAMS(p, logical);
   constexpr int NW = 4, NT = 256, MI = 2, T = KH * KW;
@@ -181,7 +184,7 @@
   }
 
   auto write_signs = [&](int slot, int cb) __attribute__((always_inline)) {
-    if constexpr (KIND == 1) {
+    if constexpr (SGN) {
       unsigned char* ss = smem + PT_S_OFF + slot * s_stage;
 #pragma unroll
       for (int j = 0; j < 2; ++j) {
@@ -245,7 +248,7 @@
 #pragma unroll
       for (int ni = 0; ni < 2; ++ni) f.wm[kk][ni] = *(const u32x4*)(ws + (row * BN + ni * 32 + l31) * 16);
     }
-    if constexpr (KIND == 1) {
+    if constexpr (SGN) {
 #pragma unroll
       for (int mi = 0; mi < MIA; ++mi) f.sw[mi] = *(const uint32_t*)(ss + q[mi] * 4);
     }
@@ -295,8 +298,8 @@
           load_delta<K2>(df, smem + PT_W_OFF + wslot * DW_STAGE, l31, h);
           constexpr int t1 = (t + 1) % T, c1 = (t + 1) / T;
           load_frag(nxt, PAR ^ c1, (t1 / KW) * row_step + (t1 % KW) * p.dw, (wslot + 1) & 3, mia_tag);
-          if constexpr (FIRST && t == 0) stage_mma<PREC, K2, MI, MIA, true, KIND == 1>(cur, df, accm, accd, l31, h);
-          else stage_mma<PREC, K2, MI, MIA, false, KIND == 1>(cur, df, accm, accd, l31, h);
+          if constexpr (FIRST && t == 0) stage_mma<PREC, K2, MI, MIA, true, SGN, CARRY>(cur, df, accm, accd, l31, h);
+          else stage_mma<PREC, K2, MI, MIA, false, SGN, CARRY>(cur, df, accm, accd, l31, h);
           if (!last) end_stage<WOPS + KP>();
           else end_stage<(c3 == 0) ? WOPS : 0>();
         } else {
@@ -305,7 +308,7 @@
           __builtin_amdgcn_sched_barrier(0);
           asm volatile("s_barrier" ::: "memory");
           __builtin_amdgcn_sched_barrier(0);
-          stage_mma<PREC, KIND, MI, MIA>(cur, df, accm, accd, l31, h);
+          stage_mma<PREC, KIND, MI, MIA, false, !CARRY, CARRY>(cur, df, accm, accd, l31, h);
           __builtin_amdgcn_sched_barrier(0);
           if (!last) {
             end_stage<2 * WOPS + KP + tp_pieces<T>(t - 1) + tp_pieces<T>(t - 2)>();
@@ -370,8 +373,8 @@
           staged_epilogue<0, NW>(pe, rl, accd, accd, smem, tid, wave, lane, 2 * ntile + 1, group, split, m0, nvalid, -1, true, ba1);
         }
       } else
-      if (tall) staged_epilogue_pm<KIND, NW, PixTall>(pe, rl, accm, accd, smem, tid, wave, lane, ntile, group, split, pmt);
-      else staged_epilogue<KIND, NW>(pe, rl, accm, accd, smem, tid, wave, lane, ntile, group, split, m0, nvalid);
+      if (tall) staged_epilogue_pm<KIND, NW, PixTall, false, EpNoHook, ST16>(pe, rl, accm, accd, smem, tid, wave, lane, ntile, group, split, pmt);
+      else staged_epilogue<KIND, NW, false, ST16>(pe, rl, accm, accd, smem, tid, wave, lane, ntile, group, split, m0, nvalid);
     } else {
       float* ba_lds = (float*)(smem_all + 131072);
       const bool to_partial = pe.ksplits > 1;
@@ -415,13 +418,13 @@
       }
       __syncthreads();
       if (kg == 0) {
-        if (tall) staged_epilogue_pm<KIND, NW, PixTall>(pe, rl, accm, accd, smem_all, tid, wave, lane, ntile, group, split, pmt, -1,
-                                                        true, ba_lds);
-        else staged_epilogue<KIND, NW>(pe, rl, accm, accd, smem_all, tid, wave, lane, ntile, group, split, m0, nvalid, -1, true,
-                                       ba_lds);
-      }
-    }
-  }
-}
-
-}
+        if (tall) staged_epilogue_pm<KIND, NW, PixTall, false, EpNoHook, ST16>(pe, rl, accm, accd, smem_all, tid, wave, lane, ntile, group,
+                                                                               split, pmt, -1, true, ba_lds);
+        else staged_epilogue<KIND, NW, false, ST16>(pe, rl, accm, accd, smem_all, tid, wave, lane, ntile, group, split, m0, nvalid, -1,
+                                                    true, ba_lds);
+      }
+    }
+  }
+}
+
+}
diff --git a/bayesian_torch_amd/csrc/btx_contract_taps2.h b/bayesian_torch_amd/csrc/btx_contract_taps2.h
--- a/bayesian_torch_amd/csrc/btx_contract_taps2.h
+++ b/bayesian_torch_amd/csrc/btx_contract_taps2.h
@@ -280,7 +280,7 @@
       staged_epilogue<0, NW>(pe, rl, accm, accm, smem, tid, wave, lane, 2 * ntile, group, split, m0, nvalid, -1, true, ba0);
       staged_epilogue<0, NW>(pe, rl, accd, accd, smem, tid, wave, lane, 2 * ntile + 1, group, split, m0, nvalid, -1, true, ba1);
     } else
-    staged_epilogue<KIND, NW>(pe, rl, accm, accd, smem, tid, wave, lane, ntile, group, split, m0, nvalid);
+    staged_epilogue<KIND, NW, false, PREC == 1 && KIND == 1>(pe, rl, accm, accd, smem, tid, wave, lane, ntile, group, split, m0, nvalid);
   }
 }
 
diff --git a/bayesian_torch_amd/csrc/btx_epilogue.h b/bayesian_torch_amd/csrc/btx_epilogue.h
--- a/bayesian_torch_amd/csrc/btx_epilogue.h
+++ b/bayesian_torch_amd/csrc/btx_epilogue.h
@@ -131,7 +131,7 @@
 struct EpNoHook {
   __device__ __forceinline__ void operator()() const {}
 };
-template <int KIND, int NW, class PM = PixContig, bool RES_PRE = false, class HOOK = EpNoHook>
+template <int KIND, int NW, class PM = PixContig, bool RES_PRE = false, class HOOK = EpNoHook, bool BF16ST = false>
 __device__ __forceinline__ void staged_epilogue_pm(const ContractParams& p, const RngLive& rl, const f32x16 (&accm)[2][2],
                                                    const f32x16 (&accd)[2][2], unsigned char* smem, int tid, int wave,
                                                    int lane, int ntile, int group, int split, const PM& pm,
@@ -185,8 +185,20 @@
 
   const bool fast = (ntile * BN + BN <= p.Ng) &&
                     (KIND == 0 || (!p.sign_out && (p.N & 31) == 0 && ((group * p.Ng) & 31) == 0));
+  const bool st16 = BF16ST && KIND == 1 && p.carry_out && fast && p.out_bf16 && !to_partial && p.ep_res == nullptr && p.ep_relu != 0 &&
+                    has_ba && ((p.N & 7) == 0) && (((group * p.Ng) & 7) == 0);
+  const int st_x = l31 & 7, st_h = (h ^ ((l31 >> 3) & 1)) * 8;
   if (fast) {
     uint32_t wsh[2][2];
+    uint32_t wcr[2][2] = {{0u, 0u}, {0u, 0u}};
+    uint32_t ckin_a = 0u, ckin_b = 0u;
+    const bool carry = st16;
+    if constexpr (KIND == 1 && BF16ST) {
+      if (carry) {
+        const BtxPhilox4 kc = btx_philox4x32_10(0u, rl.sample, p.carry_layer, p.swap_signs ? 3u : 2u, p.seed_lo, p.seed_hi);
+        ckin_a = __builtin_amdgcn_readfirstlane(kc.x[0]); ckin_b = __builtin_amdgcn_readfirstlane(kc.x[1]);
+      }
+    }
     uint32_t SB = 0x80000000u;
     asm volatile("" : "+s"(SB));
     if constexpr (KIND == 1) {
@@ -203,9 +215,24 @@
             wsh[mi][ni] = btx_sign_word((orow + 32u * ni) >> 5, rl.kout_a, rl.kout_b) << (2 * h);
         }
       }
-    }
-    auto body = [&](auto bias_tag, auto aff_tag) __attribute__((always_inline)) {
+      if constexpr (BF16ST) {
+        if (carry) {
+#pragma unroll
+          for (int mi = 0; mi < 2; ++mi) {
+            bool pok;
+            const uint32_t orow = pm(pwave * 64 + mi * 32 + l31, pok) * (uint32_t)p.N + (uint32_t)(group * p.Ng + ntile * BN);
+#pragma unroll
+            for (int ni = 0; ni < 2; ++ni) wcr[mi][ni] = btx_sign_word((orow + 32u * ni) >> 5, ckin_a, ckin_b) << (2 * h);
+          }
+        }
+      }
+    }
+    const float clamp_hi = p.ep_relu == 2 ? 6.f : __builtin_inff();
+    auto body = [&](auto bias_tag, auto aff_tag, auto st_tag) __attribute__((always_inline)) {
       constexpr bool BIAS = decltype(bias_tag)::value, BA = decltype(aff_tag)::value;
+      constexpr int ST = decltype(st_tag)::value;
+      uint32_t SB2 = 0x80008000u;
+      if constexpr (ST == 2) asm volatile("" : "+s"(SB2));
       struct Cst { f32x4 bm, bd, sc, sh; };
       auto ldc = [&](int g, Cst& c) __attribute__((always_inline)) {
         const int cl = (g >> 2) * 32 + 8 * (g & 3) + 4 * h;
@@ -240,15 +267,38 @@
               val += u2f(__builtin_amdgcn_bitop3_b32(f2u(dl), wsh[mi][ni] << sft, SB, 0x78));
             }
             if constexpr (BA) val = __builtin_fmaf(val, cur.sc[rr], cur.sh[rr]);
+            if constexpr (ST != 0) val = fminf(fmaxf(val, 0.f), clamp_hi);
             v[rr] = val;
           }
-          *(f32x4*)(ep + (mi * 32 + l31) * EP_ROW + cl * 4) = v;
+          if constexpr (ST == 0) {
+            *(f32x4*)(ep + (mi * 32 + l31) * EP_ROW + cl * 4) = v;
+          } else {
+            u32x2 pk = __builtin_bit_cast(u32x2, __builtin_convertvector(v, bf16x4));
+            if constexpr (ST == 2) {
+              pk[0] |= (wcr[mi][ni] << (4 * q)) & SB2;
+              pk[1] |= (wcr[mi][ni] << (4 * q + 1)) & SB2;
+            }
+            *(u32x2*)(ep + (mi * 32 + l31) * 128 + (((4 * ni + q) ^ st_x) << 4) + st_h) = pk;
+          }
         }
       });
     };
-    if (has_bias) body(std::true_type{}, std::true_type{});
-    else if (has_ba) body(std::false_type{}, std::true_type{});
-    else body(std::false_type{}, std::false_type{});
+    using EpF = std::false_type;
+    using EpT = std::true_type;
+    using St0 = std::integral_constant<int, 0>;
+    bool done16 = false;
+    if constexpr (BF16ST && KIND == 1) {
+      if (st16) {
+        done16 = true;
+        if (has_bias) body(EpT{}, EpT{}, std::integral_constant<int, 2>{});
+        else body(EpF{}, EpT{}, std::integral_constant<int, 2>{});
+      }
+    }
+    if (!done16) {
+      if (has_bias) body(EpT{}, EpT{}, St0{});
+      else if (has_ba) body(EpF{}, EpT{}, St0{});
+      else body(EpF{}, EpF{}, St0{});
+    }
   } else {
 #pragma unroll 1
     for (int mi = 0; mi < 2; ++mi) {
@@ -388,7 +438,30 @@
     };
     using T = std::true_type;
     using F = std::false_type;
-    if (all_vec) {
+    bool copied16 = false;
+    if constexpr (BF16ST && KIND == 1) {
+      if (st16) {
+        copied16 = true;
+        auto wk = pm.walk(pwave * 64 + (lane >> 3));
+        uint32_t boff[8];
+        u32x4 t[8];
+#pragma unroll
+        for (int i = 0; i < 8; ++i) {
+          bool ok;
+          const uint32_t gp = wk.get(ok);
+          wk.step8();
+          boff[i] = ok ? (gp * (uint32_t)p.N + cbase) * 2u : 0xfffffff0u;
+        }
+#pragma unroll
+        for (int i = 0; i < 8; ++i) t[i] = *(const u32x4*)(ep + (i * 8 + (lane >> 3)) * 128 + ((cg ^ (lane >> 3)) << 4));
+        const __amdgpu_buffer_rsrc_t out_rsrc = __builtin_amdgcn_make_buffer_rsrc((void*)p.out, 0, io_bytes, 0x00020000);
+#pragma unroll
+        for (int i = 0; i < 8; ++i)
+          __builtin_amdgcn_raw_buffer_store_b128((i & 1) ? (u32x4){t[i][2], t[i][3], t[i][0], t[i][1]} : t[i], out_rsrc, boff[i], 0, 0);
+      }
+    }
+    if (copied16) {
+    } else if (all_vec) {
       if (to_partial) fast(std::integral_constant<int, 0>{}, F{}, F{});
       else if (p.out_bf16) {
         if (res) { if (relu) fast(std::integral_constant<int, 1>{}, T{}, T{}); else fast(std::integral_constant<int, 1>{}, T{}, F{}); }
@@ -399,6 +472,15 @@
       }
     } else {
       auto wk = pm.walk(pwave * 64 + (lane >> 3));
+      bool carry_e = false;
+      uint32_t cke_a = 0u, cke_b = 0u;
+      if constexpr (BF16ST && KIND == 1) {
+        if (p.carry_out && !to_partial && p.out_bf16) {
+          carry_e = true;
+          const BtxPhilox4 kc = btx_philox4x32_10(0u, rl.sample, p.carry_layer, p.swap_signs ? 3u : 2u, p.seed_lo, p.seed_hi);
+          cke_a = __builtin_amdgcn_readfirstlane(kc.x[0]); cke_b = __builtin_amdgcn_readfirstlane(kc.x[1]);
+        }
+      }
 #pragma unroll 1
       for (int r8 = 0; r8 < 8; ++r8) {
         const int pix = r8 * 8 + (lane >> 3);
@@ -415,23 +497,29 @@
             if (res) y += p.out_bf16 ? (float)((const __bf16*)p.ep_res)[idx + j] : ((const float*)p.ep_res)[idx + j];
             if (relu) y = fmaxf(y, 0.f);
             if (relu6) y = fminf(y, 6.f);
-            if (p.out_bf16) ((__bf16*)p.out)[idx + j] = (__bf16)y;
-            else ((float*)p.out)[idx + j] = y;
-          }
-        }
-      }
-    }
-  }
-}
-
-template <int KIND, int NW, bool RES_PRE = false>
+            if (p.out_bf16) {
+              uint16_t hb = __builtin_bit_cast(uint16_t, (__bf16)y);
+              if (carry_e) {
+                const uint32_t io = idx + (uint32_t)j;
+                hb |= (uint16_t)(((btx_sign_word(io >> 5, cke_a, cke_b) >> btx_sign_bitpos(io & 31u)) & 1u) << 15);
+              }
+              ((uint16_t*)p.out)[idx + j] = hb;
+            } else ((float*)p.out)[idx + j] = y;
+          }
+        }
+      }
+    }
+  }
+}
+
+template <int KIND, int NW, bool RES_PRE = false, bool BF16ST = false>
 __device__ __forceinline__ void staged_epilogue(const ContractParams& p, const RngLive& rl, const f32x16 (&accm)[2][2],
                                                 const f32x16 (&accd)[2][2], unsigned char* smem, int tid, int wave,
                                                 int lane, int ntile, int group, int split, uint32_t m0, int nvalid,
                                                 int pwave = -1, bool first = true, float* ba_ext = nullptr) {
   const PixContig pm = {m0, nvalid};
-  staged_epilogue_pm<KIND, NW, PixContig, RES_PRE>(p, rl, accm, accd, smem, tid, wave, lane, ntile, group, split, pm, pwave, first,
-                                                   ba_ext);
-}
-
-}
+  staged_epilogue_pm<KIND, NW, PixContig, RES_PRE, EpNoHook, BF16ST>(p, rl, accm, accd, smem, tid, wave, lane, ntile, group, split, pm,
+                                                                     pwave, first, ba_ext);
+}
+
+}
diff --git a/bayesian_torch_amd/csrc/btx_mma.h b/bayesian_torch_amd/csrc/btx_mma.h
--- a/bayesian_torch_amd/csrc/btx_mma.h
+++ b/bayesian_torch_amd/csrc/btx_mma.h
@@ -47,9 +47,10 @@
   }
 }
 
-template <int PREC, int KIND, int MI = 2, int MIA = MI, bool ZERO = false, bool MASK = true>
+template <int PREC, int KIND, int MI = 2, int MIA = MI, bool ZERO = false, bool MASK = true, bool CARRY = false>
 __device__ __forceinline__ void stage_mma(StageFragT<MI>& f, const DeltaFrag& dfrag, f32x16 (&accm)[MI][2],
                                           f32x16 (&accd)[MI][2], int l31, int h) {
+    static_assert(!CARRY || (PREC == 1 && KIND == 1 && !MASK), "carried signs: bf16 Flipout, no mask chain");
     const u32x4 (&wd)[NG / 2][2] = dfrag.w;
     if constexpr (PREC == 2) {
       static_assert(NG == 4, "split-bf16: one 32x32x16 K-step per 16-k stage");
@@ -87,16 +88,19 @@
     for (int kk = 0; kk < NG / 2; ++kk) {
       if constexpr (PREC == 1) {
 #pragma unroll
-        for (int mi = 0; mi < MIA; ++mi)
+        for (int mi = 0; mi < MIA; ++mi) {
+          u32x4 am = f.a[kk][mi];
+          if constexpr (CARRY) am &= 0x7fff7fffu;
 #pragma unroll
           for (int ni = 0; ni < 2; ++ni) {
             if constexpr (ZERO) {
               const f32x16 zc = {0.f, 0.f, 0.f, 0.f, 0.f, 0.f, 0.f, 0.f, 0.f, 0.f, 0.f, 0.f, 0.f, 0.f, 0.f, 0.f};
               accm[mi][ni] = __builtin_amdgcn_mfma_f32_32x32x16_bf16(
-                  __builtin_bit_cast(bf16x8, f.wm[kk][ni]), __builtin_bit_cast(bf16x8, f.a[kk][mi]), kk == 0 ? zc : accm[mi][ni], 0, 0, 0);
+                  __builtin_bit_cast(bf16x8, f.wm[kk][ni]), __builtin_bit_cast(bf16x8, am), kk == 0 ? zc : accm[mi][ni], 0, 0, 0);
             } else accm[mi][ni] = __builtin_amdgcn_mfma_f32_32x32x16_bf16(
-                __builtin_bit_cast(bf16x8, f.wm[kk][ni]), __builtin_bit_cast(bf16x8, f.a[kk][mi]), accm[mi][ni], 0, 0, 0);
+                __builtin_bit_cast(bf16x8, f.wm[kk][ni]), __builtin_bit_cast(bf16x8, am), accm[mi][ni], 0, 0, 0);
           }
+        }
       } else {
 #pragma unroll
         for (int e = 0; e < 4; ++e)
diff --git a/bayesian_torch_amd/csrc/btx_plan.cpp b/bayesian_torch_amd/csrc/btx_plan.cpp
--- a/bayesian_torch_amd/csrc/btx_plan.cpp
+++ b/bayesian_torch_amd/csrc/btx_plan.cpp
@@ -418,6 +418,13 @@
   if (dma && patch) s->pt = pt;
   else s->pt.kg = 1;
   s->need = need; s->wt_off = wt_off; s->wt_one = wt_one; s->wt_all = wt_all;
+  const bool taps_bf16_flipout = kind == BTX_KIND_FLIPOUT && prec == BTX_PREC_BF16 && act_dtype == BTX_ACT_BF16 && pl.ksplits == 1;
+  s->carry_out_ok = taps_bf16_flipout && (s->family == BTX_FAMILY_TAPS || s->family == BTX_FAMILY_TAPS2) && out_bf16 && ep &&
+                    (ep->relu == 1 || ep->relu == 2) && !ep->residual && !ep->pool && (ep->scale || ep->shift) &&
+                    !(noise && noise->sign_out) && (pl.Ng % 32) == 0 && (g->N % 32) == 0;
+  s->carry_in_ok = taps_bf16_flipout && s->family == BTX_FAMILY_TAPS && !s->pt.wide && !(noise && noise->sign_in);
+  if ((flags & BTX_FLAG_CARRY_OUT) && !s->carry_out_ok) return BTX_E_UNSUPPORTED;
+  if ((flags & BTX_FLAG_CARRIED_IN) && !s->carry_in_ok) return BTX_E_UNSUPPORTED;
   return 0;
 }
 
@@ -490,8 +497,10 @@
   if (!g || !out) return BTX_E_NULL;
   memset(out, 0, sizeof(*out));
   FwdSel s;
-  const int rc = select_fwd(kind, g, act_dtype, prec, flags, false, nullptr, ep, &s);
+  const int rc = select_fwd(kind, g, act_dtype, prec, flags & ~(BTX_FLAG_CARRY_OUT | BTX_FLAG_CARRIED_IN), false, nullptr, ep, &s);
   if (rc) return rc;
+  out->carry_out = s.carry_out_ok;
+  out->carry_in = s.carry_in_ok;
   out->family = s.family;
   out->ksplits = s.pl.ksplits;
   out->kper = s.pl.kper;
diff --git a/bayesian_torch_amd/csrc/btx_plan.h b/bayesian_torch_amd/csrc/btx_plan.h
--- a/bayesian_torch_amd/csrc/btx_plan.h
+++ b/bayesian_torch_amd/csrc/btx_plan.h
@@ -48,6 +48,7 @@
   StemPoolPlan spp;
   PatchPlan pt;
   size_t need, wt_off, wt_one, wt_all;
+  int carry_out_ok, carry_in_ok;
 };
 static inline bool uses_tiles(int family) { return family >= BTX_FAMILY_DMA; }
 
diff --git a/bayesian_torch_amd/functional.py b/bayesian_torch_amd/functional.py
--- a/bayesian_torch_amd/functional.py
+++ b/bayesian_torch_amd/functional.py
@@ -263,6 +263,35 @@
                                      L.btx_contract_plan_info(kind, ctypes.byref(g), act, prec_c, flags & ~_lib.FLAG_LANES_MASK,
                                                               None, ctypes.byref(info)) == 0, op)
     return hit[0]
+
+
+def carry_plan(kind, op, nb, spatial, dtype, prec, lanes=1, epilogue=None, extra_flags=0):
+    L = _lib.lib()
+    g = _lib.Geom()
+    g.NB, (g.D, g.H, g.W), g.C, g.N = nb, spatial, op.in_channels, op.out_channels
+    g.KD, g.KH, g.KW = op.kernel
+    g.sd, g.sh, g.sw = op.stride
+    g.pd, g.ph, g.pw = op.padding
+    g.dd, g.dh, g.dw = op.dilation
+    g.od, g.oh, g.ow = op.output_padding
+    g.groups = op.groups
+    act = _lib.ACT_BF16 if dtype == torch.bfloat16 else _lib.ACT_F32
+    ep = None
+    if epilogue is not None:
+        ep = _lib.Epilogue()
+        ep.scale = 16 if epilogue.get("scale") is not None else None
+        ep.shift = 16 if epilogue.get("shift") is not None else None
+        ep.residual = 16 if epilogue.get("residual") is not None else None
+        ep.relu = act_code(epilogue.get("relu"))
+        ep.pool = 1 if epilogue.get("pool") else 0
+    flags = (_lib.FLAG_TRANSPOSED if op.transposed else 0) | extra_flags | (_lib.FLAG_CONCURRENT if _CONCURRENT else 0)
+    info = _lib.PlanInfo()
+    tries = [flags | (lanes << _lib.FLAG_LANES_SHIFT), flags | _lib.FLAG_CONCURRENT] if lanes > 1 else [flags]
+    for f in tries:
+        if L.btx_contract_plan_info(kind, ctypes.byref(g), act, _lib.PREC_CODE[prec], f, ctypes.byref(ep) if ep is not None else None,
+                                    ctypes.byref(info)) == 0:
+            return info
+    return None
 
 
 def act_code(act):
@@ -345,6 +374,8 @@
     flags = (_lib.FLAG_TRANSPOSED if op.transposed else 0) | extra_flags | (_lib.FLAG_CONCURRENT if _CONCURRENT else 0)
     if lanes > 1:
         flags |= lanes << _lib.FLAG_LANES_SHIFT
+    if epilogue is not None and epilogue.get("carry_layer") is not None:
+        flags |= _lib.FLAG_CARRY_OUT
     rev = 0
     if _ALT_ORDER:
         _ORDER_TOGGLE[0] ^= 1
@@ -428,6 +459,8 @@
             ep.residual = rp.data_ptr()
         ep.relu = act_code(epilogue.get("relu"))
         ep.pool = 1 if epilogue.get("pool") else 0
+        if epilogue.get("carry_layer") is not None:
+            ep.carry_layer = int(epilogue["carry_layer"]) & 0xFFFFFFFF
     args = (kind, ctypes.byref(g), xp.data_ptr(), mu_p.data_ptr(), rho_p.data_ptr(),
             mu_b.data_ptr() if mu_b is not None else None, rho_b.data_ptr() if rho_b is not None else None,
             out.data_ptr(), ctypes.byref(r), ctypes.byref(nz) if nz is not None else None,
diff --git a/bayesian_torch_amd/layers/base_variational_layer.py b/bayesian_torch_amd/layers/base_variational_layer.py
--- a/bayesian_torch_amd/layers/base_variational_layer.py
+++ b/bayesian_torch_amd/layers/base_variational_layer.py
@@ -320,11 +320,11 @@
             return pre[1]
         return None
 
-    def _forward_hip(self, x, noise=None, sample_idx=None, epilogue=None, gather=False):
+    def _forward_hip(self, x, noise=None, sample_idx=None, epilogue=None, gather=False, carried_in=False):
         if self._op.nd > 0 and x.dim() == self._op.nd + 1:
             if epilogue is not None and epilogue.get("residual") is not None:
                 epilogue = dict(epilogue, residual=epilogue["residual"].unsqueeze(0))
-            return self._forward_hip(x.unsqueeze(0), noise, sample_idx, epilogue, gather).squeeze(0)
+            return self._forward_hip(x.unsqueeze(0), noise, sample_idx, epilogue, gather, carried_in).squeeze(0)
         mu, rho = self._w()
         mu_p, rho_p = BF.gemm_major_view(mu, self._op), BF.gemm_major_view(rho, self._op)
         lanes, lane_batch = self._lanes()
@@ -370,7 +370,8 @@
         return BF.contract_hip(kind, x, mu_p, rho_p, mb, rb, op, _rng.seed(), sample_idx,
                                self._btx_layer_id, prec=self.precision, noise=noise, epilogue=epilogue, sampled_w=pre,
                                sample_dev=getattr(self, "_btx_sample_dev", None),
-                               extra_flags=_lib.FLAG_GATHER if gather else 0, lanes=lanes, lane_batch=lane_batch)
+                               extra_flags=(_lib.FLAG_GATHER if gather else 0) | (_lib.FLAG_CARRIED_IN if carried_in else 0),
+                               lanes=lanes, lane_batch=lane_batch)
 
     def _rowfuse_packed(self, x, plan, dtype):
         store = self.__dict__.get("_btx_static_x")
@@ -404,10 +405,16 @@
         return BF.contract_pool_ok(plan["op"], x.shape[0], (1, plan["Hp"], plan["Wp"]), torch.bfloat16, "bf16",
                                    _lib.FLAG_ROWFUSE)
 
-    def forward_fused(self, x, scale=None, shift=None, residual=None, relu=False, pool=False, act=None):
+    def forward_fused(self, x, scale=None, shift=None, residual=None, relu=False, pool=False, act=None, carry_layer=None,
+                      carried_in=False):
         relu = BF.act_code(act if act is not None else relu)
         if self._use_hip(x) and not self._needs_grad(x):
-            return self._forward_hip(x, epilogue=dict(scale=scale, shift=shift, residual=residual, relu=relu, pool=pool))
+            ep = dict(scale=scale, shift=shift, residual=residual, relu=relu, pool=pool)
+            if carry_layer is not None:
+                ep["carry_layer"] = carry_layer
+            return self._forward_hip(x, epilogue=ep, carried_in=carried_in)
+        if carry_layer is not None or carried_in:
+            raise _lib.BtxError("the sign hand-off is an inference-only GPU path (models.fuse.carry_handoff)")
         if pool:
             raise _lib.BtxError("forward_fused(pool=True) is an inference-only GPU path (pool_fusable)")
         out = self.forward(x, return_kl=False) if self._use_hip(x) else self._forward_aten(x, False)
diff --git a/bayesian_torch_amd/models/fuse.py b/bayesian_torch_amd/models/fuse.py
--- a/bayesian_torch_amd/models/fuse.py
+++ b/bayesian_torch_amd/models/fuse.py
@@ -5,6 +5,7 @@
 
 
 STEM_POOL_FUSION = True
+SIGN_HANDOFF = True
 
 
 def fold_bn(bn):
@@ -125,9 +126,55 @@
             self._ss, self._key = fold_bn(bn), key
         return self._ss
 
-    def __call__(self, x, residual=None, relu=False, pool=False):
+    def __call__(self, x, residual=None, relu=False, pool=False, **handoff):
         scale, shift = self._scale_shift()
-        return self.conv.forward_fused(x, scale, shift, residual, relu, pool=pool)
+        return self.conv.forward_fused(x, scale, shift, residual, relu, pool=pool, **handoff)
+
+
+def _handoff_static(c1, c2, x_shape, x_dtype, relu):
+    from .. import functional as BF
+    from .. import _lib
+    if not (x_dtype == torch.bfloat16 and len(x_shape) == 4):
+        return False
+    for c in (c1, c2):
+        if getattr(c, "_family", None) != "flipout" or (c.precision or BF.get_precision()) != "bf16":
+            return False
+        if c._op.nd != 2 or c._op.transposed or c._btx_cpad is not None or c._op.in_channels <= 4:
+            return False
+    if c1._op.out_channels != c2._op.in_channels or BF.act_code(relu) == 0:
+        return False
+    lanes, lane_batch = c1._lanes()
+    nb = int(lane_batch) if lanes > 1 else int(x_shape[0])
+    sp1 = (1,) + tuple(int(v) for v in x_shape[2:])
+    sp2 = c1._op.out_spatial(sp1)
+    if min(sp2) <= 0:
+        return False
+    ep = dict(scale=True, shift=True, relu=relu)
+    p1 = BF.carry_plan(_lib.KIND_FLIPOUT, c1._op, nb, sp1, x_dtype, "bf16", lanes, epilogue=ep)
+    p2 = BF.carry_plan(_lib.KIND_FLIPOUT, c2._op, nb, sp2, x_dtype, "bf16", lanes, epilogue=dict(ep, residual=True))
+    return bool(p1 is not None and p2 is not None and p1.carry_out and p2.carry_in and p2.family == _lib.FAMILIES.index("taps")
+                and p1.ksplits == 1 and p2.ksplits == 1)
+
+
+def carry_handoff(block, x, relu=True):
+    if not SIGN_HANDOFF:
+        return False
+    c1, c2 = block.conv1, block.conv2
+    if not (_is_var(c1) and _is_var(c2) and c1._use_hip(x)) or c1._needs_grad(x) or c2._needs_grad(None):
+        return False
+    d1, d2 = c1.__dict__, c2.__dict__
+    if (c1._btx_sample != c2._btx_sample or d1.get("_btx_sample_dev") is not d2.get("_btx_sample_dev")
+            or c1._lanes() != c2._lanes()):
+        return False
+    from .. import functional as BF
+    cache = block.__dict__.setdefault("_btx_handoff_ok", {})
+    key = (tuple(x.shape), x.dtype, x.device, BF.get_precision(), c1.precision, c2.precision, c1._lanes(), BF.act_code(relu),
+           BF._CONCURRENT)
+    if key not in cache:
+        if len(cache) > 64:
+            cache.clear()
+        cache[key] = _handoff_static(c1, c2, tuple(x.shape), x.dtype, relu)
+    return cache[key]
 
 
 def _downsample(self, x):
@@ -139,6 +186,10 @@
 
 def _basic_forward(self, x):
     idt = _downsample(self, x)
+    if carry_handoff(self, x):
+        y = self._f1(x, None, True, carry_layer=self.conv2._btx_layer_id)
+        self.__dict__["_btx_handoff_taken"] = self.__dict__.get("_btx_handoff_taken", 0) + 1
+        return self._f2(y, idt, True, carried_in=True)
     y = self._f1(x, None, True)
     return self._f2(y, idt, True)
 
diff --git a/include/btx.h b/include/btx.h
--- a/include/btx.h
+++ b/include/btx.h
@@ -32,6 +32,8 @@
 #define BTX_FLAG_SWAP_SIGNS  64u
 #define BTX_FLAG_CONCURRENT 128u
 #define BTX_FLAG_REVERSE    256u
+#define BTX_FLAG_CARRY_OUT  512u
+#define BTX_FLAG_CARRIED_IN 1024u
 #define BTX_FLAG_GATHER      32u
 
 #define BTX_FLAG_LANES_SHIFT 16
@@ -107,6 +109,7 @@
   const void*  residual;
   int32_t      relu;
   int32_t      pool;
+  uint32_t     carry_layer;
 } BtxEpilogue;
 int btx_contract_pool_shape(const BtxGeom* g, int act_dtype, int prec, uint32_t flags, int32_t* Hq, int32_t* Wq);
 int btx_contract_fwd_ex(int kind, const BtxGeom* g,
@@ -152,6 +155,8 @@
   int32_t  nwg;
   int32_t  lanes;
   uint64_t ws_bytes;
+  int32_t  carry_out;
+  int32_t  carry_in;
 } BtxPlanInfo;
 int btx_contract_plan_info(int kind, const BtxGeom* g, int act_dtype, int prec, uint32_t flags,
                            const BtxEpilogue* ep , BtxPlanInfo* out);
```

Result: no change. 1974, median of 6 (+0.8%).
